# psteinb/libmultiviewnative

Hardware: AMD Instinct MI355X
Metric: RL iterations/sec on 512^3 f32, 6 views (higher is better)
Workload: dtype f32

## Files before the change

libmultiviewnative_amd/csrc/mvn_backend_emu.cpp:

```cpp
#ifndef MVN_HOST_EMU
#error "mvn_backend_emu.cpp is only for the MVN_HOST_EMU test build"
#endif

#include <atomic>
#include <chrono>
#include <cstdlib>
#include <cstring>
#include <map>
#include <memory>
#include <mutex>
#include <stdexcept>
#include <string>
#include <vector>

#include "mvn_backend.hpp"
#include "mvn_fixed_geom.hpp"
#include "mvn_wave_rows.hpp"

namespace mvn {
namespace be {

#define MVN_DISPATCH_T(T_, CALL)                                   \
  switch (T_) {                                                    \
    case 16: { constexpr int TT = 16; CALL; } break;               \
    case 8: { constexpr int TT = 8; CALL; } break;                 \
    case 4: { constexpr int TT = 4; CALL; } break;                 \
    case 2: { constexpr int TT = 2; CALL; } break;                 \
    case 1: { constexpr int TT = 1; CALL; } break;                 \
    default: throw std::invalid_argument("mvn: unsupported tile width"); \
  }


const char* backend_name() { return "host-emulation (test only)"; }

int device_count() {
  const char* e = std::getenv("MVN_EMU_DEVICES");
  const int n = e ? std::atoi(e) : 1;
  return n > 0 ? n : 1;
}
static thread_local int t_device = 0;
void set_device(int d) {
  if (d < 0 || d >= device_count()) throw std::runtime_error("emu: invalid device ordinal " + std::to_string(d));
  t_device = d;
}
int get_device() { return t_device; }
void device_name(int, char* name256) {
  std::memset(name256, 0, 256);
  std::strcpy(name256, "mvn host emulation");
}
static std::mutex g_mem_mu;
static std::map<void*, std::pair<int, size_t>> g_live;
static std::map<int, size_t> g_used;
static size_t emu_total() {
  const char* e = std::getenv("MVN_EMU_TOTAL_MB");
  return e ? (size_t)std::atoll(e) << 20 : (size_t)8 << 30;
}
long long device_total_mem(int) { return (long long)emu_total(); }
void device_mem_info(size_t* f, size_t* t) {
  std::lock_guard<std::mutex> lk(g_mem_mu);
  const size_t total = emu_total(), used = g_used[t_device];
  *t = total;
  *f = used < total ? total - used : 0;
}
void device_arch(int, int* major, int* minor) {
  *major = 0;
  *minor = 0;
}

void* dmalloc(size_t bytes) {
  {
    std::lock_guard<std::mutex> lk(g_mem_mu);
    if (g_used[t_device] + bytes > emu_total())
      throw std::runtime_error("emu: device memory exhausted (" + std::to_string(g_used[t_device]) + " + " +
                               std::to_string(bytes) + " bytes > MVN_EMU_TOTAL_MB)");
  }
  void* p = std::malloc(bytes ? bytes : 1);
  if (!p) throw std::bad_alloc();
  std::lock_guard<std::mutex> lk(g_mem_mu);
  g_live[p] = std::make_pair(t_device, bytes);
  g_used[t_device] += bytes;
  return p;
}
void dfree(void* p) {
  if (!p) return;
  {
    std::lock_guard<std::mutex> lk(g_mem_mu);
    auto it = g_live.find(p);
    if (it != g_live.end()) {
      g_used[it->second.first] -= it->second.second;
      g_live.erase(it);
    }
  }
  std::free(p);
}
void h2d(void* d, const void* h, size_t bytes, stream_t) { std::memcpy(d, h, bytes); }
void d2h(void* h, const void* d, size_t bytes, stream_t) { std::memcpy(h, d, bytes); }
void d2d(void* dst, const void* src, size_t bytes, stream_t) { std::memmove(dst, src, bytes); }
void h2d_2d(void* d, size_t dpitch, const void* h, size_t hpitch, size_t width, size_t height,
            stream_t) {
  for (size_t r = 0; r < height; ++r)
    std::memcpy((char*)d + r * dpitch, (const char*)h + r * hpitch, width);
}
void d2h_2d(void* h, size_t hpitch, const void* d, size_t dpitch, size_t width, size_t height,
            stream_t) {
  for (size_t r = 0; r < height; ++r)
    std::memcpy((char*)h + r * hpitch, (const char*)d + r * dpitch, width);
}
void d2d_2d(void* dst, size_t dpitch, const void* src, size_t spitch, size_t width, size_t height,
            stream_t) {
  for (size_t r = 0; r < height; ++r)
    std::memmove((char*)dst + r * dpitch, (const char*)src + r * spitch, width);
}
void dzero(void* d, size_t bytes, stream_t) { std::memset(d, 0, bytes); }
void enable_peer_access(int dev, int peer) {
  if (dev < 0 || dev >= device_count() || peer < 0 || peer >= device_count()) throw std::runtime_error("emu: invalid peer");
}
void copy_peer(void* dst, int, const void* src, int, size_t bytes, stream_t) { std::memmove(dst, src, bytes); }

int pointer_device(const void*) { return POINTER_ANY; }

stream_t stream_create() { return (stream_t)1; }
stream_t stream_create_upload() { return (stream_t)1; }
void stream_destroy(stream_t) {}
void stream_sync(stream_t) {}
void stream_wait_event(stream_t, event_t) {}

struct EmuEvent {
  std::chrono::steady_clock::time_point t;
};
event_t event_create() { return new EmuEvent(); }
event_t event_create_sync() { return new EmuEvent(); }
void event_destroy(event_t e) { delete (EmuEvent*)e; }
void event_record(event_t e, stream_t) { ((EmuEvent*)e)->t = std::chrono::steady_clock::now(); }
void event_sync(event_t) {}
float event_elapsed_ms(event_t a, event_t b) {
  return std::chrono::duration<float, std::milli>(((EmuEvent*)b)->t - ((EmuEvent*)a)->t).count();
}

bool graphs_supported() { return false; }
void capture_begin(stream_t) { throw std::runtime_error("mvn: no graphs in the host emulation"); }
graph_exec_t capture_end(stream_t) { throw std::runtime_error("mvn: no graphs in the host emulation"); }
void graph_launch(graph_exec_t, stream_t) { throw std::runtime_error("mvn: no graphs in the host emulation"); }
void graph_destroy(graph_exec_t) {}

static bool emu_wave_rows(const RowsParams& p, int kind_bit) {
  const char* m = std::getenv("MVN_WAVE_ROWS_MASK");
  const int mask = m && *m ? std::atoi(m) : 31;
  return (mask & kind_bit) && p.fixed && !p.lines && p.h == WrCfg::H && p.C == WrCfg::H;
}

template <int MODE, int EPI>
static void emu_wave_rows_run(const RowsParams& p) {
  typedef FxCtx<WrRegs, WrCfg::NT> Ctx;
  const long pairs = (p.rows + 1) / 2;
  const long full = (pairs + WrCfg::WAVES - 1) / WrCfg::WAVES;
  const long grid = full > 2 ? (full + 2) / 3 : full;
#pragma omp parallel
  {
    std::vector<char> lds(sizeof(cfloat) * WrCfg::lds_cfloats + 64);
    std::unique_ptr<Ctx> ctx(new Ctx());
#pragma omp for schedule(static)
    for (long b = 0; b < grid; ++b) wr_rows_body<MODE, EPI>(p, b, grid, (cfloat*)lds.data(), *ctx);
  }
}

template <int MODE>
static void emu_wave_rows_mode(const RowsParams& p) {
  switch (p.epi.mode) {
    case MVN_EPI_DIVIDE: emu_wave_rows_run<MODE, MVN_EPI_DIVIDE>(p); break;
    case MVN_EPI_DIVIDE_U16: emu_wave_rows_run<MODE, MVN_EPI_DIVIDE_U16>(p); break;
    case MVN_EPI_DIVIDE_NM: emu_wave_rows_run<MODE, MVN_EPI_DIVIDE_NM>(p); break;
    case MVN_EPI_DIVIDE_NM_U16: emu_wave_rows_run<MODE, MVN_EPI_DIVIDE_NM_U16>(p); break;
    case MVN_EPI_UPDATE: emu_wave_rows_run<MODE, MVN_EPI_UPDATE>(p); break;
    case MVN_EPI_UPDATE_STATS: emu_wave_rows_run<MODE, MVN_EPI_UPDATE_STATS>(p); break;
    case MVN_EPI_UPDATE_TV: emu_wave_rows_run<MODE, MVN_EPI_UPDATE_TV>(p); break;
    case MVN_EPI_UPDATE_STATS_TV: emu_wave_rows_run<MODE, MVN_EPI_UPDATE_STATS_TV>(p); break;
    case MVN_EPI_DELTA:
      if (MODE == MVN_WR_C2R) {
        emu_wave_rows_run<MVN_WR_C2R, MVN_EPI_DELTA>(p);
        break;
      }
      throw std::invalid_argument("mvn: DELTA epilogue only in the plain c2r pass");
    default: emu_wave_rows_run<MODE, MVN_EPI_STORE>(p); break;
  }
}

template <int H>
static long emu_rows_grid(long ntiles) {
  return FxRowsCfg<H>::WALK && ntiles > 2 ? (ntiles + 2) / 3 : ntiles;
}

static void emu_rows_lines(const RowsParams& p, long ntiles, int kind) {
  constexpr int H = 256;
  typedef FxCtx<FxRowsRegs<H>, FxRowsCfg<H>::NT> Ctx;
  typedef FxCtx<FxRowsStatRegs<H>, FxRowsCfg<H>::NT> SCtx;
  typedef FxCtx<FxRowsNmRegs<H>, FxRowsCfg<H>::NT> NCtx;
  if (!fx_rows_lines_ok<H>() || !p.fixed || p.h != H || p.C != H || !p.nyq_packed || p.lines_d1 < 1 ||
      p.lines_d1 % FxRowsCfg<H>::T || p.row_base % FxRowsCfg<H>::T || p.rows != ntiles * FxRowsCfg<H>::T)
    throw std::invalid_argument("mvn: line-layout last-axis pass outside its range");
#pragma omp parallel
  {
    std::vector<char> lds(sizeof(cfloat) * FxRowsCfg<H>::lds_cfloats + 64);
    std::unique_ptr<Ctx> ctx(new Ctx());
    std::unique_ptr<SCtx> sctx(new SCtx());
    std::unique_ptr<NCtx> nctx(new NCtx());
#pragma omp for schedule(static)
    for (long t = 0; t < ntiles; ++t) {
      cfloat* l = (cfloat*)lds.data();
      if (kind == 0) {
        fx_rows_run<H, 0, MVN_EPI_STORE, Ctx, true>(p, t, ntiles, l, *ctx);
      } else if (kind == 1) {
        switch (p.epi.mode) {
          case MVN_EPI_DIVIDE: fx_rows_run<H, 1, MVN_EPI_DIVIDE, Ctx, true>(p, t, ntiles, l, *ctx); break;
          case MVN_EPI_DIVIDE_U16: fx_rows_run<H, 1, MVN_EPI_DIVIDE_U16, Ctx, true>(p, t, ntiles, l, *ctx); break;
          case MVN_EPI_DIVIDE_NM: fx_rows_run_nm<H, 1, MVN_EPI_DIVIDE_NM, NCtx, true>(p, t, ntiles, l, *nctx); break;
          case MVN_EPI_DIVIDE_NM_U16: fx_rows_run_nm<H, 1, MVN_EPI_DIVIDE_NM_U16, NCtx, true>(p, t, ntiles, l, *nctx); break;
          case MVN_EPI_UPDATE: fx_rows_run<H, 1, MVN_EPI_UPDATE, Ctx, true>(p, t, ntiles, l, *ctx); break;
          case MVN_EPI_UPDATE_STATS: fx_rows_run_stats<H, 1, SCtx, true>(p, t, ntiles, l, *sctx); break;
          case MVN_EPI_UPDATE_TV: fx_rows_run<H, 1, MVN_EPI_UPDATE_TV, Ctx, true>(p, t, ntiles, l, *ctx); break;
          case MVN_EPI_UPDATE_STATS_TV: fx_rows_run_stats<H, 1, SCtx, true, MVN_EPI_UPDATE_STATS_TV>(p, t, ntiles, l, *sctx); break;
          case MVN_EPI_DELTA: fx_rows_run<H, 1, MVN_EPI_DELTA, Ctx, true>(p, t, ntiles, l, *ctx); break;
          default: fx_rows_run<H, 1, MVN_EPI_STORE, Ctx, true>(p, t, ntiles, l, *ctx); break;
        }
      } else {
        switch (p.epi.mode) {
          case MVN_EPI_DIVIDE: fx_rows_run<H, 2, MVN_EPI_DIVIDE, Ctx, true>(p, t, ntiles, l, *ctx); break;
          case MVN_EPI_DIVIDE_U16: fx_rows_run<H, 2, MVN_EPI_DIVIDE_U16, Ctx, true>(p, t, ntiles, l, *ctx); break;
          case MVN_EPI_DIVIDE_NM: fx_rows_run_nm<H, 2, MVN_EPI_DIVIDE_NM, NCtx, true>(p, t, ntiles, l, *nctx); break;
          case MVN_EPI_DIVIDE_NM_U16: fx_rows_run_nm<H, 2, MVN_EPI_DIVIDE_NM_U16, NCtx, true>(p, t, ntiles, l, *nctx); break;
          case MVN_EPI_UPDATE: fx_rows_run<H, 2, MVN_EPI_UPDATE, Ctx, true>(p, t, ntiles, l, *ctx); break;
          case MVN_EPI_UPDATE_STATS: fx_rows_run_stats<H, 2, SCtx, true>(p, t, ntiles, l, *sctx); break;
          case MVN_EPI_UPDATE_TV: fx_rows_run<H, 2, MVN_EPI_UPDATE_TV, Ctx, true>(p, t, ntiles, l, *ctx); break;
          case MVN_EPI_UPDATE_STATS_TV: fx_rows_run_stats<H, 2, SCtx, true, MVN_EPI_UPDATE_STATS_TV>(p, t, ntiles, l, *sctx); break;
          default: fx_rows_run<H, 2, MVN_EPI_STORE, Ctx, true>(p, t, ntiles, l, *ctx); break;
        }
      }
    }
  }
}

static std::atomic<long> g_mid_fused_launches{0};
long mid_fused_launch_count() { return g_mid_fused_launches.load(); }

template <int K>
static void emu_mid_fused(const MidFusedParams& p) {
  typedef FxCtx<MfRegs<K>, MF_NT> Ctx;
  const long blocks = mf_blocks(p);
#pragma omp parallel
  {
    std::vector<cfloat> lds(MF_LDS_CFLOATS + 8);
    std::unique_ptr<Ctx> ctx(new Ctx());
#pragma omp for schedule(static)
    for (long b = 0; b < blocks; ++b) mf_body<K>(p, b, lds.data(), *ctx);
  }
}
#define MVN_MF_TAP_COUNTS(X) X(1) X(3) X(5) X(7) X(9) X(11) X(13) X(15) X(17) X(19) X(21) X(23) X(25) X(27) X(29) X(31)
void launch_mid_fused(const MidFusedParams& p, stream_t) {
  mf_check(p);
  if (p.mode == MF_TAPS) {
    typedef FxCtx<MfRegs<1>, MF_NT> Ctx;
    const long blocks = mf_blocks(p);
#pragma omp parallel
    {
      std::vector<cfloat> lds(MF_LDS_CFLOATS + 8);
      std::unique_ptr<Ctx> ctx(new Ctx());
#pragma omp for schedule(static)
      for (long b = 0; b < blocks; ++b) mf_taps_body(p, b, lds.data(), *ctx);
    }
    return;
  }
  ++g_mid_fused_launches;
  switch (mvn_dim0_taps_template(p.k)) {
#define X(K) case K: emu_mid_fused<K>(p); break;
    MVN_MF_TAP_COUNTS(X)
#undef X
    default: throw std::invalid_argument("mvn: no fused middle pass for this tap count");
  }
}

template <int H>
static void emu_rows_fused(const RowsParams& p, long ntiles) {
  typedef FxCtx<FxRowsRegs<H>, FxRowsCfg<H>::NT> Ctx;
  typedef FxCtx<FxRowsStatRegs<H>, FxRowsCfg<H>::NT> SCtx;
  typedef FxCtx<FxRowsNmRegs<H>, FxRowsCfg<H>::NT> NCtx;
  const long grid = emu_rows_grid<H>(ntiles);
#pragma omp parallel
  {
    std::vector<char> lds(sizeof(cfloat) * FxRowsCfg<H>::lds_cfloats + 64);
    std::unique_ptr<Ctx> ctx(new Ctx());
    std::unique_ptr<SCtx> sctx(new SCtx());
    std::unique_ptr<NCtx> nctx(new NCtx());
#pragma omp for schedule(static)
    for (long t = 0; t < grid; ++t) {
      cfloat* l = (cfloat*)lds.data();
      switch (p.epi.mode) {
        case MVN_EPI_DIVIDE: fx_rows_run<H, 2, MVN_EPI_DIVIDE>(p, t, grid, l, *ctx); break;
        case MVN_EPI_DIVIDE_U16: fx_rows_run<H, 2, MVN_EPI_DIVIDE_U16>(p, t, grid, l, *ctx); break;
        case MVN_EPI_DIVIDE_NM: fx_rows_run_nm<H, 2, MVN_EPI_DIVIDE_NM, NCtx>(p, t, grid, l, *nctx); break;
        case MVN_EPI_DIVIDE_NM_U16: fx_rows_run_nm<H, 2, MVN_EPI_DIVIDE_NM_U16, NCtx>(p, t, grid, l, *nctx); break;
        case MVN_EPI_UPDATE: fx_rows_run<H, 2, MVN_EPI_UPDATE>(p, t, grid, l, *ctx); break;
        case MVN_EPI_UPDATE_STATS: fx_rows_run_stats<H, 2, SCtx>(p, t, grid, l, *sctx); break;
        case MVN_EPI_UPDATE_TV: fx_rows_run<H, 2, MVN_EPI_UPDATE_TV>(p, t, grid, l, *ctx); break;
        case MVN_EPI_UPDATE_STATS_TV: fx_rows_run_stats<H, 2, SCtx, false, MVN_EPI_UPDATE_STATS_TV>(p, t, grid, l, *sctx); break;
        default: fx_rows_run<H, 2, MVN_EPI_STORE>(p, t, grid, l, *ctx); break;
      }
    }
  }
}

void launch_rows_c2r_r2c(const RowsParams& p0, long ntiles, int, size_t lds_bytes, stream_t) {
  RowsParams p = p0;
  mvn_arm_poison(p.epi);
  if (p.lines) return emu_rows_lines(p, ntiles, 2);
  if (emu_wave_rows(p, mvn_epi_divides(p.epi.mode) ? 4 : 8)) return emu_wave_rows_mode<MVN_WR_C2R_R2C>(p);
  if (!p.fixed) {
#pragma omp parallel
    {
      std::vector<char> lds(lds_bytes + 64);
#pragma omp for schedule(static)
      for (long t = 0; t < ntiles; ++t) {
        cfloat* l = (cfloat*)lds.data();
        if (p.epi.mode == MVN_EPI_UPDATE_STATS) {
          MVN_DISPATCH_T(p.T, (rows_c2r_even_body<TT, true, true>(p, t, 0, 1, l)));
        } else if (p.epi.mode == MVN_EPI_UPDATE_STATS_TV) {
          MVN_DISPATCH_T(p.T, (rows_c2r_even_body<TT, true, true, false, true>(p, t, 0, 1, l)));
        } else if (p.epi.mode == MVN_EPI_UPDATE_TV) {
          MVN_DISPATCH_T(p.T, (rows_c2r_even_body<TT, true, false, false, true>(p, t, 0, 1, l)));
        } else if (p.epi.mode == MVN_EPI_DIVIDE_NM) {
          MVN_DISPATCH_T(p.T, (rows_c2r_even_body<TT, true, false, false, false, true>(p, t, 0, 1, l)));
        } else if (p.epi.mode == MVN_EPI_DIVIDE_NM_U16) {
          MVN_DISPATCH_T(p.T, (rows_c2r_even_body<TT, true, false, true, false, true>(p, t, 0, 1, l)));
        } else if (p.epi.mode == MVN_EPI_DIVIDE_U16) {
          MVN_DISPATCH_T(p.T, (rows_c2r_even_body<TT, true, false, true>(p, t, 0, 1, l)));
        } else {
          MVN_DISPATCH_T(p.T, (rows_c2r_even_body<TT, true>(p, t, 0, 1, l)));
        }
      }
    }
    return;
  }
  switch (p.h) {
#define X(H) case H: emu_rows_fused<H>(p, ntiles); return;
    MVN_FIXED_ROWS_LENGTHS(X)
#undef X
    default: throw std::invalid_argument("mvn: no fixed kernel");
  }
}

template <int H>
static void emu_rows_fixed(const RowsParams& p, long ntiles, bool r2c) {
  typedef FxCtx<FxRowsRegs<H>, FxRowsCfg<H>::NT> Ctx;
  typedef FxCtx<FxRowsStatRegs<H>, FxRowsCfg<H>::NT> SCtx;
  typedef FxCtx<FxRowsNmRegs<H>, FxRowsCfg<H>::NT> NCtx;
  const long grid = emu_rows_grid<H>(ntiles);
#pragma omp parallel
  {
    std::vector<char> lds(sizeof(cfloat) * FxRowsCfg<H>::lds_cfloats + 64);
    std::unique_ptr<Ctx> ctx(new Ctx());
    std::unique_ptr<SCtx> sctx(new SCtx());
    std::unique_ptr<NCtx> nctx(new NCtx());
#pragma omp for schedule(static)
    for (long t = 0; t < grid; ++t) {
      cfloat* l = (cfloat*)lds.data();
      if (r2c)
        fx_rows_run<H, 0, MVN_EPI_STORE>(p, t, grid, l, *ctx);
      else {
        switch (p.epi.mode) {
          case MVN_EPI_DIVIDE: fx_rows_run<H, 1, MVN_EPI_DIVIDE>(p, t, grid, l, *ctx); break;
          case MVN_EPI_DIVIDE_U16: fx_rows_run<H, 1, MVN_EPI_DIVIDE_U16>(p, t, grid, l, *ctx); break;
          case MVN_EPI_DIVIDE_NM: fx_rows_run_nm<H, 1, MVN_EPI_DIVIDE_NM, NCtx>(p, t, grid, l, *nctx); break;
          case MVN_EPI_DIVIDE_NM_U16: fx_rows_run_nm<H, 1, MVN_EPI_DIVIDE_NM_U16, NCtx>(p, t, grid, l, *nctx); break;
          case MVN_EPI_UPDATE: fx_rows_run<H, 1, MVN_EPI_UPDATE>(p, t, grid, l, *ctx); break;
          case MVN_EPI_UPDATE_STATS: fx_rows_run_stats<H, 1, SCtx>(p, t, grid, l, *sctx); break;
          case MVN_EPI_UPDATE_TV: fx_rows_run<H, 1, MVN_EPI_UPDATE_TV>(p, t, grid, l, *ctx); break;
          case MVN_EPI_UPDATE_STATS_TV: fx_rows_run_stats<H, 1, SCtx, false, MVN_EPI_UPDATE_STATS_TV>(p, t, grid, l, *sctx); break;
          case MVN_EPI_DELTA: fx_rows_run<H, 1, MVN_EPI_DELTA>(p, t, grid, l, *ctx); break;
          default: fx_rows_run<H, 1, MVN_EPI_STORE>(p, t, grid, l, *ctx); break;
        }
      }
    }
  }
}

template <int N, int MODE>
static void emu_strided_fixed_mode(const StridedParams& p0, long nblocks) {
  typedef FxStridedSel<N, MODE> Sel;
  typedef typename Sel::Ctx Ctx;
  StridedParams p = p0;
  p.nblocks = nblocks;
  const long grid = nblocks > 1 ? (nblocks + 1) / 2 : 1;
#pragma omp parallel
  {
    std::vector<char> lds(sizeof(cfloat) * FxStridedCfg<N>::lds_cfloats + 64);
    std::unique_ptr<Ctx> ctx(new Ctx());
#pragma omp for schedule(static)
    for (long b = 0; b < grid; ++b) Sel::run(p, b, nblocks, grid, (cfloat*)lds.data(), *ctx);
  }
}

static std::atomic<long> g_split_launches{0};
long split_launch_count() { return g_split_launches.load(); }

template <int N>
static bool emu_try_split(int mode, const StridedParams& p, long nblocks) {
  if constexpr (FxSplitCfg<N>::USE) {
    typedef FxSplitCfg<N> C;
    if (mode == MVN_ST_FWD_MUL_INV || p.cstride != 1 || p.ncols % C::T != 0 || p.tiles_per_outer < 1)
      return false;
    StridedParams q = p;
    const long outer = nblocks / p.tiles_per_outer;
    q.tiles_per_outer = p.ncols / C::T;
    q.T = q.TP = C::T;
    const long nb = outer * q.tiles_per_outer;
    q.nblocks = nb;
    ++g_split_launches;
    const long grid = nb > 1 ? (nb + 1) / 2 : 1;
    typedef FxCtx<FxSplitRegs<N>, C::NT> Ctx;
#pragma omp parallel
    {
      std::vector<char> lds(sizeof(cfloat) * C::lds_cfloats + 64);
      std::unique_ptr<Ctx> ctx(new Ctx());
#pragma omp for schedule(static)
      for (long b = 0; b < grid; ++b) {
        if (mode == MVN_ST_FWD)
          fx_strided_split_body<N, MVN_ST_FWD>(q, b, nb, grid, (cfloat*)lds.data(), *ctx);
        else
          fx_strided_split_body<N, MVN_ST_INV>(q, b, nb, grid, (cfloat*)lds.data(), *ctx);
      }
    }
    return true;
  } else {
    (void)mode; (void)p; (void)nblocks;
    return false;
  }
}

template <int N>
static void emu_strided_fixed(int mode, const StridedParams& p, long nblocks) {
  if (emu_try_split<N>(mode, p, nblocks)) return;
  if (mode == MVN_ST_FWD) emu_strided_fixed_mode<N, MVN_ST_FWD>(p, nblocks);
  if (mode == MVN_ST_INV) emu_strided_fixed_mode<N, MVN_ST_INV>(p, nblocks);
  if (mode == MVN_ST_FWD_MUL_INV) emu_strided_fixed_mode<N, MVN_ST_FWD_MUL_INV>(p, nblocks);
}

static bool emu_rows_fixed_dispatch(const RowsParams& p, long ntiles, bool r2c) {
  switch (p.h) {
#define X(H) case H: emu_rows_fixed<H>(p, ntiles, r2c); return true;
    MVN_FIXED_ROWS_LENGTHS(X)
#undef X
    default: return false;
  }
}

static bool emu_strided_fixed_dispatch(int mode, const StridedParams& p, long nblocks) {
  switch (p.ax.n) {
#define X(N) case N: emu_strided_fixed<N>(mode, p, nblocks); return true;
    MVN_FIXED_STRIDED_LENGTHS(X)
#undef X
    default: return false;
  }
}

void launch_rows_r2c(const RowsParams& p, bool even, long ntiles, int, size_t lds_bytes,
                     stream_t) {
  if (p.lines) return emu_rows_lines(p, ntiles, 0);
  if (emu_wave_rows(p, 1)) return emu_wave_rows_run<MVN_WR_R2C, MVN_EPI_STORE>(p);
  if (p.fixed) {
    if (!emu_rows_fixed_dispatch(p, ntiles, true)) throw std::invalid_argument("mvn: no fixed kernel");
    return;
  }
#pragma omp parallel
  {
    std::vector<char> lds(lds_bytes + 64);
#pragma omp for schedule(static)
    for (long t = 0; t < ntiles; ++t) {
      cfloat* l = (cfloat*)lds.data();
      if (even) {
        MVN_DISPATCH_T(p.T, rows_r2c_even_body<TT>(p, t, 0, 1, l));
      } else {
        MVN_DISPATCH_T(p.T, rows_r2c_odd_body<TT>(p, t, 0, 1, l));
      }
    }
  }
}

void launch_rows_c2r(const RowsParams& p0, bool even, long ntiles, int, size_t lds_bytes,
                     stream_t) {
  RowsParams p = p0;
  mvn_arm_poison(p.epi);
  if (p.lines) return emu_rows_lines(p, ntiles, 1);
  if (emu_wave_rows(p, p.epi.mode == MVN_EPI_DELTA ? 16 : 2)) return emu_wave_rows_mode<MVN_WR_C2R>(p);
  if (p.fixed) {
    if (!emu_rows_fixed_dispatch(p, ntiles, false)) throw std::invalid_argument("mvn: no fixed kernel");
    return;
  }
#pragma omp parallel
  {
    std::vector<char> lds(lds_bytes + 64);
#pragma omp for schedule(static)
    for (long t = 0; t < ntiles; ++t) {
      cfloat* l = (cfloat*)lds.data();
// ... 293 lines not shown
```

libmultiviewnative_amd/csrc/mvn_engine.cpp:

```cpp
#include "mvn_engine.hpp"

#include <algorithm>
#include <cmath>
#include <atomic>
#include <cstdlib>
#include <cstring>

#include "mvn_fixed_geom.hpp"

#include <cstdio>
#include <cstdlib>
#include <cstring>
#include <stdexcept>

namespace mvn {

static const size_t kLdsSoftBudget = 80 * 1024;
static const size_t kLdsHardBudget = 160 * 1024;
static const size_t kSideMinBytes = 16u << 20;

const char* kernel_kind_name(int k) {
  static const char* names[KK_COUNT] = {"rows_r2c",    "rows_c2r",  "rows_fused_div",
                                        "rows_fused_upd", "axis1_fwd", "axis1_inv",
                                        "axis0_fused", "axis0_fwd",  "axis0_inv",
                                        "nyquist",     "other",     "axis0_direct", "mid_fused",
                                        "tv_factor"};
  return (k >= 0 && k < KK_COUNT) ? names[k] : "?";
}

be::Event Profiler::get_event() {
  if (pool_.empty()) return be::Event::timing();
  be::Event e = std::move(pool_.back());
  pool_.pop_back();
  return e;
}

void Profiler::begin(int kind, be::stream_t s) {
  if (!enabled) return;
  Rec r;
  r.kind = kind;
  r.a = get_event();
  r.b = get_event();
  be::event_record(r.a.get(), s);
  recs_.push_back(std::move(r));
}

void Profiler::end(be::stream_t s) {
  if (!enabled || recs_.empty()) return;
  be::event_record(recs_.back().b.get(), s);
}

void Profiler::collect() {
  for (size_t i = 0; i < recs_.size(); ++i) {
    be::event_sync(recs_[i].b.get());
    total_ms[recs_[i].kind] += be::event_elapsed_ms(recs_[i].a.get(), recs_[i].b.get());
    count[recs_[i].kind] += 1;
    pool_.push_back(std::move(recs_[i].a));
    pool_.push_back(std::move(recs_[i].b));
  }
  recs_.clear();
}

void Profiler::reset() {
  collect();
  for (int k = 0; k < KK_COUNT; ++k) {
    total_ms[k] = 0;
    count[k] = 0;
  }
}

Profiler::~Profiler() {
  try {
    collect();
  } catch (...) {
  }
}

struct ProfScope {
  Profiler* p;
  be::stream_t s;
  ProfScope(Profiler* p_, int kind, be::stream_t s_) : p(p_), s(s_) {
    if (p) p->begin(kind, s);
  }
  ~ProfScope() {
    if (p) p->end(s);
  }
};

template <typename T>
static be::DeviceBuffer<T> upload(const std::vector<T>& src) {
  be::DeviceBuffer<T> d(sizeof(T) * src.size());
  be::h2d(d.get(), src.data(), sizeof(T) * src.size(), nullptr);
  return d;
}

DevAxis::DevAxis(int n, bool composite) : host(n, composite) {
  tw = upload(host.tw);
  rev = upload(host.rev);
  inv = upload(host.inv);
  if (!host.tws.empty()) tws = upload(host.tws);
  if (host.bluestein) {
    chirp = upload(host.chirp);
    bhat = upload(host.bhat);
  }
  be::stream_sync(nullptr);
  view = host.view(tw.get(), rev.get(), inv.get(), tws.get(), chirp.get(), bhat.get());
}

static int env_int(const char* name, int dflt) {
  const char* v = std::getenv(name);
  return (v && *v) ? std::atoi(v) : dflt;
}

PassGeom Plan3D::pick_geom(int n, bool generic, bool rows, int max_t) {
  static const int cand[5] = {16, 8, 4, 2, 1};
  PassGeom g;
  bool found = false;
  for (int pass = 0; pass < 2 && !found; ++pass) {
    const size_t budget = pass == 0 ? kLdsSoftBudget : kLdsHardBudget;
    for (int i = 0; i < 5; ++i) {
      const int T = cand[i];
      if (T > max_t) continue;
      const int TP = rows ? (T | 1) : T;
      const size_t one = (size_t)n * (size_t)TP * sizeof(cfloat);
      const size_t twb = (size_t)n * sizeof(cfloat);
      const size_t bytes = one * (generic ? 2 : 1) + twb;
      if (bytes <= budget) {
        g.T = T;
        g.TP = TP;
        g.lds_bytes = bytes;
        g.lds_alt = generic ? (long)n * TP : 0;
        g.lds_tw = (long)n * TP * (generic ? 2 : 1);
        found = true;
        break;
      }
    }
  }
  if (!found)
    throw std::invalid_argument("mvn: axis length " + std::to_string(n) +
                                " does not fit the single-pass LDS FFT (160 KiB)");
  if (!rows && g.T < 8 && max_t >= 8) {
    const size_t one = (size_t)n * 8 * sizeof(cfloat);
    const size_t bytes = one * (generic ? 2 : 1) + (size_t)n * sizeof(cfloat);
    if (bytes <= kLdsHardBudget - 4096) {
      g.T = g.TP = 8;
      g.lds_bytes = bytes;
      g.lds_alt = generic ? (long)n * 8 : 0;
      g.lds_tw = (long)n * 8 * (generic ? 2 : 1);
    }
  }
  const long work = (long)n * g.T / 8;
  g.threads = work >= 512 ? 512 : (work >= 256 ? 256 : (work >= 128 ? 128 : 64));
  return g;
}

FormSwitches FormSwitches::from_env() {
  FormSwitches sw;
  sw.direct = env_int("MVN_DIM0_DIRECT", 1) != 0;
  sw.direct_max = env_int("MVN_DIM0_DIRECT_MAX", MVN_D0_MAX_TAPS);
  sw.min_plane = env_int("MVN_DIM0_DIRECT_MIN_PLANE", 131072);
  sw.min_items = env_int("MVN_DIM0_DIRECT_MIN_ITEMS", 0);
  sw.mid_fused = env_int("MVN_MID_FUSED", 1);
  sw.fixed = env_int("MVN_NO_FIXED", 0) == 0;
  return sw;
}

bool rows_fixed(const Layout& L, bool fixed) {
  int T = 0, threads = 0;
  size_t lds = 0;
  return fixed && L.even && fixed_rows_geom(L.h, &T, &threads, &lds) && L.rows % (size_t)T == 0;
}
bool ax1_fixed(const Layout& L, bool fixed) {
  int T = 0, threads = 0;
  size_t lds = 0;
  return fixed && fixed_strided_geom(L.d1, &T, &threads, &lds) && L.C % T == 0;
}
bool ax0_fixed(const Layout& L, bool fixed) {
  int T = 0, threads = 0;
  size_t lds = 0;
  return fixed && fixed_strided_geom(L.d0, &T, &threads, &lds) && ((long)L.d1 * L.C) % T == 0;
}

bool lines_capable(const Layout& L, bool fixed) {
  int T = 0, threads = 0;
  size_t lds = 0;
  return rows_fixed(L, fixed) && fixed_rows_geom(L.h, &T, &threads, &lds) && T == 16 && L.h == 256 && L.C == 256 &&
         L.d1 == MF_N1;
}

bool FormRule::direct(const int* kdims) const {
  if (!sw.direct || kdims[0] > sw.direct_max || !mvn_dim0_direct_possible(kdims[0], L.d0) ||
      mvn_dim0_items_for(kdims[0], L.d0, (long)L.d1 * L.C, sw.min_plane) < sw.min_items)
    return false;
  const Layout T(taps_depth(kdims[0]), L.d1, L.d2);
  return rows_fixed(T, sw.fixed) == rows_fixed(L, plan_fixed) && ax1_fixed(T, sw.fixed) == ax1_fixed(L, plan_fixed);
}

bool FormRule::lines_taps(const int* kdims) const {
  return sw.mid_fused != 0 && lines_capable(L, plan_fixed) && direct(kdims) &&
         lines_capable(Layout(taps_depth(kdims[0]), L.d1, L.d2), sw.fixed) && mvn_dim0_taps_template(kdims[0]) <= 31;
}

bool FormRule::lines_worth(int k0) const { return sw.mid_fused >= 2 || L.d0 >= 3 * k0; }

bool FormRule::all_direct(const kernel_list_t& k) const {
  for (const std::array<int, 3>& d : k)
    if (!direct(d.data())) return false;
  return true;
}

bool FormRule::all_lines(const kernel_list_t& k) const {
  for (const std::array<int, 3>& d : k)
    if (!lines(d.data())) return false;
  return true;
}

Plan3D::Plan3D(int dev, int d0, int d1, int d2, bool fixed_allowed)
    : device(dev), L(d0, d1, d2), fixed(fixed_allowed), ax2(L.h, rows_fixed(L, fixed)), ax1(d1, ax1_fixed(L, fixed)),
      ax0(d0, ax0_fixed(L, fixed)) {
  no_poison = be::DeviceBuffer<unsigned>(64);
  be::dzero(no_poison.get(), 64, nullptr);
  be::stream_sync(nullptr);
  if (L.even) {
    std::vector<cfloat> roots((size_t)L.h / 2 + 1);
    for (size_t k = 0; k < roots.size(); ++k) {
      double a = -2.0 * M_PI * (double)k / (double)d2;
      roots[k].x = (float)std::cos(a);
      roots[k].y = (float)std::sin(a);
    }
    twr = be::DeviceBuffer<cfloat>(sizeof(cfloat) * roots.size());
    be::h2d(twr.get(), roots.data(), sizeof(cfloat) * roots.size(), nullptr);
    be::stream_sync(nullptr);
  }
  g_rows = pick_geom(ax2.host.nfft, ax2.host.generic, true, 16);
  g_ax1 = pick_geom(ax1.host.nfft, ax1.host.generic, false, 16);
  g_ax0 = pick_geom(ax0.host.nfft, ax0.host.generic, false, 16);
  g_nyq1 = g_ax1;
  g_nyq0 = g_ax0;
  g_nyq1_line = pick_geom(ax1.host.nfft, ax1.host.generic, false, 1);
  {
    int T = 0, threads = 0;
    size_t lds = 0;
    if (rows_fixed(L, fixed)) {
      fixed_rows_geom(L.h, &T, &threads, &lds);
      fx_rows = true;
      gx_rows.T = T;
      gx_rows.threads = threads;
      gx_rows.lds_bytes = lds;
    }
    if (ax1_fixed(L, fixed)) {
      fixed_strided_geom(d1, &T, &threads, &lds);
      fx_ax1 = true;
      gx_ax1.T = gx_ax1.TP = T;
      gx_ax1.threads = threads;
      gx_ax1.lds_bytes = lds;
    }
    if (ax0_fixed(L, fixed)) {
      fixed_strided_geom(d0, &T, &threads, &lds);
      fx_ax0 = true;
      gx_ax0.T = gx_ax0.TP = T;
      gx_ax0.threads = threads;
      gx_ax0.lds_bytes = lds;
    }
  }
}

static long rows_in_range(const Plan3D& P, long row0, long nrows) {
  const long all = (long)P.L.rows;
  const long n = nrows < 0 ? all - row0 : nrows;
  if (row0 < 0 || n < 1 || row0 + n > all) throw std::out_of_range("mvn: row range of a last-axis pass");
  if (P.rows_need_full_tiles() && (row0 % P.rows_tile() || n % P.rows_tile()))
    throw std::logic_error("mvn: a row range of the fixed last-axis kernels must be whole tiles");
  return n;
}

static void lines_args(const Plan3D& P, RowsParams& p, long row0, const void* nyq, const void* real_side,
                       const void* cplx_side) {
  if (!P.lines_capable()) throw std::logic_error("mvn: this shape has no line-layout last-axis passes");
  if (nyq) throw std::logic_error("mvn: the line layout keeps the Nyquist bins in the DC column");
  if (real_side && real_side == cplx_side) throw std::logic_error("mvn: a plain last-axis pass on the line layout is out of place");
  p.lines = 1;
  p.lines_d1 = P.L.d1;
  p.row_base = row0;
  p.nyq_packed = 1;
}

void Plan3D::rows_r2c(const float* in_real, cfloat* out, cfloat* out_nyq, be::stream_t s,
                      Profiler* prof, long row0, long nrows, bool lines) const {
  const long R = rows_in_range(*this, row0, nrows);
  const void* real0 = in_real;
  in_real += row0 * L.RP;
  if (!lines) out += row0 * L.C;
  if (out_nyq) out_nyq += row0;
  RowsParams p;
  std::memset(&p, 0, sizeof(p));
  p.ax = ax2.view;
  p.twr = twr.get();
  p.d2 = L.d2;
  p.h = L.h;
  p.C = L.C;
  p.RP = L.RP;
  p.rows = R;
  p.T = g_rows.T;
  p.TP = g_rows.TP;
  p.lds_alt = g_rows.lds_alt;
  p.lds_tw = g_rows.lds_tw;
  p.hmul = mvn_fastdiv_mul((unsigned)L.h);
  p.Cmul = mvn_fastdiv_mul((unsigned)L.C);
  p.in_real = in_real;
  p.out_cplx = out;
  p.out_nyq = out_nyq;
  p.nyq_packed = (L.even && !out_nyq) ? 1 : 0;
  if (lines) lines_args(*this, p, row0, out_nyq, real0, out);
  ProfScope ps(prof, KK_ROWS_R2C, s);
  if (fx_rows) {
    p.fixed = 1;
    p.T = gx_rows.T;
    be::launch_rows_r2c(p, true, R / p.T, gx_rows.threads, gx_rows.lds_bytes, s);
    return;
  }
  const long ntiles = (R + p.T - 1) / p.T;
  be::launch_rows_r2c(p, L.even, ntiles, g_rows.threads, g_rows.lds_bytes, s);
}

void Plan3D::rows_c2r(const cfloat* in, const cfloat* in_nyq, float* out_real,
                      const EpilogueParams& epi_all, be::stream_t s, Profiler* prof, long row0,
                      long nrows, bool lines, const MvnStatsParams* st) const {
  const long R = rows_in_range(*this, row0, nrows);
  const void* cplx0 = in;
  const void* real0 = out_real;
  if (!lines) in += row0 * L.C;
  if (in_nyq) in_nyq += row0;
  if (out_real) out_real += row0 * L.RP;
  EpilogueParams epi = epi_all;
  const long eoff = row0 * L.RP;
  if (mvn_epi_u16(epi.mode) && row0 != 0) throw std::logic_error("mvn: a row range on a uint16 image volume");
  if (epi.view) epi.view += eoff;
  if (epi.psi) epi.psi += eoff;
  if (epi.weights) epi.weights += eoff;
  if (epi.delta) epi.delta += eoff;
  if (epi.tv) epi.tv += eoff;
  RowsParams p;
  std::memset(&p, 0, sizeof(p));
  p.ax = ax2.view;
  p.twr = twr.get();
  p.d2 = L.d2;
  p.h = L.h;
  p.C = L.C;
  p.RP = L.RP;
  p.rows = R;
  p.T = g_rows.T;
  p.TP = g_rows.TP;
  p.lds_alt = g_rows.lds_alt;
  p.lds_tw = g_rows.lds_tw;
  p.hmul = mvn_fastdiv_mul((unsigned)L.h);
  p.Cmul = mvn_fastdiv_mul((unsigned)L.C);
  p.in_cplx = in;
  p.in_nyq = in_nyq;
  p.nyq_packed = (L.even && !in_nyq) ? 1 : 0;
  if (lines) lines_args(*this, p, row0, in_nyq, real0, cplx0);
  p.out_real = out_real;
  p.epi = epi;
  if (!p.epi.poison) {
    p.epi.poison = no_poison.get();
    p.epi.poison_epoch = 0xffffffffu;
  }
  if (st) {
    p.st = *st;
    p.st.row0 = row0;
  }
  ProfScope ps(prof, KK_ROWS_C2R, s);
  if (fx_rows) {
    p.fixed = 1;
    p.T = gx_rows.T;
    be::launch_rows_c2r(p, true, R / p.T, gx_rows.threads, gx_rows.lds_bytes, s);
    return;
  }
  const long ntiles = (R + p.T - 1) / p.T;
  be::launch_rows_c2r(p, L.even, ntiles, g_rows.threads, g_rows.lds_bytes, s);
}

void Plan3D::rows_c2r_r2c(cfloat* data, cfloat* nyq, const EpilogueParams& epi_all, be::stream_t s,
                          Profiler* prof, long row0, long nrows, bool lines, const MvnStatsParams* st) const {
  if (!L.even) throw std::logic_error("mvn: rows_c2r_r2c needs an even last extent");
  const long R = rows_in_range(*this, row0, nrows);
  if (!lines) data += row0 * L.C;
  if (nyq) nyq += row0;
  EpilogueParams epi = epi_all;
  const long eoff = row0 * L.RP;
  if (mvn_epi_u16(epi.mode) && row0 != 0) throw std::logic_error("mvn: a row range on a uint16 image volume");
  if (epi.view) epi.view += eoff;
  if (epi.psi) epi.psi += eoff;
  if (epi.weights) epi.weights += eoff;
  if (epi.delta) epi.delta += eoff;
  if (epi.tv) epi.tv += eoff;
  RowsParams p;
  std::memset(&p, 0, sizeof(p));
  p.ax = ax2.view;
  p.twr = twr.get();
  p.d2 = L.d2;
  p.h = L.h;
  p.C = L.C;
  p.RP = L.RP;
  p.rows = R;
  p.in_cplx = data;
  p.in_nyq = nyq;
  p.out_cplx = data;
  p.out_nyq = nyq;
  p.nyq_packed = nyq ? 0 : 1;
  if (lines) lines_args(*this, p, row0, nyq, nullptr, nullptr);
  p.epi = epi;
  if (!p.epi.poison) {
    p.epi.poison = no_poison.get();
    p.epi.poison_epoch = 0xffffffffu;
  }
  if (st) {
    p.st = *st;
    p.st.row0 = row0;
  }
  ProfScope ps(prof, mvn_epi_reads_psi(epi.mode) ? KK_ROWS_FUSED_UPD : KK_ROWS_FUSED, s);
  if (fx_rows) {
    p.fixed = 1;
    p.T = gx_rows.T;
    be::launch_rows_c2r_r2c(p, R / p.T, gx_rows.threads, gx_rows.lds_bytes, s);
    return;
  }
  p.T = g_rows.T;
  p.TP = g_rows.TP;
  p.lds_alt = g_rows.lds_alt;
  p.lds_tw = g_rows.lds_tw;
  p.hmul = mvn_fastdiv_mul((unsigned)L.h);
  p.Cmul = mvn_fastdiv_mul((unsigned)L.C);
  const long ntiles = (R + p.T - 1) / p.T;
  be::launch_rows_c2r_r2c(p, ntiles, g_rows.threads, g_rows.lds_bytes, s);
}

void Plan3D::mid_fused(const cfloat* in, cfloat* out, const cfloat* taps, int k, int kd, unsigned* poison,
                       unsigned poison_epoch, be::stream_t s, Profiler* prof, int zbeg, int zcount, int n_peers,
                       unsigned* const* peers) const {
  if (!lines_capable()) throw std::logic_error("mvn: this shape has no fused middle pass");
  MidFusedParams p;
  std::memset(&p, 0, sizeof(p));
  p.in = in;
  p.out = out;
  p.taps = taps;
  p.kd = kd;
  p.tw = ax1.view.tw;
  p.d0 = L.d0;
  p.H = L.C;
  p.k = k;
  p.h = k / 2;
  p.seg = 0;
  p.mode = MF_CONV;
  p.packed = 1;
  p.poison = poison;
  p.poison_epoch = poison_epoch;
  p.zbeg = zbeg;
  p.zcount = zcount;
  p.n_peers = n_peers;
  p.poison_peers = peers;
  ProfScope ps(prof, KK_MID_FUSED, s);
  be::launch_mid_fused(p, s);
}

void Plan3D::taps_to_lines(cfloat* taps, be::stream_t s) const {
  if (!lines_capable()) throw std::logic_error("mvn: this shape has no fused middle pass");
  MidFusedParams p;
  std::memset(&p, 0, sizeof(p));
  p.in = taps;
  p.out = taps;
  p.tw = ax1.view.tw;
  p.d0 = L.d0;
  p.H = L.C;
  p.mode = MF_TAPS;
  be::launch_mid_fused(p, s);
}

static StridedParams make_strided(const DevAxis& ax, const PassGeom& g, cfloat* data,
                                  const cfloat* spec, long ostride, long estride, long cstride,
                                  int ncols) {
  StridedParams p;
  std::memset(&p, 0, sizeof(p));
  p.ax = ax.view;
  p.data = data;
  p.spec = spec;
  p.ostride = ostride;
  p.estride = estride;
  p.cstride = cstride;
  p.ncols = ncols;
  p.T = g.T;
  p.TP = g.TP;
  p.lds_alt = g.lds_alt;
  p.lds_tw = g.lds_tw;
  p.tiles_per_outer = (ncols + g.T - 1) / g.T;
  return p;
}

void SideStream::create() {
  s = be::Stream::create();
  fork = be::Event::sync_only();
  join = be::Event::sync_only();
}

void SideStream::fork_from(be::stream_t main) {
  be::event_record(fork.get(), main);
  be::stream_wait_event(s.get(), fork.get());
}

void SideStream::join_into(be::stream_t main) {
  be::event_record(join.get(), s.get());
  be::stream_wait_event(main, join.get());
}

void Plan3D::axis1(int mode, cfloat* data, cfloat* nyq, be::stream_t s, Profiler* prof,
                   be::stream_t s_nyq, int z0, int nz) const {
  if (!s_nyq) s_nyq = s;
  if (nz < 0) nz = L.d0 - z0;
  if (z0 < 0 || nz < 1 || z0 + nz > L.d0) throw std::out_of_range("mvn: plane range of a dim1 pass");
  data += (size_t)z0 * L.d1 * L.C;
  if (nyq) nyq += (size_t)z0 * L.d1;
  const bool ride = nyq_rides() && L.even && nyq;
  {
    const PassGeom& g = fx_ax1 ? gx_ax1 : g_ax1;
    StridedParams p = make_strided(ax1, g, data, nullptr, (long)L.d1 * L.C, L.C, 1, L.C);
    p.fixed = fx_ax1 ? 1 : 0;
    ProfScope ps(prof, mode == MVN_ST_FWD ? KK_AXIS1_FWD : KK_AXIS1_INV, s);
    if (ride) {
      StridedParams r = make_strided(ax1, g_nyq1_line, nyq, nullptr, 0, 1, L.d1, nz);
      r.is_nyq = 1;
      be::launch_strided(mode, p, (long)nz * p.tiles_per_outer, g.threads, g.lds_bytes, s, &r, g_nyq1_line.lds_bytes);
    } else {
      be::launch_strided(mode, p, (long)nz * p.tiles_per_outer, g.threads, g.lds_bytes, s);
    }
  }
  if (L.even && nyq && !ride) {
    StridedParams p = make_strided(ax1, g_nyq1, nyq, nullptr, 0, 1, L.d1, nz);
    p.is_nyq = 1;
    ProfScope ps(s_nyq == s ? prof : nullptr, KK_NYQ, s_nyq);
    be::launch_strided(mode, p, p.tiles_per_outer, g_nyq1.threads, g_nyq1.lds_bytes, s_nyq);
  }
}

void Plan3D::retile_spectrum(const cfloat* natural, cfloat* tiled, be::stream_t s) const {
  const long cols = (long)L.d1 * L.C;
  const int T = gx_ax0.T;
  be::launch_copy3d((float*)tiled, 2L * T, 2L * T * L.d0, (const float*)natural, 2L * cols, 2L * T, 2 * T,
                    L.d0, (int)(cols / T), s);
}

void Plan3D::axis0(int mode, cfloat* data, cfloat* nyq, const cfloat* spec,
                   const cfloat* spec_nyq, be::stream_t s, Profiler* prof, be::stream_t s_nyq,
                   const cfloat* src, const cfloat* src_nyq, bool spec_tiled) const {
  if (!s_nyq) s_nyq = s;
  const int kind = mode == MVN_ST_FWD ? KK_AXIS0_FWD
                                      : (mode == MVN_ST_INV ? KK_AXIS0_INV : KK_AXIS0_FUSED);
  {
    const long cols = (long)L.d1 * L.C;
    if (cols > 0x7fffffffL) throw std::invalid_argument("mvn: d1*d2 too large");
    const PassGeom& g = fx_ax0 ? gx_ax0 : g_ax0;
    StridedParams p = make_strided(ax0, g, data, spec, 0, cols, 1, (int)cols);
    p.fixed = fx_ax0 ? 1 : 0;
    p.src = src;
    if (spec_tiled && !fx_ax0) throw std::logic_error("mvn: tile-contiguous spectra need the fixed dim0 kernels");
    p.spec_tiled = spec_tiled ? 1 : 0;
    ProfScope ps(prof, kind, s);
    be::launch_strided(mode, p, p.tiles_per_outer, g.threads, g.lds_bytes, s);
  }
  if (L.even) {
    StridedParams p = make_strided(ax0, g_nyq0, nyq, spec_nyq, 0, L.d1, 1, L.d1);
    p.is_nyq = 1;
    p.src = src_nyq;
    ProfScope ps(s_nyq == s ? prof : nullptr, KK_NYQ, s_nyq);
    be::launch_strided(mode, p, p.tiles_per_outer, g_nyq0.threads, g_nyq0.lds_bytes, s_nyq);
  }
}

void Plan3D::forward(float* vol, cfloat* nyq, be::stream_t s, Profiler* prof) const {
  rows_r2c(vol, (cfloat*)vol, nyq, s, prof);
  axis1(MVN_ST_FWD, (cfloat*)vol, nyq, s, prof);
  axis0(MVN_ST_FWD, (cfloat*)vol, nyq, nullptr, nullptr, s, prof);
}

void Plan3D::backward(float* vol, cfloat* nyq, float scale, be::stream_t s,
                      Profiler* prof) const {
  axis0(MVN_ST_INV, (cfloat*)vol, nyq, nullptr, nullptr, s, prof);
  axis1(MVN_ST_INV, (cfloat*)vol, nyq, s, prof);
// ... 2070 lines not shown
```

libmultiviewnative_amd/csrc/mvn_fixed.hpp:

```cpp
#pragma once

#include <type_traits>

#include "mvn_pass_bodies.hpp"

#if defined(__HIPCC__) && !defined(MVN_HOST_EMU)
typedef float4 qfloat;
#else
struct alignas(16) qfloat {
  float x, y, z, w;
};
#endif

MVN_HD qfloat qmake(float x, float y, float z, float w) {
  qfloat q;
  q.x = x;
  q.y = y;
  q.z = z;
  q.w = w;
  return q;
}

#if defined(__HIPCC__) && !defined(MVN_HOST_EMU)
template <typename Regs, int NT>
// ... 647 lines not shown
  constexpr int R = fx_radix(N, S), M = fx_M(N, S), CH = C::CH, TPQ = C::TPQ, NT = C::NT;
  static_assert(C::M0 % (R * M) == 0, "a stage's blocks must tile a sub-line");
  constexpr int nwork = (C::W / R) * CH;
  constexpr int iters = (nwork + NT - 1) / NT;
  qfloat* buf = reinterpret_cast<qfloat*>(bufc);
#pragma unroll
  for (int it = 0; it < iters; ++it) {
    const int w = tid + it * NT;
    if (nwork % NT != 0 && w >= nwork) break;
    const int b = w / CH, q = w % CH;
    const int blk = b / M, j2 = b % M;
    qfloat* p = buf + (blk * R * M + j2) * TPQ + q;
    qfloat a[R];
#pragma unroll
    for (int j = 0; j < R; ++j) a[j] = p[j * M * TPQ];
    cfloat tw[fx_rs(R)];
    fx_tw_row<R>(twl + (fx_twoff(N, S) - C::TW1) + j2 * fx_rs(R), tw);
    if (!DIF) {
#pragma unroll
      for (int k = 1; k < R; ++k) a[k] = fx_qmul_dir<SIGN>(a[k], tw[k]);
    }
    fx_dft_q<R, SIGN>(a);
    if (DIF) {
#pragma unroll
      for (int k = 1; k < R; ++k) a[k] = fx_qmul_dir<SIGN>(a[k], tw[k]);
    }
#pragma unroll
    for (int j = 0; j < R; ++j) p[j * M * TPQ] = a[j];
    MVN_SCHED_FENCE();
  }
}

template <int N, int SIGN, bool DIF, int S, int TO, typename Ctx>
struct FxStagesQWin {
  static MVN_HD void run(cfloat* buf, const cfloat* twl, Ctx& ctx) {
    constexpr int NT_ = FxSplitCfg<N>::NT;
    (void)NT_;
    if constexpr (DIF ? (S <= TO) : (S >= TO)) {
      MVN_PHASE(ctx, (fx_stage_q_win<N, S, SIGN, DIF>(buf, twl, tid)));
      FxStagesQWin<N, SIGN, DIF, DIF ? S + 1 : S - 1, TO, Ctx>::run(buf, twl, ctx);
    }
  }
};

template <int N>
MVN_HD void fx_sp_tables(const StridedParams& P, cfloat* twl, int tid) {
  typedef FxSplitCfg<N> C;
  fx_copy_table<C::NT>(twl, P.ax.tws + C::TW1, fx_twsize(N) - C::TW1, tid);
}

template <int N, int WIN>
MVN_HD void fx_sp_collect(const cfloat* buf, FxSplitRegs<N>& r, int tid) {
  typedef FxSplitCfg<N> C;
#pragma unroll
  for (int it = 0; it < C::IT0; ++it) {
    const int w = tid + it * C::NT;
    const int q = w % C::CH, j2 = w / C::CH;
    const qfloat* d = reinterpret_cast<const qfloat*>(buf) + j2 * C::TPQ + q;
#pragma unroll
    for (int kk = 0; kk < C::SUB; ++kk) r.a[it * 8 + C::SUB * WIN + kk] = d[kk * C::M0 * C::TPQ];
  }
}

template <int N, bool PERM, int IT_LO, int IT_HI>
MVN_HD void fx_sp_fetch(const StridedParams& P, long base, int win, FxSplitRegs<N>& r, int tid) {
  typedef FxSplitCfg<N> C;
  constexpr int CH = C::CH, RL = C::RL;
  const cfloat* src0 = (P.src ? P.src : P.data) + base;
  const long kstep = PERM ? (long)fx_W(N, C::NS - 1) * P.estride : P.estride;
#pragma unroll
  for (int it = IT_LO; it < IT_HI; ++it) {
    int w = tid + it * C::NT;
    if (C::NWL % C::NT != 0 && w >= C::NWL) w = tid % C::NWL;
    const int b = w / CH, q = w % CH;
    const int pos = win * C::W + b * RL;
    long off = (long)(PERM ? fx_rev<N>(pos) : pos) * P.estride + 2 * q;
#pragma unroll
    for (int k = 0; k < RL; ++k) {
      r.pf[it * RL + k] = *reinterpret_cast<const qfloat*>(src0 + off);
      off += kstep;
      MVN_JIT_ADDRESS(off);
    }
  }
}

template <int N, int SIGN>
MVN_HD void fx_sp_last_to_lds(cfloat* buf, FxSplitRegs<N>& r, int tid) {
  typedef FxSplitCfg<N> C;
  constexpr int CH = C::CH, RL = C::RL, ITL = C::ITL;
#pragma unroll
  for (int it = 0; it < ITL; ++it) {
    const int w = tid + it * C::NT;
    if (C::NWL % C::NT != 0 && w >= C::NWL) break;
    const int b = w / CH, q = w % CH;
    qfloat x[RL];
#pragma unroll
    for (int k = 0; k < RL; ++k) x[k] = r.pf[it * RL + k];
    fx_dft_q<RL, SIGN>(x);
    qfloat* d = reinterpret_cast<qfloat*>(buf) + (b * RL) * C::TPQ + q;
#pragma unroll
    for (int k = 0; k < RL; ++k) d[k * C::TPQ] = x[k];
    MVN_SCHED_FENCE();
  }
}

template <int N, int SIGN, bool PERM>
MVN_HD void fx_sp_stage0_store(const StridedParams& P, long base, const cfloat* twl, FxSplitRegs<N>& r,
                               int tid) {
  typedef FxSplitCfg<N> C;
  const long rstep = (long)C::M0 * P.estride;
  cfloat* dst0 = P.data + base;
#pragma unroll
  for (int it = 0; it < C::IT0; ++it) {
    const int w = tid + it * C::NT;
    const int q = w % C::CH, j2 = w / C::CH;
    cfloat tw[8];
    fx_tw_row<8>(twl + fx_twoff(N, 0) + j2 * fx_rs(8), tw);
    qfloat a[8];
    a[0] = r.a[it * 8];
#pragma unroll
    for (int k = 1; k < 8; ++k) a[k] = fx_qmul_dir<SIGN>(r.a[it * 8 + k], tw[k]);
    fx_dft_q<8, SIGN>(a);
    if (PERM) {
#pragma unroll
      for (int k = 0; k < 8; ++k)
        *reinterpret_cast<qfloat*>(dst0 + (long)fx_inv<N>(j2 + k * C::M0) * P.estride + 2 * q) = a[k];
    } else {
      long off = (long)j2 * P.estride + 2 * q;
#pragma unroll
      for (int k = 0; k < 8; ++k) {
        *reinterpret_cast<qfloat*>(dst0 + off) = a[k];
        off += rstep;
        MVN_JIT_ADDRESS(off);
      }
    }
    MVN_SCHED_FENCE();
  }
}

template <int N>
MVN_HD long fx_sp_base(const StridedParams& P, long block) {
  const unsigned o = (unsigned)block / (unsigned)P.tiles_per_outer;
  const unsigned t = (unsigned)block - o * (unsigned)P.tiles_per_outer;
  return (long)o * P.ostride + (long)t * FxSplitCfg<N>::T;
}

template <int N, int SIGN, bool PERM, int WIN, typename Ctx>
struct FxSplitWindows {
  static MVN_HD void run(const StridedParams& P, long base, long next_base, bool has_next, cfloat* buf,
                         const cfloat* twl, Ctx& ctx) {
    typedef FxSplitCfg<N> C;
    constexpr int NT_ = C::NT, NS = C::NS;
    (void)NT_;
    if constexpr (WIN < C::NWIN) {
      if constexpr (WIN + 1 < C::NWIN) {
        MVN_PHASE(ctx, (fx_sp_last_to_lds<N, SIGN>(buf, r, tid), fx_sp_fetch<N, PERM, 0, C::ITL>(P, base, WIN + 1, r, tid)));
      } else {
        MVN_PHASE(ctx, (fx_sp_last_to_lds<N, SIGN>(buf, r, tid)));
      }
      FxStagesQWin<N, SIGN, false, NS - 2, 1, Ctx>::run(buf, twl, ctx);
      MVN_PHASE(ctx, (fx_sp_collect<N, WIN>(buf, r, tid)));
      FxSplitWindows<N, SIGN, PERM, WIN + 1, Ctx>::run(P, base, next_base, has_next, buf, twl, ctx);
    }
  }
};

template <int N, int MODE, typename Ctx>
MVN_HD void fx_strided_split_body(const StridedParams& P, long first, long total, long step,
                                  cfloat* lds, Ctx& ctx) {
  typedef FxSplitCfg<N> C;
  constexpr int NT_ = C::NT;
  constexpr int SIGN = MODE == MVN_ST_FWD ? -1 : +1;
  constexpr bool PERM = MODE == MVN_ST_FWD;
  (void)NT_;
  cfloat* buf = lds;
  cfloat* twl = lds + C::W * C::TP;
  if (first >= total) return;
  MVN_PHASE(ctx, (fx_sp_tables<N>(P, twl, tid)));
  for (long block = first; block < total; block += step) {
    MVN_TILE_LOOP_TOP(ctx);
    const long base = fx_sp_base<N>(P, block);
    MVN_PHASE_NOSYNC(ctx, (fx_sp_fetch<N, PERM, 0, C::ITL>(P, base, 0, r, tid)));
    const bool has_next = block + step < total;
    const long next_base = has_next ? fx_sp_base<N>(P, block + step) : base;
    FxSplitWindows<N, SIGN, PERM, 0, Ctx>::run(P, base, next_base, has_next, buf, twl, ctx);
    MVN_PHASE_NOSYNC(ctx, (fx_sp_stage0_store<N, SIGN, PERM>(P, base, twl, r, tid)));
  }
}

template <int N, int MODE>
struct FxStridedSel {
  static constexpr bool LDS_FUSED = MODE == MVN_ST_FWD_MUL_INV && FxFusedCfg<N>::USE;
  static constexpr int NT = LDS_FUSED ? FxFusedCfg<N>::NT : FxStridedCfg<N>::NT;
  static constexpr int WAVES = LDS_FUSED ? FxFusedCfg<N>::WAVES : FxStridedCfg<N>::WAVES;
  typedef typename std::conditional<LDS_FUSED, FxFusedRegs<N>, FxStridedRegs<N>>::type Regs;
  typedef FxCtx<Regs, NT> Ctx;
  static MVN_HD void run(const StridedParams& P, long first, long total, long step, cfloat* lds,
                         Ctx& ctx) {
    if constexpr (LDS_FUSED) {
      for (long block = first; block < total; block += step) fx_fused_lds_body<N>(P, block, lds, ctx);
    } else
      fx_strided_body<N, MODE>(P, first, total, step, lds, ctx);
  }
};

template <int H>
struct FxRowsCfg {
  static constexpr bool PAD = fx_pow2(H);
  static constexpr int WALK_T = (H >= 640 || H == 480)                         ? 2
                                : (H == 192 || H == 144 || H == 80 || H == 48) ? 8
                                : (H >= 160 && !(fx_pow2(H) && H < 512))       ? 4
                                                                               : 0;
  static constexpr bool SMALL = WALK_T > 0;
  static constexpr bool WALK = SMALL;
  static constexpr bool TWT = WALK;
  static constexpr int T = SMALL ? WALK_T : (H > 512 ? 8 : 16);
  static constexpr int TP = T + 1;
  static constexpr int QR = H / 2;
  static constexpr int R0 = fx_radix(H, 0);
  static constexpr int M0 = fx_M(H, 0);
  static constexpr int NT = SMALL ? ((M0 * T + 63) / 64) * 64
                                  : fx_pick_nt(1024, H * T / 8 >= 64 ? H * T / 8 : 64, T * QR, M0 * T, H / 2 * T);
  static constexpr int NTD = NT > 0 ? NT : 1;
  static constexpr int U = (T * QR + NTD - 1) / NTD;
  static constexpr int IT0 = (M0 * T + NTD - 1) / NTD;
  static constexpr bool EXACT = (T * QR) % NTD == 0 && (M0 * T) % NTD == 0 && (H / 2 * T) % NTD == 0;
  static constexpr int ROWS = fx_rows_alloc(H, PAD);
  static constexpr int TILE = (ROWS * TP + 1) & ~1;
  static constexpr int TWR = (H / 2 + 2) & ~1;
  static constexpr int lds_cfloats = TILE + fx_twsize(H) + TWR + H / 2;
  static constexpr int ITP = (H / 2 * T + NTD - 1) / NTD;
  static_assert(fx_smooth(H) && H % 2 == 0 && H >= 32 && H <= 1024, "unsupported fixed length");
  static_assert(NT >= 64 && R0 == 8, "stage 0: whole radix-8 butterflies per thread");
  static_assert(sizeof(cfloat) * lds_cfloats <= 160 * 1024, "tile does not fit the LDS");
};

template <int H>
struct FxRowsRegs {
  qfloat v[FxRowsCfg<H>::U];
  cfloat ea[FxRowsCfg<H>::IT0][FxRowsCfg<H>::R0];
  cfloat eb[FxRowsCfg<H>::IT0][FxRowsCfg<H>::R0];
  unsigned eu[FxRowsCfg<H>::IT0][FxRowsCfg<H>::R0];
};
template <int H>
struct FxRowsStatRegs : FxRowsRegs<H> {
  MvnStatAcc st;
};
template <int H>
struct FxRowsNmRegs : FxRowsRegs<H> {
  MvnNmAcc nm;
};
template <int H, int EPI>
using FxRowsRegsFor = typename std::conditional<
    mvn_epi_base(EPI) == MVN_EPI_UPDATE_STATS, FxRowsStatRegs<H>,
    typename std::conditional<mvn_epi_nm(EPI), FxRowsNmRegs<H>, FxRowsRegs<H>>::type>::type;

struct FxPair {
  int a, b;
};

template <int H>
MVN_HD void fx_build_pair_table(FxPair* tab, int tid) {
  typedef FxRowsCfg<H> C;
  for (int k = tid; k < H / 2; k += C::NT) {
    FxPair e;
    e.a = fx_row<C::PAD>(fx_inv<H>(k)) * C::TP;
    e.b = fx_row<C::PAD>(fx_inv<H>(k == 0 ? H / 2 : H - k)) * C::TP;
    tab[k] = e;
  }
}

template <int R>
MVN_HD void fx_load_tw_row(const cfloat* row, cfloat* tw) {
  const qfloat* t4 = reinterpret_cast<const qfloat*>(row);
#pragma unroll
  for (int k = 0; k < fx_rs(R) / 2; ++k) {
    const qfloat t = t4[k];
    tw[2 * k] = cmake(t.x, t.y);
    tw[2 * k + 1] = cmake(t.z, t.w);
  }
}

template <int H>
MVN_HD void fx_rows_tables(const RowsParams& P, cfloat* tws, cfloat* twr, int tid) {
  typedef FxRowsCfg<H> C;
  if constexpr (C::TWT) {
    for (int st = 0; st < fx_nstages(H); ++st) {
      const int M = fx_M(H, st), Q = fx_rs(fx_radix(H, st)) / 2;
      if (M <= 1) continue;
      const qfloat* src = reinterpret_cast<const qfloat*>(P.ax.tws + fx_twoff(H, st));
      qfloat* dst = reinterpret_cast<qfloat*>(tws + fx_twoff(H, st));
      for (int i = tid; i < M * Q; i += C::NT) {
        const qfloat t = src[i];
        dst[(i % Q) * M + i / Q] = qmake(t.x, t.y, t.z, t.w);
      }
    }
  } else {
    fx_copy_table<C::NT>(tws, P.ax.tws, fx_twsize(H), tid);
  }
  fx_copy_table<C::NT>(twr, P.twr, H / 2 + 1, tid);
  fx_build_pair_table<H>(reinterpret_cast<FxPair*>(twr + C::TWR), tid);
}

template <int H>
MVN_HD void fx_r2c_load_stage0(const RowsParams& P, long r0, cfloat* buf, cfloat* tws, cfloat* twr,
                               int tid) {
  typedef FxRowsCfg<H> C;
  constexpr int TP = C::TP, NT = C::NT, R = C::R0, M = C::M0;
  cfloat a[C::IT0][R];
#pragma unroll
  for (int it = 0; it < C::IT0; ++it) {
    const int w = tid + it * NT;
    if (!C::EXACT && w >= M * C::T) break;
    const int j2 = w % M, rho = w / M;
    const cfloat* src = reinterpret_cast<const cfloat*>(P.in_real + (r0 + rho) * P.RP) + j2;
#pragma unroll
    for (int j = 0; j < R; ++j) a[it][j] = src[j * M];
  }
  if (!C::WALK) fx_rows_tables<H>(P, tws, twr, tid);
#pragma unroll
  for (int it = 0; it < C::IT0; ++it) {
    const int w = tid + it * NT;
    if (!C::EXACT && w >= M * C::T) break;
    const int j2 = w % M, rho = w / M;
    cfloat tw[fx_rs(R)];
    if constexpr (C::WALK)
      fx_tw_fetch<H, 0, C::TWT>(tws, j2, tw);
    else
      fx_load_tw_row<R>(P.ax.tws + j2 * fx_rs(R), tw);
    dftR<R, -1>(a[it]);
#pragma unroll
    for (int k = 1; k < R; ++k) a[it][k] = cmul(a[it][k], tw[k]);
    cfloat* p = buf + fx_row<C::PAD>(j2) * TP + rho;
#pragma unroll
    for (int k = 0; k < R; ++k) p[fx_rowoff<C::PAD, R, M>(k) * TP] = a[it][k];
  }
}

template <int H>
MVN_HD void fx_r2c_post(const RowsParams& P, long r0, cfloat* buf, const cfloat* twr, int tid) {
  typedef FxRowsCfg<H> C;
  constexpr int T = C::T, NT = C::NT;
  const FxPair* tab = reinterpret_cast<const FxPair*>(twr + C::TWR);
#pragma unroll
  for (int it = 0; it < C::ITP; ++it) {
    const int i = tid + it * NT;
    if (!C::EXACT && i >= H / 2 * T) break;
    const int k = i / T, rho = i % T;
    const FxPair t = tab[k];
    cfloat* pa = buf + t.a + rho;
    cfloat* pb = buf + t.b + rho;
    const cfloat zk = *pa;
    const cfloat zm = *pb;
    if (k == 0) {
      if (P.nyq_packed) {
        *pa = cmake(zk.x + zk.y, zk.x - zk.y);
      } else {
        *pa = cmake(zk.x + zk.y, 0.f);
        P.out_nyq[r0 + rho] = cmake(zk.x - zk.y, 0.f);
      }
      *pb = cconj(zm);
    } else {
      const cfloat E = cscale(cadd_c(zk, zm), 0.5f);
      const cfloat D = cscale(csub_c(zk, zm), 0.5f);
      const cfloat G = cmul(D, twr[k]);
      *pa = cadd_i<-1>(E, G);
      *pb = cconj_add_i<-1>(E, G);
    }
  }
}

template <int EPI>
constexpr bool fx_lines_wide() {
  return !mvn_epi_reads_psi(EPI);
}
template <int H>
MVN_HD long fx_lines_base(const RowsParams& P, long r0) {
  const long R = P.row_base + r0;
  const long z = R / P.lines_d1;
  return z * (long)H * P.lines_d1 + (R - z * P.lines_d1);
}

template <int H, bool LINES = false, bool W16 = true>
MVN_HD void fx_r2c_store(const RowsParams& P, long r0, const cfloat* buf, int tid) {
  typedef FxRowsCfg<H> C;
  constexpr int TP = C::TP, NT = C::NT, U = C::U;
  if constexpr (LINES) {
    static_assert((C::T * H) % NT == 0, "line layout: whole sweeps");
    cfloat* dst = P.out_cplx + fx_lines_base<H>(P, r0);
    if constexpr (W16) {
#pragma unroll
      for (int u = 0; u < U; ++u) {
        const int e = tid + u * NT;
        const int r2 = 2 * (e % (C::T / 2)), p = e / (C::T / 2);
        const cfloat a = buf[fx_row<C::PAD>(p) * TP + r2], b = buf[fx_row<C::PAD>(p) * TP + r2 + 1];
        *reinterpret_cast<qfloat*>(dst + (long)p * P.lines_d1 + r2) = qmake(a.x, a.y, b.x, b.y);
      }
    } else {
#pragma unroll
      for (int u = 0; u < 2 * U; ++u) {
        const int e = tid + u * NT;
        const int rho = e % C::T, p = e / C::T;
        dst[(long)p * P.lines_d1 + rho] = buf[fx_row<C::PAD>(p) * TP + rho];
      }
    }
    return;
  }
#pragma unroll
  for (int u = 0; u < U; ++u) {
    const int e = tid + u * NT;
    if (!C::EXACT && e >= C::T * C::QR) break;
    const int rho = e / C::QR, kk = e % C::QR;
    const cfloat a = buf[fx_row<C::PAD>(2 * kk) * TP + rho];
    const cfloat b = buf[fx_row<C::PAD>(2 * kk + 1) * TP + rho];
    reinterpret_cast<qfloat*>(P.out_cplx + (r0 + rho) * P.C)[kk] = qmake(a.x, a.y, b.x, b.y);
  }
}

template <int H, typename Ctx, bool LINES = false>
MVN_HD void fx_rows_r2c_body(const RowsParams& P, long tile, cfloat* lds, Ctx& ctx) {
  typedef FxRowsCfg<H> C;
  constexpr int T = C::T, TP = C::TP, NT = C::NT, NT_ = C::NT;
  (void)NT_;
  const long r0 = tile * T;
  cfloat* buf = lds;
  cfloat* tws = lds + C::TILE;
  cfloat* twr = tws + fx_twsize(H);
  MVN_PHASE(ctx, (fx_r2c_load_stage0<H>(P, r0, buf, tws, twr, tid)));
  fx_dif<H, T, TP, C::PAD, NT, -1, 1, C::TWT>(buf, tws, ctx);
  MVN_PHASE(ctx, (fx_r2c_post<H>(P, r0, buf, twr, tid)));
  MVN_PHASE(ctx, (fx_r2c_store<H, LINES, fx_lines_wide<MVN_EPI_STORE>()>(P, r0, buf, tid)));
}

template <int EPI>
MVN_HD cfloat fx_epilogue_pair_value(const EpilogueParams& e, long i, cfloat z, cfloat a, cfloat b) {
  return mvn_epilogue_pair_value<mvn_epi_tv(EPI)>(mvn_epi_math(EPI), e, i, z, a, b);
}

template <int EPI>
MVN_HD cfloat fx_operand(cfloat a, unsigned u) {
  if constexpr (mvn_epi_u16(EPI))
    return mvn_u16_pair_widen(u);
  else
    return a;
}

template <int H, int EPI, bool LINES = false>
MVN_HD void fx_c2r_load(const RowsParams& P, long r0, cfloat* buf, cfloat* tws, cfloat* twr,
                        FxRowsRegs<H>& r, int tid) {
  typedef FxRowsCfg<H> C;
  constexpr int TP = C::TP, NT = C::NT, U = C::U;
  if constexpr (LINES) {
    const cfloat* src = P.in_cplx + fx_lines_base<H>(P, r0);
    if constexpr (fx_lines_wide<EPI>()) {
#pragma unroll
      for (int u = 0; u < U; ++u) {
        const int e = tid + u * NT;
        r.v[u] = *reinterpret_cast<const qfloat*>(src + (long)(e / (C::T / 2)) * P.lines_d1 + 2 * (e % (C::T / 2)));
      }
    } else {
#pragma unroll
      for (int u = 0; u < U; ++u) {
        const int e0 = tid + 2 * u * NT, e1 = e0 + NT;
        const cfloat a = src[(long)(e0 / C::T) * P.lines_d1 + e0 % C::T];
        const cfloat b = src[(long)(e1 / C::T) * P.lines_d1 + e1 % C::T];
        r.v[u] = qmake(a.x, a.y, b.x, b.y);
      }
    }
  } else {
#pragma unroll
  for (int u = 0; u < U; ++u) {
    const int e = tid + u * NT;
    if (!C::EXACT && e >= C::T * C::QR) break;
    const int rho = e / C::QR, kk = e % C::QR;
    r.v[u] = reinterpret_cast<const qfloat*>(P.in_cplx + (r0 + rho) * P.C)[kk];
  }
  }
  constexpr int mode = EPI;
  const float* pa = mvn_epi_divides(mode) ? P.epi.view : P.epi.psi;
  if constexpr (mvn_epi_u16(mode)) {
#pragma unroll
    for (int it = 0; it < C::IT0; ++it) {
      const int w = tid + it * NT;
      if (!C::EXACT && w >= C::M0 * C::T) break;
      const unsigned short* src = P.epi.view16 + (r0 + w / C::M0) * P.RP + 2 * (w % C::M0);
#pragma unroll
      for (int jo = 0; jo < C::R0; ++jo) r.eu[it][jo] = mvn_u16_pair_fetch(src + 2 * jo * C::M0);
    }
  } else if (mode != MVN_EPI_STORE) {
#pragma unroll
    for (int it = 0; it < C::IT0; ++it) {
      const int w = tid + it * NT;
      if (!C::EXACT && w >= C::M0 * C::T) break;
      const cfloat* src = reinterpret_cast<const cfloat*>(pa + (r0 + w / C::M0) * P.RP) + (w % C::M0);
#pragma unroll
      for (int jo = 0; jo < C::R0; ++jo) r.ea[it][jo] = src[jo * C::M0];
    }
  }
  if (mvn_epi_reads_psi(mode)) {
#pragma unroll
    for (int it = 0; it < C::IT0; ++it) {
      const int w = tid + it * NT;
      if (!C::EXACT && w >= C::M0 * C::T) break;
      const cfloat* src =
          reinterpret_cast<const cfloat*>(P.epi.weights + (r0 + w / C::M0) * P.RP) + (w % C::M0);
#pragma unroll
      for (int jo = 0; jo < C::R0; ++jo) r.eb[it][jo] = src[jo * C::M0];
    }
  }
  if (!C::WALK) fx_rows_tables<H>(P, tws, twr, tid);
  if constexpr (LINES) {
    if constexpr (fx_lines_wide<EPI>()) {
#pragma unroll
      for (int u = 0; u < U; ++u) {
        const int e = tid + u * NT;
        cfloat* q = buf + fx_row<C::PAD>(e / (C::T / 2)) * TP + 2 * (e % (C::T / 2));
        q[0] = cmake(r.v[u].x, r.v[u].y);
        q[1] = cmake(r.v[u].z, r.v[u].w);
      }
    } else {
#pragma unroll
      for (int u = 0; u < U; ++u) {
        const int e0 = tid + 2 * u * NT, e1 = e0 + NT;
        buf[fx_row<C::PAD>(e0 / C::T) * TP + e0 % C::T] = cmake(r.v[u].x, r.v[u].y);
        buf[fx_row<C::PAD>(e1 / C::T) * TP + e1 % C::T] = cmake(r.v[u].z, r.v[u].w);
      }
    }
    return;
  }
#pragma unroll
  for (int u = 0; u < U; ++u) {
    const int e = tid + u * NT;
    if (!C::EXACT && e >= C::T * C::QR) break;
    const int rho = e / C::QR, kk = e % C::QR;
    buf[fx_row<C::PAD>(2 * kk) * TP + rho] = cmake(r.v[u].x, r.v[u].y);
    buf[fx_row<C::PAD>(2 * kk + 1) * TP + rho] = cmake(r.v[u].z, r.v[u].w);
  }
}

template <int H>
MVN_HD void fx_c2r_pre(const RowsParams& P, long r0, cfloat* buf, const cfloat* twr, int tid) {
  typedef FxRowsCfg<H> C;
  constexpr int T = C::T, NT = C::NT;
  const FxPair* tab = reinterpret_cast<const FxPair*>(twr + C::TWR);
#pragma unroll
  for (int it = 0; it < C::ITP; ++it) {
    const int i = tid + it * NT;
    if (!C::EXACT && i >= H / 2 * T) break;
    const int k = i / T, rho = i % T;
    const FxPair t = tab[k];
    cfloat* pa = buf + t.a + rho;
    cfloat* pb = buf + t.b + rho;
    const cfloat xk = *pa;
    const cfloat xm = *pb;
    if (k == 0) {
      const float xh = P.nyq_packed ? xk.y : P.in_nyq[r0 + rho].x;
      *pa = cmake(xk.x + xh, xk.x - xh);
      *pb = cmake(2.f * xm.x, -2.f * xm.y);
    } else {
      const cfloat E = cadd_c(xk, xm);
      const cfloat Dk = csub_c(xk, xm);
      const cfloat O = cmulc(Dk, twr[k]);
      *pa = cadd_i<+1>(E, O);
      *pb = cconj_add_i<+1>(E, O);
    }
  }
}

template <int H, bool KEEP, int EPI, typename Regs>
MVN_HD void fx_c2r_stage0_epilogue(const RowsParams& P, long r0, cfloat* buf, const cfloat* tws, Regs& r, int tid) {
  typedef FxRowsCfg<H> C;
  constexpr int TP = C::TP, NT = C::NT, R = C::R0, M = C::M0;
#pragma unroll
  for (int it = 0; it < C::IT0; ++it) {
    const int w = tid + it * NT;
    if (!C::EXACT && w >= M * C::T) break;
    const int j2 = w % M, rho = w / M;
    cfloat* p = buf + fx_row<C::PAD>(j2) * TP + rho;
    cfloat a[R];
#pragma unroll
    for (int k = 0; k < R; ++k) a[k] = p[fx_rowoff<C::PAD, R, M>(k) * TP];
    cfloat tw[fx_rs(R)];
    fx_tw_fetch<H, 0, C::TWT>(tws, j2, tw);
#pragma unroll
    for (int k = 1; k < R; ++k) a[k] = cmulc(a[k], tw[k]);
    dftR<R, +1>(a);
    const long i0 = (r0 + rho) * P.RP + 2 * j2;
    if constexpr (mvn_epi_nm(EPI)) {
      const bool row_in = mvn_stat_row_in(P.st, r0 + rho);
#pragma unroll
      for (int jo = 0; jo < R; ++jo) {
        a[jo] = mvn_nm_pair(P.epi, a[jo], fx_operand<EPI>(r.ea[it][jo], r.eu[it][jo]), r.nm, P.st, row_in, 2 * (j2 + jo * M));
        if (!KEEP) *reinterpret_cast<cfloat*>(P.out_real + i0 + 2 * jo * M) = a[jo];
      }
    }
    if constexpr (mvn_epi_base(EPI) == MVN_EPI_UPDATE_STATS) {
      const bool row_in = mvn_stat_row_in(P.st, r0 + rho);
#pragma unroll
      for (int jo = 0; jo < R; ++jo)
        a[jo] = mvn_update_pair_stats<mvn_epi_tv(EPI)>(P.epi, i0 + 2 * jo * M, a[jo], r.ea[it][jo], r.eb[it][jo], r.st, P.st, row_in,
                                      2 * (j2 + jo * M));
    }
    if (KEEP) {
#pragma unroll
      for (int jo = 0; jo < R; ++jo)
        if constexpr (mvn_epi_base(EPI) != MVN_EPI_UPDATE_STATS && !mvn_epi_nm(EPI))
          a[jo] = fx_epilogue_pair_value<EPI>(P.epi, i0 + 2 * jo * M, a[jo], fx_operand<EPI>(r.ea[it][jo], r.eu[it][jo]),
                                                            r.eb[it][jo]);
      dftR<R, -1>(a);
#pragma unroll
      for (int k = 1; k < R; ++k) a[k] = cmul(a[k], tw[k]);
#pragma unroll
      for (int k = 0; k < R; ++k) p[fx_rowoff<C::PAD, R, M>(k) * TP] = a[k];
    } else if constexpr (mvn_epi_base(EPI) != MVN_EPI_UPDATE_STATS && !mvn_epi_nm(EPI)) {
#pragma unroll
      for (int jo = 0; jo < R; ++jo)
        mvn_epilogue_pair_t<EPI>(P.epi, P.out_real, i0 + 2 * jo * M, a[jo], fx_operand<EPI>(r.ea[it][jo], r.eu[it][jo]),
                                               r.eb[it][jo]);
    }
  }
}

template <int H, int EPI, typename Ctx, bool LINES = false>
MVN_HD void fx_rows_c2r_r2c_body(const RowsParams& P, long tile, cfloat* lds, Ctx& ctx) {
  typedef FxRowsCfg<H> C;
  constexpr int T = C::T, TP = C::TP, NT = C::NT, NT_ = C::NT;
  (void)NT_;
  const long r0 = tile * T;
  cfloat* buf = lds;
  cfloat* tws = lds + C::TILE;
  cfloat* twr = tws + fx_twsize(H);
  MVN_PHASE(ctx, (fx_c2r_load<H, EPI, LINES>(P, r0, buf, tws, twr, r, tid)));
  MVN_PHASE(ctx, (fx_c2r_pre<H>(P, r0, buf, twr, tid)));
  fx_dit<H, T, TP, C::PAD, NT, +1, 1, C::TWT>(buf, tws, ctx);
  MVN_PHASE(ctx, (fx_c2r_stage0_epilogue<H, true, EPI>(P, r0, buf, tws, r, tid)));
  fx_dif<H, T, TP, C::PAD, NT, -1, 1, C::TWT>(buf, tws, ctx);
  MVN_PHASE(ctx, (fx_r2c_post<H>(P, r0, buf, twr, tid)));
  MVN_PHASE(ctx, (fx_r2c_store<H, LINES, fx_lines_wide<EPI>()>(P, r0, buf, tid)));
}

template <int H, int EPI, typename Ctx, bool LINES = false>
MVN_HD void fx_rows_c2r_body(const RowsParams& P, long tile, cfloat* lds, Ctx& ctx) {
  typedef FxRowsCfg<H> C;
  constexpr int T = C::T, TP = C::TP, NT = C::NT, NT_ = C::NT;
  (void)NT_;
  const long r0 = tile * T;
  cfloat* buf = lds;
  cfloat* tws = lds + C::TILE;
  cfloat* twr = tws + fx_twsize(H);
  MVN_PHASE(ctx, (fx_c2r_load<H, EPI, LINES>(P, r0, buf, tws, twr, r, tid)));
  MVN_PHASE(ctx, (fx_c2r_pre<H>(P, r0, buf, twr, tid)));
  fx_dit<H, T, TP, C::PAD, NT, +1, 1, C::TWT>(buf, tws, ctx);
  MVN_PHASE(ctx, (fx_c2r_stage0_epilogue<H, false, EPI>(P, r0, buf, tws, r, tid)));
}

template <int H, int KIND, int EPI, typename Ctx, bool LINES = false>
MVN_HD void fx_rows_tile(const RowsParams& P, long tile, cfloat* lds, Ctx& ctx) {
  if constexpr (KIND == 0)
    fx_rows_r2c_body<H, Ctx, LINES>(P, tile, lds, ctx);
  else if constexpr (KIND == 1)
    fx_rows_c2r_body<H, EPI, Ctx, LINES>(P, tile, lds, ctx);
  else
    fx_rows_c2r_r2c_body<H, EPI, Ctx, LINES>(P, tile, lds, ctx);
}

template <int H>
constexpr bool fx_rows_lines_ok() {
  return H == 256 && !FxRowsCfg<H>::WALK && FxRowsCfg<H>::T == 16 && FxRowsCfg<H>::EXACT;
}

template <int H, int KIND, int EPI, typename Ctx, bool LINES = false>
MVN_HD void fx_rows_run(const RowsParams& P, long block, long nblocks, cfloat* lds, Ctx& ctx) {
  if constexpr (LINES) {
    fx_rows_tile<H, KIND, EPI, Ctx, true>(P, block, lds, ctx);
    return;
  }
  typedef FxRowsCfg<H> C;
  if constexpr (C::WALK) {
    constexpr int NT_ = C::NT;
    (void)NT_;
    cfloat* tws = lds + C::TILE;
    cfloat* twr = tws + fx_twsize(H);
    MVN_PHASE(ctx, (fx_rows_tables<H>(P, tws, twr, tid)));
    const long ntiles = P.rows / C::T;
    for (long tile = block; tile < ntiles; tile += nblocks) fx_rows_tile<H, KIND, EPI>(P, tile, lds, ctx);
  } else {
    fx_rows_tile<H, KIND, EPI>(P, block, lds, ctx);
  }
}

template <int NT, typename Ctx>
MVN_HD void fx_stat_flush(const MvnStatsParams& s, long block, long nblocks, cfloat* lds, Ctx& ctx) {
  constexpr int NT_ = NT;
  (void)NT_;
  char* l = reinterpret_cast<char*>(lds);
  MVN_PHASE(ctx, (void)0);
  MVN_PHASE(ctx, (mvn_stat_put(l, NT, tid, r.st)));
  for (int h = mvn_pow2_ceil(NT) >> 1; h > 0; h >>= 1) {
    MVN_PHASE(ctx, (mvn_stat_tree_step(l, NT, h, tid)));
  }
  MVN_PHASE_NOSYNC(ctx, (tid == 0 ? mvn_stat_record(s, l, NT, block, nblocks) : (void)0));
}

template <int H, int KIND, typename Ctx, bool LINES = false, int EPI = MVN_EPI_UPDATE_STATS>
MVN_HD void fx_rows_run_stats(const RowsParams& P, long block, long nblocks, cfloat* lds, Ctx& ctx) {
  static_assert(mvn_stat_lds_bytes(FxRowsCfg<H>::NT) <= (long)sizeof(cfloat) * FxRowsCfg<H>::lds_cfloats,
                "statistics scratch exceeds the LDS");
  constexpr int NT_ = FxRowsCfg<H>::NT;
  (void)NT_;
  MVN_PHASE_NOSYNC(ctx, (mvn_stat_init(r.st)));
  fx_rows_run<H, KIND, EPI, Ctx, LINES>(P, block, nblocks, lds, ctx);
  fx_stat_flush<FxRowsCfg<H>::NT>(P.st, block, nblocks, lds, ctx);
}

template <int NT, typename Ctx>
MVN_HD void fx_nm_flush(const MvnStatsParams& s, long block, long nblocks, cfloat* lds, Ctx& ctx) {
  constexpr int NT_ = NT;
  (void)NT_;
  char* l = reinterpret_cast<char*>(lds);
  MVN_PHASE(ctx, (void)0);
  MVN_PHASE(ctx, (mvn_nm_put(l, NT, tid, r.nm)));
  for (int h = mvn_pow2_ceil(NT) >> 1; h > 0; h >>= 1) {
    MVN_PHASE(ctx, (mvn_nm_tree_step(l, NT, h, tid)));
  }
  MVN_PHASE_NOSYNC(ctx, (tid == 0 ? mvn_nm_record(s, l, NT, block, nblocks) : (void)0));
}

template <int H, int KIND, int EPI, typename Ctx, bool LINES = false>
MVN_HD void fx_rows_run_nm(const RowsParams& P, long block, long nblocks, cfloat* lds, Ctx& ctx) {
  static_assert(mvn_epi_nm(EPI), "a noise-model divide epilogue");
  static_assert(mvn_nm_lds_bytes(FxRowsCfg<H>::NT) <= (long)sizeof(cfloat) * FxRowsCfg<H>::lds_cfloats,
                "statistics scratch exceeds the LDS");
  constexpr int NT_ = FxRowsCfg<H>::NT;
  (void)NT_;
  MVN_PHASE_NOSYNC(ctx, (mvn_nm_init(r.nm)));
  fx_rows_run<H, KIND, EPI, Ctx, LINES>(P, block, nblocks, lds, ctx);
  fx_nm_flush<FxRowsCfg<H>::NT>(P.st, block, nblocks, lds, ctx);
}
```

libmultiviewnative_amd/csrc/mvn_kernels.hip:

```cpp
#include <hip/hip_runtime.h>

#include <atomic>
#include <cstdio>
#include <cstdlib>
#include <cstring>
#include <map>
#include <mutex>
#include <tuple>
#include <stdexcept>
#include <string>

#include "mvn_backend.hpp"
#include "mvn_fixed_geom.hpp"
#include "mvn_wave_rows.hpp"

#define HIP_CHECK(expr)                                                                      \
  do {                                                                                       \
    hipError_t _e = (expr);                                                                  \
    if (_e != hipSuccess)                                                                    \
      throw std::runtime_error(std::string("HIP error '") + hipGetErrorString(_e) + "' at " + \
                               __FILE__ + ":" + std::to_string(__LINE__) + " (" #expr ")");  \
  } while (0)

template <bool EVEN, int T>
// ... 328 lines not shown
  hipDeviceProp_t prop;
  HIP_CHECK(hipGetDeviceProperties(&prop, dev));
  std::memset(name256, 0, 256);
  std::strncpy(name256, prop.name, 255);
  if (!name256[0]) std::snprintf(name256, 256, "AMD GPU %s", prop.gcnArchName);
}

long long device_total_mem(int dev) {
  hipDeviceProp_t prop;
  HIP_CHECK(hipGetDeviceProperties(&prop, dev));
  return (long long)prop.totalGlobalMem;
}

void device_mem_info(size_t* free_b, size_t* total_b) { HIP_CHECK(hipMemGetInfo(free_b, total_b)); }

void device_arch(int dev, int* major, int* minor) {
  hipDeviceProp_t prop;
  HIP_CHECK(hipGetDeviceProperties(&prop, dev));
  const char* a = prop.gcnArchName;
  *major = 0;
  *minor = 0;
  if (std::strncmp(a, "gfx", 3) != 0) return;
  a += 3;
  size_t len = 0;
  while (a[len] && a[len] != ':') ++len;
  if (len == 0) return;
  for (size_t i = 0; i + 1 < len; ++i)
    if (a[i] >= '0' && a[i] <= '9') *major = *major * 10 + (a[i] - '0');
  const char c = a[len - 1];
  *minor = (c >= '0' && c <= '9') ? c - '0' : ((c >= 'a' && c <= 'f') ? 10 + c - 'a' : 0);
}

void* dmalloc(size_t bytes) {
  void* p = nullptr;
  HIP_CHECK(hipMalloc(&p, bytes ? bytes : 1));
  return p;
}

void dfree(void* p) {
  if (p) (void)hipFree(p);
}

static hipStream_t hs(stream_t s) { return (hipStream_t)s; }

void h2d(void* d, const void* h, size_t bytes, stream_t s) {
  HIP_CHECK(hipMemcpyAsync(d, h, bytes, hipMemcpyHostToDevice, hs(s)));
}
void d2h(void* h, const void* d, size_t bytes, stream_t s) {
  HIP_CHECK(hipMemcpyAsync(h, d, bytes, hipMemcpyDeviceToHost, hs(s)));
}
void d2d(void* dst, const void* src, size_t bytes, stream_t s) {
  HIP_CHECK(hipMemcpyAsync(dst, src, bytes, hipMemcpyDeviceToDevice, hs(s)));
}
void h2d_2d(void* d, size_t dpitch, const void* h, size_t hpitch, size_t width, size_t height,
            stream_t s) {
  if (dpitch == width && hpitch == width) return h2d(d, h, width * height, s);
  HIP_CHECK(hipMemcpy2DAsync(d, dpitch, h, hpitch, width, height, hipMemcpyHostToDevice, hs(s)));
}
void d2h_2d(void* h, size_t hpitch, const void* d, size_t dpitch, size_t width, size_t height,
            stream_t s) {
  if (dpitch == width && hpitch == width) return d2h(h, d, width * height, s);
  HIP_CHECK(hipMemcpy2DAsync(h, hpitch, d, dpitch, width, height, hipMemcpyDeviceToHost, hs(s)));
}
void d2d_2d(void* dst, size_t dpitch, const void* src, size_t spitch, size_t width, size_t height,
            stream_t s) {
  if (dpitch == width && spitch == width) return d2d(dst, src, width * height, s);
  HIP_CHECK(hipMemcpy2DAsync(dst, dpitch, src, spitch, width, height, hipMemcpyDeviceToDevice, hs(s)));
}
void dzero(void* d, size_t bytes, stream_t s) { HIP_CHECK(hipMemsetAsync(d, 0, bytes, hs(s))); }

void enable_peer_access(int dev, int peer) {
  if (dev == peer) return;
  int can = 0;
  HIP_CHECK(hipDeviceCanAccessPeer(&can, dev, peer));
  if (!can) throw std::runtime_error("mvn: device " + std::to_string(dev) + " cannot access device " + std::to_string(peer));
  int cur = 0;
  HIP_CHECK(hipGetDevice(&cur));
  HIP_CHECK(hipSetDevice(dev));
  const hipError_t e = hipDeviceEnablePeerAccess(peer, 0);
  (void)hipSetDevice(cur);
  if (e == hipErrorPeerAccessAlreadyEnabled) {
    (void)hipGetLastError();
    return;
  }
  HIP_CHECK(e);
}
void copy_peer(void* dst, int dst_dev, const void* src, int src_dev, size_t bytes, stream_t s) {
  if (dst_dev == src_dev)
    HIP_CHECK(hipMemcpyAsync(dst, src, bytes, hipMemcpyDeviceToDevice, hs(s)));
  else
    HIP_CHECK(hipMemcpyPeerAsync(dst, dst_dev, src, src_dev, bytes, hs(s)));
}

int pointer_device(const void* p) {
  hipPointerAttribute_t attr;
  std::memset(&attr, 0, sizeof(attr));
  const hipError_t e = hipPointerGetAttributes(&attr, p);
  if (e != hipSuccess) {
    (void)hipGetLastError();
    return POINTER_HOST;
  }
  switch (attr.type) {
    case hipMemoryTypeDevice: return attr.device;
    case hipMemoryTypeManaged: return POINTER_ANY;
    default: return POINTER_HOST;
  }
}

stream_t stream_create() {
  hipStream_t s;
  HIP_CHECK(hipStreamCreateWithFlags(&s, hipStreamNonBlocking));
  return (stream_t)s;
}
stream_t stream_create_upload() {
  int least = 0, greatest = 0;
  HIP_CHECK(hipDeviceGetStreamPriorityRange(&least, &greatest));
  hipStream_t s;
  HIP_CHECK(hipStreamCreateWithPriority(&s, hipStreamNonBlocking, greatest));
  return (stream_t)s;
}
void stream_destroy(stream_t s) {
  if (s) (void)hipStreamDestroy(hs(s));
}
void stream_sync(stream_t s) { HIP_CHECK(hipStreamSynchronize(hs(s))); }

void stream_wait_event(stream_t s, event_t e) {
  HIP_CHECK(hipStreamWaitEvent(hs(s), (hipEvent_t)e, 0));
}

event_t event_create() {
  hipEvent_t e;
  HIP_CHECK(hipEventCreate(&e));
  return (event_t)e;
}
event_t event_create_sync() {
  hipEvent_t e;
  HIP_CHECK(hipEventCreateWithFlags(&e, hipEventDisableTiming));
  return (event_t)e;
}
void event_destroy(event_t e) {
  if (e) (void)hipEventDestroy((hipEvent_t)e);
}
void event_record(event_t e, stream_t s) { HIP_CHECK(hipEventRecord((hipEvent_t)e, hs(s))); }
void event_sync(event_t e) { HIP_CHECK(hipEventSynchronize((hipEvent_t)e)); }
float event_elapsed_ms(event_t a, event_t b) {
  float ms = 0.f;
  HIP_CHECK(hipEventElapsedTime(&ms, (hipEvent_t)a, (hipEvent_t)b));
  return ms;
}

bool graphs_supported() { return true; }
void capture_begin(stream_t s) {
  HIP_CHECK(hipStreamBeginCapture(hs(s), hipStreamCaptureModeThreadLocal));
}
graph_exec_t capture_end(stream_t s) {
  hipGraph_t g = nullptr;
  HIP_CHECK(hipStreamEndCapture(hs(s), &g));
  hipGraphExec_t e = nullptr;
  hipError_t err = hipGraphInstantiate(&e, g, nullptr, nullptr, 0);
  (void)hipGraphDestroy(g);
  HIP_CHECK(err);
  return (graph_exec_t)e;
}
void graph_launch(graph_exec_t g, stream_t s) { HIP_CHECK(hipGraphLaunch((hipGraphExec_t)g, hs(s))); }
void graph_destroy(graph_exec_t g) {
  if (g) (void)hipGraphExecDestroy((hipGraphExec_t)g);
}

template <typename K>
static void ensure_lds(K kernel, size_t lds_bytes) {
  if (lds_bytes <= 64 * 1024) return;
  static std::mutex mu;
  static std::map<std::pair<const void*, int>, size_t> done;
  int dev = 0;
  HIP_CHECK(hipGetDevice(&dev));
  const void* fn = reinterpret_cast<const void*>(kernel);
  const auto key = std::make_pair(fn, dev);
  std::lock_guard<std::mutex> lk(mu);
  auto it = done.find(key);
  if (it != done.end() && it->second >= lds_bytes) return;
  HIP_CHECK(hipFuncSetAttribute(fn, hipFuncAttributeMaxDynamicSharedMemorySize, (int)lds_bytes));
  done[key] = lds_bytes;
}

static void check_launch(long nblocks, int nthreads, size_t lds_bytes) {
  if (nblocks < 1 || nblocks > 0x7fffffffL) throw std::invalid_argument("mvn: grid size out of range");
  if (nthreads < 64 || nthreads > 1024 || nthreads % 64) throw std::invalid_argument("mvn: bad block size");
  if (lds_bytes > 160 * 1024) throw std::invalid_argument("mvn: LDS request exceeds 160 KiB");
}

template <typename K, typename P>
static void launch_pass(K kernel, const P& p, long nblocks, int nthreads, size_t lds_bytes, stream_t s) {
  ensure_lds(kernel, lds_bytes);
  hipLaunchKernelGGL(kernel, dim3((unsigned)nblocks), dim3(nthreads), lds_bytes, hs(s), p);
  HIP_CHECK(hipGetLastError());
}

template <bool WALK, typename K>
static void launch_rows_fixed(K kernel, const RowsParams& p, long nblocks, int nthreads, size_t lds_bytes,
                              stream_t s);

static int current_device() {
  int dev = 0;
  HIP_CHECK(hipGetDevice(&dev));
  return dev;
}

static int device_cu_count() {
  static std::mutex mu;
  static std::map<int, int> cache;
  const int dev = current_device();
  std::lock_guard<std::mutex> lk(mu);
  auto it = cache.find(dev);
  if (it != cache.end()) return it->second;
  hipDeviceProp_t prop;
  HIP_CHECK(hipGetDeviceProperties(&prop, dev));
  const int cus = prop.multiProcessorCount > 0 ? prop.multiProcessorCount : 1;
  cache[dev] = cus;
  return cus;
}

static int resident_per_cu(const void* kernel, int nthreads, size_t lds_bytes) {
  static std::mutex mu;
  static std::map<std::tuple<int, const void*, int, size_t>, int> cache;
  const int dev = current_device();
  std::lock_guard<std::mutex> lk(mu);
  const auto key = std::make_tuple(dev, kernel, nthreads, lds_bytes);
  auto it = cache.find(key);
  if (it != cache.end()) return it->second;
  int per_cu = 0;
  HIP_CHECK(hipOccupancyMaxActiveBlocksPerMultiprocessor(&per_cu, kernel, nthreads, lds_bytes));
  if (per_cu < 1) per_cu = 1;
  cache[key] = per_cu;
  return per_cu;
}

template <typename K>
static void launch_walking(K kernel, StridedParams p, long nblocks, int nthreads, size_t lds_bytes,
                           stream_t s, bool walk, const StridedParams* rider = nullptr, size_t rider_lds = 0) {
  if (rider && rider_lds > lds_bytes) lds_bytes = rider_lds;
  ensure_lds(kernel, lds_bytes);
  long grid = nblocks;
  if (walk) {
    const long resident = (long)resident_per_cu(reinterpret_cast<const void*>(kernel), nthreads, lds_bytes) *
                          device_cu_count();
    if (grid > resident) grid = resident;
  }
  p.nblocks = nblocks;
  const long lines = rider ? rider->tiles_per_outer : 0;
  if (grid + lines > 0x7fffffffL) throw std::invalid_argument("mvn: grid size out of range");
  hipLaunchKernelGGL(kernel, dim3((unsigned)(grid + lines)), dim3(nthreads), lds_bytes, hs(s), p, rider ? *rider : p,
                     (unsigned)grid);
  HIP_CHECK(hipGetLastError());
}

static bool wave_rows_enabled(const RowsParams& p, int kind_bit) {
  static const int mask = [] {
    const char* e = std::getenv("MVN_WAVE_ROWS_MASK");
    return e && *e ? std::atoi(e) : 28;
  }();
  return (mask & kind_bit) && p.fixed && !p.lines && p.h == WrCfg::H && p.C == WrCfg::H;
}

template <typename K>
static void launch_wave_rows(K kernel, const RowsParams& p, stream_t s, long mult = 16) {
  const size_t lds = sizeof(cfloat) * (size_t)WrCfg::lds_cfloats;
  const long pairs = (p.rows + 1) / 2;
  long grid = (pairs + WrCfg::WAVES - 1) / WrCfg::WAVES;
  const long resident = (long)resident_per_cu(reinterpret_cast<const void*>(kernel), WrCfg::NT, lds) *
                        device_cu_count() * mult;
  if (grid > resident) grid = resident;
  hipLaunchKernelGGL(kernel, dim3((unsigned)grid), dim3(WrCfg::NT), lds, hs(s), p);
  HIP_CHECK(hipGetLastError());
}

template <bool WALK, typename K>
static void launch_rows_fixed(K kernel, const RowsParams& p, long nblocks, int nthreads, size_t lds_bytes,
                              stream_t s) {
  if (WALK) {
    ensure_lds(kernel, lds_bytes);
    const long resident = (long)resident_per_cu(reinterpret_cast<const void*>(kernel), nthreads, lds_bytes) *
                          device_cu_count() * 8;
    if (nblocks > resident) nblocks = resident;
  }
  launch_pass(kernel, p, nblocks, nthreads, lds_bytes, s);
}

#define MVN_DISPATCH_T(T_, KERNEL_EXPR)                                        \
  switch (T_) {                                                                \
    case 16: { constexpr int TT = 16; launch_pass(KERNEL_EXPR, p, nblocks, nthreads, lds_bytes, s); } break; \
    case 8: { constexpr int TT = 8; launch_pass(KERNEL_EXPR, p, nblocks, nthreads, lds_bytes, s); } break;   \
    case 4: { constexpr int TT = 4; launch_pass(KERNEL_EXPR, p, nblocks, nthreads, lds_bytes, s); } break;   \
    case 2: { constexpr int TT = 2; launch_pass(KERNEL_EXPR, p, nblocks, nthreads, lds_bytes, s); } break;   \
    case 1: { constexpr int TT = 1; launch_pass(KERNEL_EXPR, p, nblocks, nthreads, lds_bytes, s); } break;   \
    default: throw std::invalid_argument("mvn: unsupported tile width");       \
  }

static void check_aligned16(const void* p, const char* what) {
  if (((size_t)p) & 15) throw std::invalid_argument(std::string("mvn: fixed kernels need 16-byte aligned ") + what);
}

static void check_lines(const RowsParams& p, long nblocks) {
  constexpr int H = 256;
  if (!fx_rows_lines_ok<H>() || !p.fixed || p.h != H || p.C != H || !p.nyq_packed || p.lines_d1 < 1 ||
      p.lines_d1 % FxRowsCfg<H>::T || p.row_base % FxRowsCfg<H>::T || p.rows != nblocks * FxRowsCfg<H>::T)
    throw std::invalid_argument("mvn: line-layout last-axis pass outside its range");
}

void launch_rows_r2c(const RowsParams& p, bool even, long nblocks, int nthreads, size_t lds_bytes,
                     stream_t s) {
  check_launch(nblocks, nthreads, lds_bytes);
  if (p.lines) {
    check_lines(p, nblocks);
    return launch_pass(kx_rows_r2c<256, true>, p, nblocks, nthreads, lds_bytes, s);
  }
  if (p.fixed) {
    check_aligned16(p.in_real, "input");
    check_aligned16(p.out_cplx, "output");
    if (wave_rows_enabled(p, 1)) return launch_wave_rows(kw_rows<MVN_WR_R2C, MVN_EPI_STORE>, p, s);
    switch (p.h) {
#define X(H) case H: launch_rows_fixed<FxRowsCfg<H>::WALK>(kx_rows_r2c<H>, p, nblocks, nthreads, lds_bytes, s); return;
      MVN_FIXED_ROWS_LENGTHS(X)
#undef X
      default: throw std::invalid_argument("mvn: no fixed rows kernel for this length");
    }
  }
  if (even) {
    MVN_DISPATCH_T(p.T, (k_rows_r2c<true, TT>));
  } else {
    MVN_DISPATCH_T(p.T, (k_rows_r2c<false, TT>));
  }
}

void launch_rows_c2r(const RowsParams& p, bool even, long nblocks, int nthreads, size_t lds_bytes,
                     stream_t s) {
  check_launch(nblocks, nthreads, lds_bytes);
  if (p.lines) {
    check_lines(p, nblocks);
    switch (p.epi.mode) {
      case MVN_EPI_DIVIDE: return launch_pass(kx_rows_c2r<256, MVN_EPI_DIVIDE, true>, p, nblocks, nthreads, lds_bytes, s);
      case MVN_EPI_DIVIDE_U16: return launch_pass(kx_rows_c2r<256, MVN_EPI_DIVIDE_U16, true>, p, nblocks, nthreads, lds_bytes, s);
      case MVN_EPI_DIVIDE_NM: return launch_pass(kx_rows_c2r<256, MVN_EPI_DIVIDE_NM, true>, p, nblocks, nthreads, lds_bytes, s);
      case MVN_EPI_DIVIDE_NM_U16: return launch_pass(kx_rows_c2r<256, MVN_EPI_DIVIDE_NM_U16, true>, p, nblocks, nthreads, lds_bytes, s);
      case MVN_EPI_UPDATE: return launch_pass(kx_rows_c2r<256, MVN_EPI_UPDATE, true>, p, nblocks, nthreads, lds_bytes, s);
      case MVN_EPI_UPDATE_STATS: return launch_pass(kx_rows_c2r<256, MVN_EPI_UPDATE_STATS, true>, p, nblocks, nthreads, lds_bytes, s);
      case MVN_EPI_UPDATE_TV: return launch_pass(kx_rows_c2r<256, MVN_EPI_UPDATE_TV, true>, p, nblocks, nthreads, lds_bytes, s);
      case MVN_EPI_UPDATE_STATS_TV: return launch_pass(kx_rows_c2r<256, MVN_EPI_UPDATE_STATS_TV, true>, p, nblocks, nthreads, lds_bytes, s);
      case MVN_EPI_DELTA: return launch_pass(kx_rows_c2r<256, MVN_EPI_DELTA, true>, p, nblocks, nthreads, lds_bytes, s);
      default: return launch_pass(kx_rows_c2r<256, MVN_EPI_STORE, true>, p, nblocks, nthreads, lds_bytes, s);
    }
  }
  if (p.fixed) {
    check_aligned16(p.in_cplx, "input");
    check_aligned16(p.out_real, "output");
    if (wave_rows_enabled(p, p.epi.mode == MVN_EPI_DELTA ? 16 : 2)) {
      switch (p.epi.mode) {
        case MVN_EPI_DIVIDE: return launch_wave_rows(kw_rows<MVN_WR_C2R, MVN_EPI_DIVIDE>, p, s);
        case MVN_EPI_DIVIDE_U16: return launch_wave_rows(kw_rows<MVN_WR_C2R, MVN_EPI_DIVIDE_U16>, p, s);
        case MVN_EPI_DIVIDE_NM: return launch_wave_rows(kw_rows<MVN_WR_C2R, MVN_EPI_DIVIDE_NM>, p, s);
        case MVN_EPI_DIVIDE_NM_U16: return launch_wave_rows(kw_rows<MVN_WR_C2R, MVN_EPI_DIVIDE_NM_U16>, p, s);
        case MVN_EPI_UPDATE: return launch_wave_rows(kw_rows<MVN_WR_C2R, MVN_EPI_UPDATE>, p, s);
        case MVN_EPI_UPDATE_STATS: return launch_wave_rows(kw_rows<MVN_WR_C2R, MVN_EPI_UPDATE_STATS>, p, s);
        case MVN_EPI_UPDATE_TV: return launch_wave_rows(kw_rows<MVN_WR_C2R, MVN_EPI_UPDATE_TV>, p, s);
        case MVN_EPI_UPDATE_STATS_TV: return launch_wave_rows(kw_rows<MVN_WR_C2R, MVN_EPI_UPDATE_STATS_TV>, p, s);
        case MVN_EPI_DELTA: return launch_wave_rows(kw_rows<MVN_WR_C2R, MVN_EPI_DELTA>, p, s);
        default: return launch_wave_rows(kw_rows<MVN_WR_C2R, MVN_EPI_STORE>, p, s);
      }
    }
    switch (p.h) {
#define X(H)                                                                                  \
  case H:                                                                                     \
    switch (p.epi.mode) {                                                                     \
      case MVN_EPI_DIVIDE: launch_rows_fixed<FxRowsCfg<H>::WALK>(kx_rows_c2r<H, MVN_EPI_DIVIDE>, p, nblocks, nthreads, lds_bytes, s); break; \
      case MVN_EPI_DIVIDE_U16: launch_rows_fixed<FxRowsCfg<H>::WALK>(kx_rows_c2r<H, MVN_EPI_DIVIDE_U16>, p, nblocks, nthreads, lds_bytes, s); break; \
      case MVN_EPI_DIVIDE_NM: launch_rows_fixed<FxRowsCfg<H>::WALK>(kx_rows_c2r<H, MVN_EPI_DIVIDE_NM>, p, nblocks, nthreads, lds_bytes, s); break; \
      case MVN_EPI_DIVIDE_NM_U16: launch_rows_fixed<FxRowsCfg<H>::WALK>(kx_rows_c2r<H, MVN_EPI_DIVIDE_NM_U16>, p, nblocks, nthreads, lds_bytes, s); break; \
      case MVN_EPI_UPDATE: launch_rows_fixed<FxRowsCfg<H>::WALK>(kx_rows_c2r<H, MVN_EPI_UPDATE>, p, nblocks, nthreads, lds_bytes, s); break; \
      case MVN_EPI_UPDATE_STATS: launch_rows_fixed<FxRowsCfg<H>::WALK>(kx_rows_c2r<H, MVN_EPI_UPDATE_STATS>, p, nblocks, nthreads, lds_bytes, s); break; \
      case MVN_EPI_UPDATE_TV: launch_rows_fixed<FxRowsCfg<H>::WALK>(kx_rows_c2r<H, MVN_EPI_UPDATE_TV>, p, nblocks, nthreads, lds_bytes, s); break; \
      case MVN_EPI_UPDATE_STATS_TV: launch_rows_fixed<FxRowsCfg<H>::WALK>(kx_rows_c2r<H, MVN_EPI_UPDATE_STATS_TV>, p, nblocks, nthreads, lds_bytes, s); break; \
      case MVN_EPI_DELTA: launch_rows_fixed<FxRowsCfg<H>::WALK>(kx_rows_c2r<H, MVN_EPI_DELTA>, p, nblocks, nthreads, lds_bytes, s); break;   \
      default: launch_rows_fixed<FxRowsCfg<H>::WALK>(kx_rows_c2r<H, MVN_EPI_STORE>, p, nblocks, nthreads, lds_bytes, s); break;             \
    }                                                                                         \
    return;
      MVN_FIXED_ROWS_LENGTHS(X)
#undef X
      default: throw std::invalid_argument("mvn: no fixed rows kernel for this length");
    }
  }
  if (p.epi.mode == MVN_EPI_UPDATE_STATS) {
    lds_bytes = std::max(lds_bytes, (size_t)mvn_stat_lds_bytes(nthreads));
    if (even) {
      MVN_DISPATCH_T(p.T, (k_rows_c2r_stats<true, TT>));
    } else {
      MVN_DISPATCH_T(p.T, (k_rows_c2r_stats<false, TT>));
    }
    return;
  }
  if (mvn_epi_tv(p.epi.mode)) {
    const bool stats = p.epi.mode == MVN_EPI_UPDATE_STATS_TV;
    if (stats) lds_bytes = std::max(lds_bytes, (size_t)mvn_stat_lds_bytes(nthreads));
    if (even && stats) {
      MVN_DISPATCH_T(p.T, (k_rows_c2r_tv<true, TT, true>));
    } else if (even) {
      MVN_DISPATCH_T(p.T, (k_rows_c2r_tv<true, TT, false>));
    } else if (stats) {
      MVN_DISPATCH_T(p.T, (k_rows_c2r_tv<false, TT, true>));
    } else {
      MVN_DISPATCH_T(p.T, (k_rows_c2r_tv<false, TT, false>));
    }
    return;
  }
  if (mvn_epi_nm(p.epi.mode)) {
    lds_bytes = std::max(lds_bytes, (size_t)mvn_nm_lds_bytes(nthreads));
    const bool u16 = p.epi.mode == MVN_EPI_DIVIDE_NM_U16;
    if (even && u16) {
      MVN_DISPATCH_T(p.T, (k_rows_c2r_nm<true, TT, true>));
    } else if (even) {
      MVN_DISPATCH_T(p.T, (k_rows_c2r_nm<true, TT, false>));
    } else if (u16) {
      MVN_DISPATCH_T(p.T, (k_rows_c2r_nm<false, TT, true>));
    } else {
      MVN_DISPATCH_T(p.T, (k_rows_c2r_nm<false, TT, false>));
    }
    return;
  }
  if (p.epi.mode == MVN_EPI_DIVIDE_U16) {
    if (even) {
      MVN_DISPATCH_T(p.T, (k_rows_c2r_u16<true, TT>));
    } else {
      MVN_DISPATCH_T(p.T, (k_rows_c2r_u16<false, TT>));
    }
    return;
  }
  if (even) {
    MVN_DISPATCH_T(p.T, (k_rows_c2r<true, TT>));
  } else {
    MVN_DISPATCH_T(p.T, (k_rows_c2r<false, TT>));
  }
}

void launch_rows_c2r_r2c(const RowsParams& p, long nblocks, int nthreads, size_t lds_bytes,
                         stream_t s) {
  check_launch(nblocks, nthreads, lds_bytes);
  if (p.lines) {
    check_lines(p, nblocks);
    switch (p.epi.mode) {
      case MVN_EPI_DIVIDE: return launch_pass(kx_rows_c2r_r2c<256, MVN_EPI_DIVIDE, true>, p, nblocks, nthreads, lds_bytes, s);
      case MVN_EPI_DIVIDE_U16: return launch_pass(kx_rows_c2r_r2c<256, MVN_EPI_DIVIDE_U16, true>, p, nblocks, nthreads, lds_bytes, s);
      case MVN_EPI_DIVIDE_NM: return launch_pass(kx_rows_c2r_r2c<256, MVN_EPI_DIVIDE_NM, true>, p, nblocks, nthreads, lds_bytes, s);
      case MVN_EPI_DIVIDE_NM_U16: return launch_pass(kx_rows_c2r_r2c<256, MVN_EPI_DIVIDE_NM_U16, true>, p, nblocks, nthreads, lds_bytes, s);
      case MVN_EPI_UPDATE: return launch_pass(kx_rows_c2r_r2c<256, MVN_EPI_UPDATE, true>, p, nblocks, nthreads, lds_bytes, s);
      case MVN_EPI_UPDATE_STATS: return launch_pass(kx_rows_c2r_r2c<256, MVN_EPI_UPDATE_STATS, true>, p, nblocks, nthreads, lds_bytes, s);
      case MVN_EPI_UPDATE_TV: return launch_pass(kx_rows_c2r_r2c<256, MVN_EPI_UPDATE_TV, true>, p, nblocks, nthreads, lds_bytes, s);
      case MVN_EPI_UPDATE_STATS_TV: return launch_pass(kx_rows_c2r_r2c<256, MVN_EPI_UPDATE_STATS_TV, true>, p, nblocks, nthreads, lds_bytes, s);
      default: return launch_pass(kx_rows_c2r_r2c<256, MVN_EPI_STORE, true>, p, nblocks, nthreads, lds_bytes, s);
    }
  }
  if (!p.fixed) {
    if (p.epi.mode == MVN_EPI_UPDATE_STATS) {
      lds_bytes = std::max(lds_bytes, (size_t)mvn_stat_lds_bytes(nthreads));
      MVN_DISPATCH_T(p.T, (k_rows_c2r_r2c_stats<TT>));
      return;
    }
    if (p.epi.mode == MVN_EPI_UPDATE_STATS_TV) {
      lds_bytes = std::max(lds_bytes, (size_t)mvn_stat_lds_bytes(nthreads));
      MVN_DISPATCH_T(p.T, (k_rows_c2r_r2c_tv<TT, true>));
      return;
    }
    if (p.epi.mode == MVN_EPI_UPDATE_TV) {
      MVN_DISPATCH_T(p.T, (k_rows_c2r_r2c_tv<TT, false>));
      return;
    }
    if (mvn_epi_nm(p.epi.mode)) {
      lds_bytes = std::max(lds_bytes, (size_t)mvn_nm_lds_bytes(nthreads));
      if (p.epi.mode == MVN_EPI_DIVIDE_NM_U16) {
        MVN_DISPATCH_T(p.T, (k_rows_c2r_r2c_nm<TT, true>));
      } else {
        MVN_DISPATCH_T(p.T, (k_rows_c2r_r2c_nm<TT, false>));
      }
      return;
    }
    if (p.epi.mode == MVN_EPI_DIVIDE_U16) {
      MVN_DISPATCH_T(p.T, (k_rows_c2r_r2c_u16<TT>));
      return;
    }
    MVN_DISPATCH_T(p.T, (k_rows_c2r_r2c<TT>));
    return;
  }
  check_aligned16(p.in_cplx, "input");
  check_aligned16(p.out_cplx, "output");
  if (wave_rows_enabled(p, mvn_epi_divides(p.epi.mode) ? 4 : 8)) {
    switch (p.epi.mode) {
      case MVN_EPI_DIVIDE: return launch_wave_rows(kw_rows<MVN_WR_C2R_R2C, MVN_EPI_DIVIDE>, p, s);
      case MVN_EPI_DIVIDE_U16: return launch_wave_rows(kw_rows<MVN_WR_C2R_R2C, MVN_EPI_DIVIDE_U16>, p, s);
      case MVN_EPI_DIVIDE_NM: return launch_wave_rows(kw_rows<MVN_WR_C2R_R2C, MVN_EPI_DIVIDE_NM>, p, s);
      case MVN_EPI_DIVIDE_NM_U16: return launch_wave_rows(kw_rows<MVN_WR_C2R_R2C, MVN_EPI_DIVIDE_NM_U16>, p, s);
      case MVN_EPI_UPDATE: return launch_wave_rows(kw_rows<MVN_WR_C2R_R2C, MVN_EPI_UPDATE>, p, s, 32);
      case MVN_EPI_UPDATE_STATS: return launch_wave_rows(kw_rows<MVN_WR_C2R_R2C, MVN_EPI_UPDATE_STATS>, p, s, 32);
      case MVN_EPI_UPDATE_TV: return launch_wave_rows(kw_rows<MVN_WR_C2R_R2C, MVN_EPI_UPDATE_TV>, p, s, 32);
      case MVN_EPI_UPDATE_STATS_TV: return launch_wave_rows(kw_rows<MVN_WR_C2R_R2C, MVN_EPI_UPDATE_STATS_TV>, p, s, 32);
      default: return launch_wave_rows(kw_rows<MVN_WR_C2R_R2C, MVN_EPI_STORE>, p, s);
    }
  }
  switch (p.h) {
#define X(H)                                                                                  \
  case H:                                                                                     \
    switch (p.epi.mode) {                                                                     \
      case MVN_EPI_DIVIDE: launch_rows_fixed<FxRowsCfg<H>::WALK>(kx_rows_c2r_r2c<H, MVN_EPI_DIVIDE>, p, nblocks, nthreads, lds_bytes, s); break; \
      case MVN_EPI_DIVIDE_U16: launch_rows_fixed<FxRowsCfg<H>::WALK>(kx_rows_c2r_r2c<H, MVN_EPI_DIVIDE_U16>, p, nblocks, nthreads, lds_bytes, s); break; \
      case MVN_EPI_DIVIDE_NM: launch_rows_fixed<FxRowsCfg<H>::WALK>(kx_rows_c2r_r2c<H, MVN_EPI_DIVIDE_NM>, p, nblocks, nthreads, lds_bytes, s); break; \
      case MVN_EPI_DIVIDE_NM_U16: launch_rows_fixed<FxRowsCfg<H>::WALK>(kx_rows_c2r_r2c<H, MVN_EPI_DIVIDE_NM_U16>, p, nblocks, nthreads, lds_bytes, s); break; \
      case MVN_EPI_UPDATE: launch_rows_fixed<FxRowsCfg<H>::WALK>(kx_rows_c2r_r2c<H, MVN_EPI_UPDATE>, p, nblocks, nthreads, lds_bytes, s); break; \
      case MVN_EPI_UPDATE_STATS: launch_rows_fixed<FxRowsCfg<H>::WALK>(kx_rows_c2r_r2c<H, MVN_EPI_UPDATE_STATS>, p, nblocks, nthreads, lds_bytes, s); break; \
      case MVN_EPI_UPDATE_TV: launch_rows_fixed<FxRowsCfg<H>::WALK>(kx_rows_c2r_r2c<H, MVN_EPI_UPDATE_TV>, p, nblocks, nthreads, lds_bytes, s); break; \
      case MVN_EPI_UPDATE_STATS_TV: launch_rows_fixed<FxRowsCfg<H>::WALK>(kx_rows_c2r_r2c<H, MVN_EPI_UPDATE_STATS_TV>, p, nblocks, nthreads, lds_bytes, s); break; \
      default: launch_rows_fixed<FxRowsCfg<H>::WALK>(kx_rows_c2r_r2c<H, MVN_EPI_STORE>, p, nblocks, nthreads, lds_bytes, s); break;             \
    }                                                                                         \
    return;
    MVN_FIXED_ROWS_LENGTHS(X)
#undef X
    default: throw std::invalid_argument("mvn: no fixed rows kernel for this length");
  }
}

void launch_convergence_reduce(const double* rec, const unsigned* counts, int nviews, long cap, double* out,
                               stream_t s) {
  hipLaunchKernelGGL(k_convergence_reduce, dim3(1), dim3(256), 0, hs(s), rec, counts, nviews, cap, out);
  HIP_CHECK(hipGetLastError());
}

void launch_nm_reduce(const double* rec, const unsigned* counts, int nviews, long cap, double* out, stream_t s) {
  hipLaunchKernelGGL(k_nm_reduce, dim3((unsigned)nviews), dim3(256), 0, hs(s), rec, counts, cap, out);
  HIP_CHECK(hipGetLastError());
}

static std::atomic<long> g_split_launches{0};
long split_launch_count() { return g_split_launches.load(); }
static std::atomic<long> g_mid_fused_launches{0};
long mid_fused_launch_count() { return g_mid_fused_launches.load(); }

template <int N>
static bool try_launch_split(int mode, const StridedParams& p, long nblocks, stream_t s, const StridedParams* rider,
                             size_t rider_lds) {
  if constexpr (FxSplitCfg<N>::USE) {
    typedef FxSplitCfg<N> C;
    if (mode == MVN_ST_FWD_MUL_INV || p.cstride != 1 || p.ncols % C::T != 0 || p.tiles_per_outer < 1)
      return false;
    StridedParams q = p;
    const long outer = nblocks / p.tiles_per_outer;
    q.tiles_per_outer = p.ncols / C::T;
    q.T = q.TP = C::T;
    const long nb = outer * q.tiles_per_outer;
    const size_t lds = sizeof(cfloat) * (size_t)C::lds_cfloats;
    ++g_split_launches;
    if (mode == MVN_ST_FWD)
      launch_walking(kx_strided_split<N, MVN_ST_FWD>, q, nb, C::NT, lds, s, true, rider, rider_lds);
    else
      launch_walking(kx_strided_split<N, MVN_ST_INV>, q, nb, C::NT, lds, s, true, rider, rider_lds);
    return true;
  } else {
    (void)mode; (void)p; (void)nblocks; (void)s; (void)rider; (void)rider_lds;
    return false;
  }
}

void launch_strided(int mode, const StridedParams& p, long nblocks, int nthreads,
                    size_t lds_bytes, stream_t s, const StridedParams* rider, size_t rider_lds) {
  check_launch(nblocks, nthreads, lds_bytes);
  if (rider && (!p.fixed || mode == MVN_ST_FWD_MUL_INV || rider->T != 1 || rider->fixed || rider_lds > 160 * 1024))
    throw std::invalid_argument("mvn: Nyquist lines ride only in the plain fixed-length strided passes, one per workgroup");
  if (p.fixed) {
    check_aligned16(p.data, "data");
    if (mode == MVN_ST_FWD_MUL_INV) check_aligned16(p.spec, "spectrum");
    switch (p.ax.n) {
#define X(N)                                                                                       \
  case N:                                                                                          \
    if (try_launch_split<N>(mode, p, nblocks, s, rider, rider_lds)) return;                        \
    if (mode == MVN_ST_FWD) launch_walking(kx_strided<N, MVN_ST_FWD>, p, nblocks, FxStridedSel<N, MVN_ST_FWD>::NT, lds_bytes, s, true, rider, rider_lds); \
    else if (mode == MVN_ST_INV) launch_walking(kx_strided<N, MVN_ST_INV>, p, nblocks, FxStridedSel<N, MVN_ST_INV>::NT, lds_bytes, s, true, rider, rider_lds); \
    else launch_walking(kx_strided<N, MVN_ST_FWD_MUL_INV>, p, nblocks, FxStridedSel<N, MVN_ST_FWD_MUL_INV>::NT, lds_bytes, s, !FxStridedSel<N, MVN_ST_FWD_MUL_INV>::LDS_FUSED); \
    return;
      MVN_FIXED_STRIDED_LENGTHS(X)
#undef X
      default: throw std::invalid_argument("mvn: no fixed strided kernel for this length");
    }
  }
  if (p.is_nyq) {
    switch (mode) {
      case MVN_ST_FWD: MVN_DISPATCH_T(p.T, (k_strided<MVN_ST_FWD, TT, true>)); break;
      case MVN_ST_INV: MVN_DISPATCH_T(p.T, (k_strided<MVN_ST_INV, TT, true>)); break;
      case MVN_ST_FWD_MUL_INV: MVN_DISPATCH_T(p.T, (k_strided<MVN_ST_FWD_MUL_INV, TT, true>)); break;
      default: throw std::invalid_argument("mvn: unknown strided mode");
    }
    return;
  }
  switch (mode) {
    case MVN_ST_FWD: MVN_DISPATCH_T(p.T, (k_strided<MVN_ST_FWD, TT, false>)); break;
    case MVN_ST_INV: MVN_DISPATCH_T(p.T, (k_strided<MVN_ST_INV, TT, false>)); break;
    case MVN_ST_FWD_MUL_INV: MVN_DISPATCH_T(p.T, (k_strided<MVN_ST_FWD_MUL_INV, TT, false>)); break;
    default: throw std::invalid_argument("mvn: unknown strided mode");
  }
}

void launch_dim0_direct(const Dim0DirectParams& p, stream_t s) {
  if (!mvn_dim0_direct_possible(p.k, p.d0) || p.kd < p.k + 1 || p.h != p.k / 2 || p.plane < 0 || p.plane + p.plane2 < 1 || (p.plane > 0 && p.in == p.out) ||
      p.plane2 < 0 || (p.plane2 > 0 && (!p.in2 || !p.out2 || !p.taps2 || p.in2 == p.out2)))
    throw std::invalid_argument("mvn: direct dim0 convolution called outside its range");
// ... 240 lines not shown
```

libmultiviewnative_amd/csrc/mvn_mid_fused.hpp:

```cpp
#pragma once

#include <stdexcept>

#include "mvn_dim0_direct.hpp"
#include "mvn_wave_rows.hpp"

#if defined(__HIPCC__) && !defined(MVN_HOST_EMU)
#define MF_WPHASE(ctx, ...)                                         \
  {                                                                 \
    const int tid = (ctx).tid;                                      \
    auto& r = (ctx).regs;                                           \
    (void)r;                                                        \
    __VA_ARGS__;                                                    \
  }                                                                 \
  __builtin_amdgcn_fence(__ATOMIC_SEQ_CST, "wavefront", "local");   \
  __builtin_amdgcn_wave_barrier();
#else
#define MF_WPHASE(ctx, ...) MVN_PHASE(ctx, __VA_ARGS__)
#endif

#define MF_N1 512
#define MF_NT 512
#define MF_LINES 8
#define MF_PITCH 576
#define MF_BUF (MF_LINES * MF_PITCH)
#define MF_TWL 512
#define MF_LDS_CFLOATS (4 * MF_BUF + MF_TWL)

struct MidFusedParams {
  const cfloat* in;
  cfloat* out;
  const cfloat* taps;
  int kd;
  const cfloat* tw;
  int d0, H;
  int k, h;
  int seg;
  int mode;
  int packed;
  int zbeg, zcount;
  unsigned* poison;
  unsigned poison_epoch;
  int n_peers;
  unsigned* const* poison_peers;
};
enum { MF_CONV = 0, MF_TAPS = 1 };
enum { MF_DC_NONE = 0, MF_DC_LOW = 1, MF_DC_HIGH = 2, MF_DC_SELF = 3 };

constexpr int mf_slots(int K) { return (K + 7) / 8 * 8; }

template <int K>
struct MfRegs {
  cfloat tap[K];
  cfloat w[mf_slots(K)];
  cfloat xr[8];
  cfloat t[8];
  cfloat bad;
  cfloat t2[8];
  cfloat xn[2], xp[2];
  int dcmode, qm, cpar;
};

inline long mf_pieces(const MidFusedParams& P) { return (P.seg > 0 && P.zcount <= 0) ? (P.d0 + P.seg - 1) / P.seg : 1; }
inline long mf_blocks(const MidFusedParams& P) { return P.mode == MF_TAPS ? (long)P.H * ((P.d0 + MF_LINES - 1) / MF_LINES) : (long)P.H * mf_pieces(P); }

MVN_HD void mf_job(const MidFusedParams& P, long block, int& c, int& z0, int& nout) {
  const long piece = block / P.H;
  c = (int)(block - piece * P.H);
  if (P.zcount > 0) {
    z0 = P.zbeg;
    nout = P.zcount;
  } else if (P.seg > 0) {
    z0 = (int)(piece * P.seg);
    nout = P.d0 - z0 < P.seg ? P.d0 - z0 : P.seg;
  } else {
    z0 = 0;
    nout = P.d0;
  }
}

MVN_HD int mf_tap_plane(const MidFusedParams& P, int j) {
  const int p = j - P.h;
  return p < 0 ? p + P.kd : p;
}

inline void mf_check(const MidFusedParams& P) {
  const bool taps_mode = P.mode == MF_TAPS;
  if (!P.in || !P.out || !P.tw || P.d0 < 1 || P.H < 1 || (long)P.d0 * P.H * MF_N1 >= (1L << 31) * 4 || P.seg < 0)
    throw std::invalid_argument("mvn: fused middle pass: bad arguments");
  if (P.zcount < 0 || P.zbeg < 0 || P.zbeg + P.zcount > P.d0 || P.n_peers < 0 || P.n_peers > MVN_D0_MAX_PEERS ||
      (P.n_peers > 0 && !P.poison_peers))
    throw std::invalid_argument("mvn: fused middle pass: bad plane range or peers");
  if (!taps_mode && (!P.taps || P.in == P.out || P.k < 1 || mvn_dim0_taps_template(P.k) > 31 || P.h != P.k / 2 || P.kd < P.k))
    throw std::invalid_argument("mvn: fused middle pass called outside its range");
}

MVN_HD int mf_in_plane(const MidFusedParams& P, int z0, int n) {
  int z = (z0 - P.h + n) % P.d0;
  return z < 0 ? z + P.d0 : z;
}

template <int K>
MVN_HD void mf_fetch(const MidFusedParams& P, MfRegs<K>& r, int c, int z0, int batch, int nsteps, int tid) {
  const int wv = tid >> 6, l = tid & 63;
  const int n = batch * MF_LINES + wv;
  if (n >= nsteps) return;
  const cfloat* src = P.in + ((long)mf_in_plane(P, z0, n) * P.H + c) * MF_N1 + l;
#pragma unroll
  for (int m = 0; m < 8; ++m) r.xr[m] = src[64 * m];
}

template <int K>
MVN_HD void mf_setup(const MidFusedParams& P, MfRegs<K>& r, int c, int z0, int nsteps, int tid) {
  r.bad = cmake(0.f, 0.f);
  r.dcmode = MF_DC_NONE;
  r.qm = r.cpar = 0;
#pragma unroll
  for (int j = 0; j < K; ++j) r.tap[j] = j < P.k ? P.taps[((long)mf_tap_plane(P, j) * P.H + c) * MF_N1 + tid] : cmake(0.f, 0.f);
#pragma unroll
  for (int s = 0; s < mf_slots(K); ++s) r.w[s] = cmake(0.f, 0.f);
  mf_fetch<K>(P, r, c, z0, 0, nsteps, tid);
}

MVN_HD cfloat mf_cmul(cfloat a, cfloat w) {
#if defined(MVN_PACKED)
  cfloat t, r;
  MVN_PK2(t, "v_pk_mul_f32", a, w, "op_sel_hi:[0,1]");
  MVN_PK3(r, "v_pk_fma_f32", a, w, t, "op_sel:[1,1,0] op_sel_hi:[1,0,1] neg_lo:[0,1,0]");
  return r;
#else
  return cmul(a, w);
#endif
}
MVN_HD cfloat mf_cmulc(cfloat a, cfloat w) {
#if defined(MVN_PACKED)
  cfloat t, r;
  MVN_PK2(t, "v_pk_mul_f32", a, w, "op_sel_hi:[0,1] neg_hi:[0,1]");
  MVN_PK3(r, "v_pk_fma_f32", a, w, t, "op_sel:[1,1,0] op_sel_hi:[1,0,1]");
  return r;
#else
  return cmulc(a, w);
#endif
}

MVN_HD void mf_build_twiddles(const MidFusedParams& P, cfloat* twl, int tid) {
  if (tid < 448) {
    const int m = tid / 64 + 1, l = tid & 63;
    twl[tid] = P.tw[l * m];
  } else if (tid < 448 + 56) {
    const int e = tid - 448, m = e / 8 + 1, j = e & 7;
    twl[tid] = P.tw[8 * j * m];
  }
}
MVN_HD cfloat mf_tw0(const cfloat* twl, int l, int m) { return twl[(m - 1) * 64 + l]; }
MVN_HD cfloat mf_tw1(const cfloat* twl, int l, int m) { return twl[448 + (m - 1) * 8 + (l & 7)]; }

template <int K>
MVN_HD void mf_fwd0(MfRegs<K>& r, cfloat* buf, int tid) {
  const int wv = tid >> 6, l = tid & 63;
  cfloat* line = buf + wv * MF_PITCH;
  cfloat a[8];
#pragma unroll
  for (int m = 0; m < 8; ++m) a[m] = r.xr[m];
  dftR<8, -1>(a);
#pragma unroll
  for (int m = 1; m < 8; ++m) a[m] = mf_cmul(a[m], r.t2[m]);
#pragma unroll
  for (int m = 0; m < 8; ++m) line[72 * m + l] = a[m];
}
template <int K>
MVN_HD void mf_tw0_ahead(MfRegs<K>& r, const cfloat* twl, int tid) {
  const int l = tid & 63;
#pragma unroll
  for (int m = 1; m < 8; ++m) r.t2[m] = mf_tw0(twl, l, m);
}
template <int K>
MVN_HD void mf_fwd1_r(MfRegs<K>& r, const cfloat* buf, int tid) {
  const int wv = tid >> 6, l = tid & 63;
  const cfloat* p = buf + wv * MF_PITCH + 72 * (l >> 3) + (l & 7);
#pragma unroll
  for (int m = 0; m < 8; ++m) r.t[m] = p[8 * m];
}
template <int K>
MVN_HD void mf_fwd1_c(MfRegs<K>& r, const cfloat* twl, int tid) {
  const int l = tid & 63;
  (void)l;
  dftR<8, -1>(r.t);
#pragma unroll
  for (int m = 1; m < 8; ++m) r.t[m] = mf_cmul(r.t[m], mf_tw1(twl, l, m));
}
template <int K>
MVN_HD void mf_fwd1_r2(MfRegs<K>& r, const cfloat* buf, int tid) {
  const int wv = tid >> 6, l = tid & 63;
  const cfloat* p = buf + wv * MF_PITCH + 72 * (l >> 3) + (l & 7);
#pragma unroll
  for (int m = 0; m < 8; ++m) r.t2[m] = p[8 * m];
}
template <int K>
MVN_HD void mf_fwd1_c2(MfRegs<K>& r, const cfloat* twl, int tid) {
  const int l = tid & 63;
  (void)l;
  dftR<8, -1>(r.t2);
#pragma unroll
  for (int m = 1; m < 8; ++m) r.t2[m] = mf_cmul(r.t2[m], mf_tw1(twl, l, m));
}
template <int K>
MVN_HD void mf_fwd1_b2(const MfRegs<K>& r, cfloat* buf, int tid) {
  const int wv = tid >> 6, l = tid & 63;
  cfloat* p = buf + wv * MF_PITCH + 72 * (l >> 3) + (l & 7);
#pragma unroll
  for (int m = 0; m < 8; ++m) p[9 * m] = r.t2[m];
}
template <int K>
MVN_HD void mf_fwd2_r2(MfRegs<K>& r, const cfloat* buf, int tid) {
  const int wv = tid >> 6, l = tid & 63;
  const cfloat* p = buf + wv * MF_PITCH + 72 * (l >> 3) + 9 * (l & 7);
#pragma unroll
  for (int m = 0; m < 8; ++m) r.t2[m] = p[m];
}
template <int K>
MVN_HD void mf_fwd2_b2(const MfRegs<K>& r, cfloat* buf, int tid) {
  const int wv = tid >> 6, l = tid & 63;
  cfloat* line = buf + wv * MF_PITCH;
#pragma unroll
  for (int m = 0; m < 8; ++m) line[64 * m + l] = r.t2[m];
}
template <int K>
MVN_HD void mf_fwd1_a(MfRegs<K>& r, const cfloat* buf, const cfloat* twl, int tid) {
  mf_fwd1_r<K>(r, buf, tid);
  mf_fwd1_c<K>(r, twl, tid);
}
template <int K>
MVN_HD void mf_fwd1_b(const MfRegs<K>& r, cfloat* buf, int tid) {
  const int wv = tid >> 6, l = tid & 63;
  cfloat* p = buf + wv * MF_PITCH + 72 * (l >> 3) + (l & 7);
#pragma unroll
  for (int m = 0; m < 8; ++m) p[9 * m] = r.t[m];
}
template <int K>
MVN_HD void mf_fwd2_r(MfRegs<K>& r, const cfloat* buf, int tid) {
  const int wv = tid >> 6, l = tid & 63;
  const cfloat* p = buf + wv * MF_PITCH + 72 * (l >> 3) + 9 * (l & 7);
#pragma unroll
  for (int m = 0; m < 8; ++m) r.t[m] = p[m];
}
template <int K>
MVN_HD void mf_fwd2_a(MfRegs<K>& r, const cfloat* buf, int tid) {
  mf_fwd2_r<K>(r, buf, tid);
  dftR<8, -1>(r.t);
}
template <int K>
MVN_HD void mf_fwd2_b(const MfRegs<K>& r, cfloat* buf, int tid) {
  const int wv = tid >> 6, l = tid & 63;
  cfloat* line = buf + wv * MF_PITCH;
#pragma unroll
  for (int m = 0; m < 8; ++m) line[64 * m + l] = r.t[m];
}

template <int K>
MVN_HD void mf_inv2_r(MfRegs<K>& r, const cfloat* buf, int tid) {
  const int wv = tid >> 6, l = tid & 63;
  const cfloat* line = buf + wv * MF_PITCH;
#pragma unroll
  for (int m = 0; m < 8; ++m) r.t[m] = line[64 * m + l];
}
template <int K>
MVN_HD void mf_inv2_a(MfRegs<K>& r, const cfloat* buf, int tid) {
  mf_inv2_r<K>(r, buf, tid);
  dftR<8, +1>(r.t);
}
template <int K>
MVN_HD void mf_inv2_b(const MfRegs<K>& r, cfloat* buf, int tid) {
  const int wv = tid >> 6, l = tid & 63;
  cfloat* p = buf + wv * MF_PITCH + 72 * (l >> 3) + 9 * (l & 7);
#pragma unroll
  for (int m = 0; m < 8; ++m) p[m] = r.t[m];
}
template <int K>
MVN_HD void mf_inv1_r(MfRegs<K>& r, const cfloat* buf, int tid) {
  const int wv = tid >> 6, l = tid & 63;
  const cfloat* p = buf + wv * MF_PITCH + 72 * (l >> 3) + (l & 7);
#pragma unroll
  for (int m = 0; m < 8; ++m) r.t[m] = p[9 * m];
}
template <int K>
MVN_HD void mf_inv1_c(MfRegs<K>& r, const cfloat* twl, int tid) {
  const int l = tid & 63;
  (void)l;
#pragma unroll
  for (int m = 1; m < 8; ++m) r.t[m] = mf_cmulc(r.t[m], mf_tw1(twl, l, m));
  dftR<8, +1>(r.t);
}
template <int K>
MVN_HD void mf_inv1_a(MfRegs<K>& r, const cfloat* buf, const cfloat* twl, int tid) {
  mf_inv1_r<K>(r, buf, tid);
  mf_inv1_c<K>(r, twl, tid);
}
template <int K>
MVN_HD void mf_inv1_b(const MfRegs<K>& r, cfloat* buf, int tid) {
  const int wv = tid >> 6, l = tid & 63;
  cfloat* p = buf + wv * MF_PITCH + 72 * (l >> 3) + (l & 7);
#pragma unroll
  for (int m = 0; m < 8; ++m) p[8 * m] = r.t[m];
}
template <int K>
MVN_HD void mf_inv0_r(MfRegs<K>& r, const cfloat* buf, int tid) {
  const int wv = tid >> 6, l = tid & 63;
  const cfloat* line = buf + wv * MF_PITCH;
#pragma unroll
  for (int m = 0; m < 8; ++m) r.t[m] = line[72 * m + l];
}
template <int K>
MVN_HD void mf_inv0_c_store(MfRegs<K>& r, const cfloat* twl, cfloat* dst, int tid) {
  const int l = tid & 63;
#pragma unroll
  for (int m = 1; m < 8; ++m) r.t[m] = mf_cmulc(r.t[m], mf_tw0(twl, l, m));
  dftR<8, +1>(r.t);
#pragma unroll
  for (int m = 0; m < 8; ++m) dst[l + 64 * m] = r.t[m];
}
template <int K>
MVN_HD void mf_inv0_store(MfRegs<K>& r, const cfloat* buf, const cfloat* twl, cfloat* dst, int tid) {
  mf_inv0_r<K>(r, buf, tid);
  mf_inv0_c_store<K>(r, twl, dst, tid);
}

template <int K>
MVN_HD void mf_store_line(const MidFusedParams& P, MfRegs<K>& r, const cfloat* buf, const cfloat* twl, int c, int z0,
                          int nout, int batch, int tid) {
  const int m = batch * MF_LINES + (tid >> 6) - (K - 1);
  if (m < 0 || m >= nout) return;
  int z = z0 + m;
  z = z >= P.d0 ? z - P.d0 : z;
  mf_inv0_store<K>(r, buf, twl, P.out + ((long)z * P.H + c) * MF_N1, tid);
}
template <int K>
MVN_HD void mf_store_line_c(const MidFusedParams& P, MfRegs<K>& r, const cfloat* twl, int c, int z0, int nout, int batch,
                            int tid) {
  const int m = batch * MF_LINES + (tid >> 6) - (K - 1);
  if (m < 0 || m >= nout) return;
  int z = z0 + m;
  z = z >= P.d0 ? z - P.d0 : z;
  mf_inv0_c_store<K>(r, twl, P.out + ((long)z * P.H + c) * MF_N1, tid);
}

MVN_HD int mf_bin_of(int f) { return 64 * (f >> 6) + 8 * (f & 7) + ((f >> 3) & 7); }
MVN_HD int mf_freq_of(int q) { return ((q >> 3) & 7) + 8 * (q & 7) + 64 * (q >> 6); }
MVN_HD cfloat mf_herm0(cfloat a, cfloat b) { return cmake(0.5f * (a.x + b.x), 0.5f * (a.y - b.y)); }
MVN_HD cfloat mf_hermh(cfloat a, cfloat b) { return cmake(0.5f * (a.y + b.y), 0.5f * (b.x - a.x)); }


template <int K>
MVN_HD void mf_setup_dc(const MidFusedParams& P, MfRegs<K>& r, int tid) {
  const int f = mf_freq_of(tid), fm = (MF_N1 - f) & (MF_N1 - 1);
  r.qm = mf_bin_of(fm);
  r.dcmode = f == fm ? MF_DC_SELF : (f < MF_N1 / 2 ? MF_DC_LOW : MF_DC_HIGH);
  {
    const int l = tid & 63, g = (l >> 3) + 8 * (l & 7);
    r.cpar = g == 0 ? 64 : 8 * ((64 - g) & 7) + ((64 - g) >> 3);
  }
  const cfloat* tp = P.taps + r.qm;
#pragma unroll
  for (int j = 0; j < K; ++j) {
    const cfloat a = r.tap[j], b = j < P.k ? tp[(long)mf_tap_plane(P, j) * P.H * MF_N1] : cmake(0.f, 0.f);
    r.tap[j] = f == fm ? a : (f < MF_N1 / 2 ? mf_herm0(a, b) : mf_hermh(b, a));
  }
}

template <int K>
MVN_HD void mf_fread(MfRegs<K>& r, const cfloat* in, int c, bool dc, int tid) {
  r.xn[c & 1] = in[c * MF_PITCH + tid];
  if (dc) r.xp[c & 1] = in[c * MF_PITCH + r.qm];
}
template <int K>
MVN_HD cfloat mf_filter_input(MfRegs<K>& r, int c, bool dc) {
  cfloat x = r.xn[c & 1];
  if (dc) {
    const cfloat xp = r.xp[c & 1];
    const cfloat lo = mf_herm0(x, xp), hi = mf_hermh(xp, x);
    x = r.dcmode == MF_DC_LOW ? lo : (r.dcmode == MF_DC_HIGH ? hi : x);
  }
  return x;
}
template <int K, int U, int C, bool FILL>
MVN_HD void mf_filter_line(MfRegs<K>& r, const cfloat* in, cfloat* out, bool dc, int tid) {
  constexpr int KW = mf_slots(K), S = 8 * U + C;
  if (FILL) {
    r.w[S] = mf_filter_input<K>(r, C, dc);
    return;
  }
  constexpr int NC = K < 4 ? K : 4;
  cfloat a1[NC], a2[NC];
#pragma unroll
  for (int j = K - 1; j >= 1; --j) {
    const int ch = j % NC;
    const bool first = j + NC > K - 1;
    if (first)
      mvn_cmul2(a1[ch], a2[ch], r.w[(S - j + 2 * KW) % KW], r.tap[j]);
    else
      mvn_cmac2(a1[ch], a2[ch], r.w[(S - j + 2 * KW) % KW], r.tap[j]);
  }
  const cfloat x = mf_filter_input<K>(r, C, dc);
  if (K <= NC)
    mvn_cmul2(a1[0], a2[0], x, r.tap[0]);
  else
    mvn_cmac2(a1[0], a2[0], x, r.tap[0]);
  cfloat s1 = a1[0], s2 = a2[0];
#pragma unroll
  for (int ch = 1; ch < NC; ++ch) {
    s1 = cadd(s1, a1[ch]);
    s2 = cadd(s2, a2[ch]);
  }
  r.w[S] = x;
  r.bad = mvn_dim0_track(r.bad, x);
  cfloat o = cadd_i<+1>(s1, s2);
  if (dc) o = r.dcmode == MF_DC_SELF ? cmake(s1.x, s2.y) : o;
  out[C * MF_PITCH + tid] = o;
}
template <int K, int C>
MVN_HD void mf_fread_ahead(MfRegs<K>& r, const cfloat* in, bool dc, int tid) {
  if (C + 1 < MF_LINES) mf_fread<K>(r, in, C + 1, dc, tid);
}
template <int K, int C, int U>
MVN_HD void mf_fline_dispatch(MfRegs<K>& r, const cfloat* in, cfloat* out, int u, bool fill, bool dc, int tid) {
  if (u == U) {
    if (fill)
      mf_filter_line<K, U, C, true>(r, in, out, dc, tid);
    else
      mf_filter_line<K, U, C, false>(r, in, out, dc, tid);
    return;
  }
  if constexpr (U + 1 < mf_slots(K) / 8) mf_fline_dispatch<K, C, U + 1>(r, in, out, u, fill, dc, tid);
}

template <int K>
MVN_HD void mf_inv2_fix_dc(MfRegs<K>& r, const cfloat* buf, int tid) {
  const int wv = tid >> 6, l = tid & 63;
  const cfloat* line = buf + wv * MF_PITCH;
#pragma unroll
  for (int m = 0; m < 8; ++m) {
    const cfloat o = r.t[m];
    const cfloat p = line[(64 * (7 - m) + r.cpar) & (MF_N1 - 1)];
    const cfloat low = cmake(o.x - p.y, o.y + p.x), high = cmake(p.x + o.y, o.x - p.y);
    cfloat v = m < 4 ? low : high;
    if (m == 0 || m == 4) v = l == 0 ? o : v;
    r.t[m] = v;
  }
}
template <int K>
MVN_HD void mf_inv2_r_dc(MfRegs<K>& r, const cfloat* buf, int tid) {
  mf_inv2_r<K>(r, buf, tid);
  mf_inv2_fix_dc<K>(r, buf, tid);
}

template <int K>
MVN_HD void mf_report(const MidFusedParams& P, const MfRegs<K>& r) {
  if (r.bad.x != 0.f || r.bad.y != 0.f) {
    if (P.poison) *P.poison = P.poison_epoch;
    for (int i = 0; i < P.n_peers; ++i) *P.poison_peers[i] = P.poison_epoch;
  }
}

template <int K, typename Ctx>
MVN_HD void mf_body(const MidFusedParams& P, long block, cfloat* lds, Ctx& ctx) {
  constexpr int NT_ = MF_NT;
  (void)NT_;
  int c, z0, nout;
  mf_job(P, block, c, z0, nout);
  const int nsteps = nout + K - 1;
  const int nb = (nsteps + MF_LINES - 1) / MF_LINES;
  const bool dc = P.packed && c == 0;
  cfloat* twl = lds + 4 * MF_BUF;
  MVN_PHASE_NOSYNC(ctx, (mf_setup<K>(P, r, c, z0, nsteps, tid), mf_build_twiddles(P, twl, tid)));
  if (dc) {
    MVN_PHASE_NOSYNC(ctx, (mf_setup_dc<K>(P, r, tid)));
  }
  MVN_PHASE(ctx, (void)0);
  MVN_PHASE_NOSYNC(ctx, (mf_tw0_ahead<K>(r, twl, tid)));
#if defined(__HIPCC__) && !defined(MVN_HOST_EMU)
  const int wave_young = mvn_uniform((ctx.tid >> 8) & 1);
#define MF_PRIO_RESET() __builtin_amdgcn_s_setprio(0);
#define MF_PRIO_RAISE_YOUNG() \
  if (wave_young != 0) __builtin_amdgcn_s_setprio(2);
#else
#define MF_PRIO_RESET()
#define MF_PRIO_RAISE_YOUNG()
#endif
  for (int i = -1; i <= nb; ++i) {
    const cfloat* fin = lds + (i & 1) * MF_BUF;
    cfloat* fout = lds + (2 + (i & 1)) * MF_BUF;
    cfloat* fwd = lds + ((i + 1) & 1) * MF_BUF;
    cfloat* inv = lds + (2 + ((i + 1) & 1)) * MF_BUF;
    const bool F = i >= 0 && i < nb;
    const bool fill = i * MF_LINES + MF_LINES - 1 < K - 1;
    const int u = F ? i % (mf_slots(K) / 8) : 0;
#define MF_FLINE(C)                                                                \
  if (F) {                                                                         \
    MF_WPHASE(ctx, (mf_fread_ahead<K, C>(r, fin, dc, tid), mf_fline_dispatch<K, C, 0>(r, fin, fout, u, fill, dc, tid)));  \
  }
    MF_PRIO_RESET()
    if (F) {
      MF_WPHASE(ctx, (mf_fread<K>(r, fin, 0, dc, tid)));
    }
    MF_WPHASE(ctx, (mf_inv2_r<K>(r, inv, tid)));
    if (dc) {
      MF_WPHASE(ctx, (mf_inv2_fix_dc<K>(r, inv, tid)));
    }
    MF_WPHASE(ctx, (mf_fwd0<K>(r, fwd, tid), mf_fetch<K>(P, r, c, z0, i + 2, nsteps, tid)));
    MF_FLINE(0)
    MF_WPHASE(ctx, (dftR<8, +1>(r.t), mf_inv2_b<K>(r, inv, tid)));
    MF_WPHASE(ctx, (mf_inv1_r<K>(r, inv, tid)));
    MF_WPHASE(ctx, (mf_fwd1_r2<K>(r, fwd, tid)));
    MF_FLINE(1)
    MF_FLINE(2)
    MF_PRIO_RAISE_YOUNG()
    MF_WPHASE(ctx, (mf_inv1_c<K>(r, twl, tid), mf_inv1_b<K>(r, inv, tid)));
    MF_WPHASE(ctx, (mf_fwd1_c2<K>(r, twl, tid), mf_fwd1_b2<K>(r, fwd, tid)));
    MF_WPHASE(ctx, (mf_inv0_r<K>(r, inv, tid)));
    MF_WPHASE(ctx, (mf_fwd2_r2<K>(r, fwd, tid)));
    MF_FLINE(3)
    MF_FLINE(4)
    MF_WPHASE(ctx, (mf_store_line_c<K>(P, r, twl, c, z0, nout, i - 1, tid)));
    MF_WPHASE(ctx, (dftR<8, -1>(r.t2), mf_fwd2_b2<K>(r, fwd, tid)));
    MF_FLINE(5)
    MF_FLINE(6)
    MF_FLINE(7)
#undef MF_FLINE
    MF_WPHASE(ctx, (mf_tw0_ahead<K>(r, twl, tid)));
    MVN_PHASE(ctx, (void)0);
  }
#undef MF_PRIO_RESET
#undef MF_PRIO_RAISE_YOUNG
  MVN_PHASE_NOSYNC(ctx, (mf_report<K>(P, r)));
}

MVN_HD void mf_taps_load(const MidFusedParams& P, MfRegs<1>& r, long batch, int c, int tid) {
  const int l = tid & 63, z = (int)batch * MF_LINES + (tid >> 6);
  if (z >= P.d0) return;
  const cfloat* src = P.in + ((long)z * P.H + c) * MF_N1 + l;
#pragma unroll
  for (int m = 0; m < 8; ++m) r.xr[m] = src[64 * m];
}
MVN_HD void mf_taps_store(const MidFusedParams& P, const cfloat* lds, long batch, int c, int tid) {
  const int l = tid & 63, wv = tid >> 6, z = (int)batch * MF_LINES + wv;
  if (z >= P.d0) return;
  cfloat* dst = P.out + ((long)z * P.H + c) * MF_N1 + l;
#pragma unroll
  for (int m = 0; m < 8; ++m) dst[64 * m] = lds[wv * MF_PITCH + 64 * m + l];
}
template <typename Ctx>
MVN_HD void mf_taps_body(const MidFusedParams& P, long block, cfloat* lds, Ctx& ctx) {
  constexpr int NT_ = MF_NT;
  (void)NT_;
  const long batch = block / P.H;
  const int c = (int)(block - batch * P.H);
  cfloat* twl = lds + 4 * MF_BUF;
  MVN_PHASE(ctx, (mf_taps_load(P, r, batch, c, tid), mf_build_twiddles(P, twl, tid)));
  MF_WPHASE(ctx, (mf_tw0_ahead<1>(r, twl, tid)));
  MF_WPHASE(ctx, (mf_fwd0<1>(r, lds, tid)));
  MF_WPHASE(ctx, (mf_fwd1_a<1>(r, lds, twl, tid)));
  MF_WPHASE(ctx, (mf_fwd1_b<1>(r, lds, tid)));
  MF_WPHASE(ctx, (mf_fwd2_a<1>(r, lds, tid)));
  MF_WPHASE(ctx, (mf_fwd2_b<1>(r, lds, tid)));
  MVN_PHASE_NOSYNC(ctx, (mf_taps_store(P, lds, batch, c, tid)));
}
```

libmultiviewnative_amd/csrc/mvn_pass_bodies.hpp:

```cpp
#pragma once

#include <math.h>

#include "mvn_fft_core.hpp"

#if defined(__clang__)
#define MVN_FP_EXACT _Pragma("clang fp contract(off)")
#else
#define MVN_FP_EXACT
#endif

enum MvnEpilogue {
  MVN_EPI_STORE = 0,
  MVN_EPI_DIVIDE = 1,
  MVN_EPI_UPDATE = 2,
  MVN_EPI_DELTA = 3,
  MVN_EPI_UPDATE_STATS = 4,
  MVN_EPI_DIVIDE_U16 = 5,
  MVN_EPI_UPDATE_TV = 6,
  MVN_EPI_UPDATE_STATS_TV = 7,
  MVN_EPI_DIVIDE_NM = 8,
  MVN_EPI_DIVIDE_NM_U16 = 9
};

// ... 191 lines not shown

MVN_HD float mvn_blend(float w, float next, float last) {
  MVN_FP_EXACT
  return w * (next - last) + last;
}

struct MvnStatsParams {
  long row0;
  int d1;
  int o0, o1, o2;
  unsigned n0, n1, n2;
  double* rec;
  unsigned* count;
  long cap;
};

struct MvnStatAcc {
  double sum, mass;
  float max;
};

MVN_HD void mvn_stat_init(MvnStatAcc& a) {
  a.sum = 0.;
  a.mass = 0.;
  a.max = 0.f;
}

MVN_HD bool mvn_stat_row_in(const MvnStatsParams& s, long row) {
  const unsigned g = (unsigned)(s.row0 + row), d1 = (unsigned)s.d1;
  const unsigned z = g / d1, y = g - z * d1;
  return z - (unsigned)s.o0 < s.n0 && y - (unsigned)s.o1 < s.n1;
}

MVN_HD float mvn_stat_max(float m, float d) { return (d > m || d != d) ? d : m; }

MVN_HD void mvn_stat_add(MvnStatAcc& a, bool in, float last, float y, float x) {
  MVN_FP_EXACT
  const float d = fabsf(y - last) + (x - x);
  a.sum += in ? (double)d : 0.;
  a.mass += in ? (double)y : 0.;
  a.max = in ? mvn_stat_max(a.max, d) : a.max;
}

template <bool TV = false>
MVN_HD cfloat mvn_update_pair_stats(const EpilogueParams& e, long i, cfloat z, cfloat a, cfloat b, MvnStatAcc& acc,
                                    const MvnStatsParams& s, bool row_in, int col) {
  MVN_FP_EXACT
  float x0 = z.x * e.scale, x1 = z.y * e.scale;
  if constexpr (TV) {
    const cfloat t = mvn_tv_pair<TV>(e, i);
    x0 *= t.x, x1 *= t.y;
  }
  const float n0 = mvn_next_value(a.x, x0, e.lambda, e.lambda_inv, e.min_value);
  const float n1 = mvn_next_value(a.y, x1, e.lambda, e.lambda_inv, e.min_value);
  const cfloat y = cmake(mvn_blend(b.x, n0, a.x), mvn_blend(b.y, n1, a.y));
  *reinterpret_cast<cfloat*>(e.psi + i) = y;
  const unsigned c = (unsigned)(col - s.o2);
  mvn_stat_add(acc, row_in && c < s.n2, a.x, y.x, x0);
  mvn_stat_add(acc, row_in && c + 1u < s.n2, a.y, y.y, x1);
  return y;
}

template <bool TV = false>
MVN_HD void mvn_update_stats(const EpilogueParams& e, long i, float x, MvnStatAcc& acc, bool in) {
  MVN_FP_EXACT
  x *= e.scale;
  if constexpr (TV) x *= mvn_tv_one<TV>(e, i);
  const float last = e.psi[i];
  const float next = mvn_next_value(last, x, e.lambda, e.lambda_inv, e.min_value);
  const float y = e.weights[i] * (next - last) + last;
  e.psi[i] = y;
  mvn_stat_add(acc, in, last, y, x);
}

MVN_HD constexpr long mvn_stat_lds_bytes(int nthreads) { return 20L * nthreads; }

MVN_HD void mvn_stat_tree_step(char* lds, int n, int h, int tid) {
  double* ls = reinterpret_cast<double*>(lds);
  double* lm = ls + n;
  float* lx = reinterpret_cast<float*>(lm + n);
  if (tid < h && tid + h < n) {
    ls[tid] += ls[tid + h];
    lm[tid] += lm[tid + h];
    lx[tid] = mvn_stat_max(lx[tid], lx[tid + h]);
  }
}
MVN_HD void mvn_stat_put(char* lds, int n, int tid, const MvnStatAcc& a) {
  double* ls = reinterpret_cast<double*>(lds);
  ls[tid] = a.sum;
  ls[n + tid] = a.mass;
  reinterpret_cast<float*>(ls + 2 * n)[tid] = a.max;
}
MVN_HD void mvn_stat_record(const MvnStatsParams& s, const char* lds, int n, long block, long nblocks) {
  const double* ls = reinterpret_cast<const double*>(lds);
  if (block < s.cap) {
    s.rec[3 * block] = ls[0];
    s.rec[3 * block + 1] = (double)reinterpret_cast<const float*>(ls + 2 * n)[0];
    s.rec[3 * block + 2] = ls[n];
  }
  if (block == 0) *s.count = (unsigned)nblocks;
}
MVN_HD int mvn_pow2_ceil(int n) {
  int p = 1;
  while (p < n) p <<= 1;
  return p;
}

MVN_HD void mvn_stat_flush(const MvnStatsParams& s, const MvnStatAcc& a, long block, long nblocks, cfloat* lds,
                           int tid, int nthreads) {
  char* l = reinterpret_cast<char*>(lds);
  MVN_SYNC();
  for (int t = tid; t < nthreads; t += nthreads) mvn_stat_put(l, nthreads, t, a);
  MVN_SYNC();
  for (int h = mvn_pow2_ceil(nthreads) >> 1; h > 0; h >>= 1) {
    for (int t = tid; t < h; t += nthreads) mvn_stat_tree_step(l, nthreads, h, t);
    MVN_SYNC();
  }
  if (tid == 0) mvn_stat_record(s, l, nthreads, block, nblocks);
}

MVN_HD void mvn_convergence_reduce_body(const double* rec, const unsigned* counts, int nviews, long cap,
                                        double* out, double* lds, int tid, int nthreads) {
  for (int t = tid; t < nthreads; t += nthreads) {
    double s = 0., m = 0., p = 0.;
    for (int v = 0; v < nviews; ++v) {
      const long n = (long)counts[v] < cap ? (long)counts[v] : cap;
      const double* r = rec + 3 * (long)v * cap;
      for (long i = t; i < n; i += nthreads) {
        s += r[3 * i];
        m = (r[3 * i + 1] > m || r[3 * i + 1] != r[3 * i + 1]) ? r[3 * i + 1] : m;
        p += r[3 * i + 2];
      }
    }
    lds[t] = s;
    lds[nthreads + t] = m;
    lds[2 * nthreads + t] = p;
  }
  MVN_SYNC();
  for (int h = mvn_pow2_ceil(nthreads) >> 1; h > 0; h >>= 1) {
    for (int t = tid; t < h; t += nthreads) {
      if (t + h < nthreads) {
        lds[t] += lds[t + h];
        const double a = lds[nthreads + t], b = lds[nthreads + t + h];
        lds[nthreads + t] = (b > a || b != b) ? b : a;
        lds[2 * nthreads + t] += lds[2 * nthreads + t + h];
      }
    }
    MVN_SYNC();
  }
  if (tid == 0) {
    out[0] = lds[0];
    out[1] = lds[nthreads];
    out[2] = lds[2 * nthreads];
  }
}

struct MvnNmAcc {
  double d, y, m;
};

MVN_HD void mvn_nm_init(MvnNmAcc& a) {
  a.d = 0.;
  a.y = 0.;
  a.m = 0.;
}

MVN_HD float mvn_nm_one(const EpilogueParams& e, float y, float x, MvnNmAcc& a, bool in) {
  MVN_FP_EXACT
  const float m = e.background != 0.f ? x + e.background : x;
  const float q = mvn_quotient_g(y, m, e.guard_zero_view);
  const float term = y > 0.f ? (y * logf(q) - y) + m : m - y;
  a.d += in ? (double)term : 0.;
  a.y += in ? (double)y : 0.;
  a.m += in ? (double)m : 0.;
  return q;
}

MVN_HD cfloat mvn_nm_pair(const EpilogueParams& e, cfloat z, cfloat a, MvnNmAcc& acc, const MvnStatsParams& s,
                          bool row_in, int col) {
  MVN_FP_EXACT
  const float x0 = z.x * e.scale, x1 = z.y * e.scale;
  const unsigned c = (unsigned)(col - s.o2);
  const float q0 = mvn_nm_one(e, a.x, x0, acc, row_in && c < s.n2);
  const float q1 = mvn_nm_one(e, a.y, x1, acc, row_in && c + 1u < s.n2);
  return cmake(q0, q1);
}

MVN_HD constexpr long mvn_nm_lds_bytes(int nthreads) { return 24L * nthreads; }

MVN_HD void mvn_nm_put(char* lds, int n, int tid, const MvnNmAcc& a) {
  double* l = reinterpret_cast<double*>(lds);
  l[tid] = a.d;
  l[n + tid] = a.y;
  l[2 * n + tid] = a.m;
}
MVN_HD void mvn_nm_tree_step(char* lds, int n, int h, int tid) {
  double* l = reinterpret_cast<double*>(lds);
  if (tid < h && tid + h < n) {
    l[tid] += l[tid + h];
    l[n + tid] += l[n + tid + h];
    l[2 * n + tid] += l[2 * n + tid + h];
  }
}
MVN_HD void mvn_nm_record(const MvnStatsParams& s, const char* lds, int n, long block, long nblocks) {
  const double* l = reinterpret_cast<const double*>(lds);
  if (block < s.cap) {
    s.rec[3 * block] = l[0];
    s.rec[3 * block + 1] = l[n];
    s.rec[3 * block + 2] = l[2 * n];
  }
  if (block == 0) *s.count = (unsigned)nblocks;
}

MVN_HD void mvn_nm_flush(const MvnStatsParams& s, const MvnNmAcc& a, long block, long nblocks, cfloat* lds, int tid,
                         int nthreads) {
  char* l = reinterpret_cast<char*>(lds);
  MVN_SYNC();
  for (int t = tid; t < nthreads; t += nthreads) mvn_nm_put(l, nthreads, t, a);
  MVN_SYNC();
  for (int h = mvn_pow2_ceil(nthreads) >> 1; h > 0; h >>= 1) {
    for (int t = tid; t < h; t += nthreads) mvn_nm_tree_step(l, nthreads, h, t);
    MVN_SYNC();
  }
  if (tid == 0) mvn_nm_record(s, l, nthreads, block, nblocks);
}

MVN_HD void mvn_nm_reduce_body(const double* rec, const unsigned* count, long cap, double* out, double* lds, int tid,
                               int nthreads) {
  for (int t = tid; t < nthreads; t += nthreads) {
    double d = 0., y = 0., m = 0.;
    const long n = (long)*count < cap ? (long)*count : cap;
    for (long i = t; i < n; i += nthreads) {
      d += rec[3 * i];
      y += rec[3 * i + 1];
      m += rec[3 * i + 2];
    }
    lds[t] = d;
    lds[nthreads + t] = y;
    lds[2 * nthreads + t] = m;
  }
  MVN_SYNC();
  for (int h = mvn_pow2_ceil(nthreads) >> 1; h > 0; h >>= 1) {
    for (int t = tid; t < h; t += nthreads) mvn_nm_tree_step(reinterpret_cast<char*>(lds), nthreads, h, t);
    MVN_SYNC();
  }
  if (tid == 0) {
    out[0] = lds[0];
    out[1] = lds[nthreads];
    out[2] = lds[2 * nthreads];
  }
}

template <bool TV = false>
MVN_HD cfloat mvn_epilogue_pair_value(int mode, const EpilogueParams& e, long i, cfloat z, cfloat a,
                                      cfloat b) {
  MVN_FP_EXACT
  float x0 = z.x * e.scale, x1 = z.y * e.scale;
  if constexpr (TV) {
    const cfloat t = mvn_tv_pair<TV>(e, i);
    x0 *= t.x, x1 *= t.y;
  }
  if (mode == MVN_EPI_DIVIDE)
    return cmake(mvn_quotient_g(a.x, x0, e.guard_zero_view), mvn_quotient_g(a.y, x1, e.guard_zero_view));
  if (mode == MVN_EPI_UPDATE) {
    const float n0 = mvn_next_value(a.x, x0, e.lambda, e.lambda_inv, e.min_value);
    const float n1 = mvn_next_value(a.y, x1, e.lambda, e.lambda_inv, e.min_value);
    const cfloat y = cmake(mvn_blend(b.x, n0, a.x), mvn_blend(b.y, n1, a.y));
    *reinterpret_cast<cfloat*>(e.psi + i) = y;
    return y;
  }
  return cmake(x0, x1);
}

template <int EPI>
MVN_HD void mvn_epilogue_pair_t(const EpilogueParams& e, float* out, long i, cfloat z, cfloat a,
                                cfloat b) {
  EpilogueParams ee = e;
  ee.mode = mvn_epi_math(EPI);
  mvn_epilogue_pair<mvn_epi_tv(EPI)>(ee, out, i, z, a, b);
}

#define MVN_ROWS_U 8

struct RowsParams {
  AxisPlan ax;
  const cfloat* twr;
  int d2, h, C, RP;
  long rows;
  int T, TP;
  long lds_alt;
  long lds_tw;
  unsigned hmul, Cmul;
  int fixed;
  const float* in_real;
  cfloat* out_cplx;
  cfloat* out_nyq;
  const cfloat* in_cplx;
  const cfloat* in_nyq;
  float* out_real;
  EpilogueParams epi;
  int nyq_packed;
  int lines, lines_d1;
  long row_base;
  MvnStatsParams st;
};

template <int T>
MVN_HD unsigned mvn_stat_tile_rows(const RowsParams& P, long r0) {
  static_assert(T <= 32, "one bit per row");
  unsigned bits = 0;
  for (int rho = 0; rho < T; ++rho)
    if (r0 + rho < P.rows && mvn_stat_row_in(P.st, r0 + rho)) bits |= 1u << rho;
  return bits;
}

template <int T>
MVN_HD void rows_r2c_even_tail(const RowsParams& P, long r0, cfloat*& buf, cfloat*& alt,
                               const cfloat* tw, int tid, int nthreads) {
  const int h = P.h, TP = P.TP;
  lds_fft_dif<-1, T>(buf, alt, TP, P.ax, tw, tid, nthreads);
  const int npairs = h / 2 + 1;
  for (int w = tid; w < npairs * T; w += nthreads) {
    const int k = w / T, rho = w - k * T;
    const int m = (h - k) % h;
    const int pk = P.ax.inv[k], pm = P.ax.inv[m];
    const cfloat zk = buf[pk * TP + rho];
    if (k == 0) {
      if (P.nyq_packed) {
        buf[pk * TP + rho] = cmake(zk.x + zk.y, zk.x - zk.y);
      } else {
        buf[pk * TP + rho] = cmake(zk.x + zk.y, 0.f);
        if (r0 + rho < P.rows) P.out_nyq[r0 + rho] = cmake(zk.x - zk.y, 0.f);
      }
    } else {
      const cfloat zm = buf[pm * TP + rho];
      const cfloat E = cmake(0.5f * (zk.x + zm.x), 0.5f * (zk.y - zm.y));
      const cfloat D = cmake(0.5f * (zk.x - zm.x), 0.5f * (zk.y + zm.y));
      const cfloat G = cmul(P.twr[k], D);
      buf[pk * TP + rho] = cadd(E, cmul_si<-1>(G));
      if (m != k) buf[pm * TP + rho] = cadd(cconj(E), cmul_si<-1>(cconj(G)));
    }
  }
  MVN_SYNC();
  for (int w = tid; w < T * h; w += nthreads) {
    const int rho = (int)mvn_fastdiv((unsigned)w, (unsigned)h, P.hmul), p = w - rho * h;
    const long row = r0 + rho;
    if (row < P.rows) P.out_cplx[row * P.C + p] = buf[p * TP + rho];
  }
}

template <int T>
MVN_HD void rows_r2c_even_body(const RowsParams& P, long tile, int tid, int nthreads, cfloat* lds) {
  const int h = P.h, TP = P.TP;
  const long r0 = tile * T;
  cfloat* buf = lds;
  cfloat* alt = lds + P.lds_alt;
  const cfloat* tw = lds_stage_twiddles(lds + P.lds_tw, P.ax, tid, nthreads);
  constexpr int U = MVN_ROWS_U;
  const int total = T * h;
  const long last_row = P.rows - 1;
  for (int w0 = tid; w0 < total; w0 += U * nthreads) {
    cfloat v[U];
#pragma unroll
    for (int u = 0; u < U; ++u) {
      int w = w0 + u * nthreads;
      w = w < total ? w : total - 1;
      const int rho = (int)mvn_fastdiv((unsigned)w, (unsigned)h, P.hmul), j = w - rho * h;
      long row = r0 + rho;
      row = row < last_row ? row : last_row;
      v[u] = reinterpret_cast<const cfloat*>(P.in_real + row * P.RP)[j];
    }
#pragma unroll
    for (int u = 0; u < U; ++u) {
      const int w = w0 + u * nthreads;
      if (w < total) {
        const int rho = (int)mvn_fastdiv((unsigned)w, (unsigned)h, P.hmul), j = w - rho * h;
        buf[j * TP + rho] = (r0 + rho <= last_row) ? v[u] : cmake(0.f, 0.f);
      }
    }
  }
  MVN_SYNC();
  rows_r2c_even_tail<T>(P, r0, buf, alt, tw, tid, nthreads);
}

template <int T, bool KEEP = false, bool STATS = false, bool U16 = false, bool TV = false, bool NM = false>
MVN_HD void rows_c2r_even_body(const RowsParams& P, long tile, int tid, int nthreads, cfloat* lds) {
  EpilogueParams epi = P.epi;
  mvn_arm_poison(epi);
  MvnStatAcc acc;
  unsigned rin = 0;
  if constexpr (STATS) {
    epi.mode = MVN_EPI_UPDATE;
    mvn_stat_init(acc);
    rin = mvn_stat_tile_rows<T>(P, tile * T);
  }
  if constexpr (U16) epi.mode = MVN_EPI_DIVIDE;
  if constexpr (TV) epi.mode = MVN_EPI_UPDATE;
  MvnNmAcc nacc;
  if constexpr (NM) {
    epi.mode = MVN_EPI_DIVIDE;
    mvn_nm_init(nacc);
    rin = mvn_stat_tile_rows<T>(P, tile * T);
  }
  constexpr int U = MVN_ROWS_U;
  const int h = P.h, TP = P.TP;
  const long r0 = tile * T;
  const int total = T * h;
  const bool single = total <= U * nthreads;
  cfloat* buf = lds;
  cfloat* alt = lds + P.lds_alt;
  const cfloat* tw = lds_stage_twiddles(lds + P.lds_tw, P.ax, tid, nthreads);
  cfloat ea[U], eb[U];
  unsigned eu[U];
#pragma unroll
  for (int u = 0; u < U; ++u) {
    ea[u] = cmake(0.f, 0.f);
    eb[u] = cmake(0.f, 0.f);
    eu[u] = 0u;
  }
  const long last_row = P.rows - 1;
  for (int w0 = tid; w0 < total; w0 += U * nthreads) {
    cfloat v[U];
    long idx[U];
#pragma unroll
    for (int u = 0; u < U; ++u) {
      int w = w0 + u * nthreads;
      w = w < total ? w : total - 1;
      const int rho = (int)mvn_fastdiv((unsigned)w, (unsigned)h, P.hmul), k = w - rho * h;
      long row = r0 + rho;
      row = row < last_row ? row : last_row;
      v[u] = P.in_cplx[row * P.C + k];
      idx[u] = row * P.RP + 2 * k;
    }
    if (single) {
      if constexpr (U16)
        mvn_epilogue_fetch_batch_u16<U>(epi, idx, eu);
      else
        mvn_epilogue_fetch_batch<U>(epi, idx, ea, eb);
    }
#pragma unroll
    for (int u = 0; u < U; ++u) {
      const int w = w0 + u * nthreads;
      if (w < total) {
        const int rho = (int)mvn_fastdiv((unsigned)w, (unsigned)h, P.hmul), p = w - rho * h;
        buf[p * TP + rho] = (r0 + rho <= last_row) ? v[u] : cmake(0.f, 0.f);
      }
    }
  }
  MVN_SYNC();
  const int npairs = h / 2 + 1;
  for (int w = tid; w < npairs * T; w += nthreads) {
    const int k = w / T, rho = w - k * T;
    const int m = (h - k) % h;
    const int pk = P.ax.inv[k], pm = P.ax.inv[m];
    const cfloat xk = buf[pk * TP + rho];
    if (k == 0) {
      float xh = 0.f;
      if (P.nyq_packed)
        xh = xk.y;
      else if (r0 + rho < P.rows)
        xh = P.in_nyq[r0 + rho].x;
      buf[pk * TP + rho] = cmake(xk.x + xh, xk.x - xh);
    } else {
      const cfloat xm = buf[pm * TP + rho];
      const cfloat E = cmake(xk.x + xm.x, xk.y - xm.y);
      const cfloat Dk = cmake(xk.x - xm.x, xk.y + xm.y);
      const cfloat O = cmul(Dk, cconj(P.twr[k]));
      buf[pk * TP + rho] = cadd(E, cmul_si<+1>(O));
      if (m != k) buf[pm * TP + rho] = cadd(cconj(E), cmul_si<+1>(cconj(O)));
    }
  }
  MVN_SYNC();
  lds_fft_dit<+1, T>(buf, alt, TP, P.ax, tw, tid, nthreads);
  for (int w0 = tid; w0 < total; w0 += U * nthreads) {
    if (!single) {
      long idx[U];
#pragma unroll
      for (int u = 0; u < U; ++u) {
        int w = w0 + u * nthreads;
        w = w < total ? w : total - 1;
        const int rho = (int)mvn_fastdiv((unsigned)w, (unsigned)h, P.hmul), j = w - rho * h;
        long row = r0 + rho;
        row = row < last_row ? row : last_row;
        idx[u] = row * P.RP + 2 * j;
      }
      if constexpr (U16)
        mvn_epilogue_fetch_batch_u16<U>(epi, idx, eu);
      else
        mvn_epilogue_fetch_batch<U>(epi, idx, ea, eb);
    }
#pragma unroll
    for (int u = 0; u < U; ++u) {
      const int w = w0 + u * nthreads;
      const int rho = (int)mvn_fastdiv((unsigned)w, (unsigned)h, P.hmul), j = w - rho * h;
      const long row = r0 + rho;
      if (w < total && row <= last_row) {
        if constexpr (U16) ea[u] = mvn_u16_pair_widen(eu[u]);
        if constexpr (NM) {
          const cfloat q = mvn_nm_pair(epi, buf[j * TP + rho], ea[u], nacc, P.st, (rin >> rho) & 1u, 2 * j);
          if (KEEP)
            buf[j * TP + rho] = q;
          else
            *reinterpret_cast<cfloat*>(P.out_real + row * P.RP + 2 * j) = q;
        } else if constexpr (STATS) {
          const cfloat y = mvn_update_pair_stats<TV>(epi, row * P.RP + 2 * j, buf[j * TP + rho], ea[u], eb[u], acc,
                                                     P.st, (rin >> rho) & 1u, 2 * j);
          if (KEEP) buf[j * TP + rho] = y;
        } else if (KEEP)
          buf[j * TP + rho] = mvn_epilogue_pair_value<TV>(epi.mode, epi, row * P.RP + 2 * j,
                                                          buf[j * TP + rho], ea[u], eb[u]);
        else
          mvn_epilogue_pair<TV>(epi, P.out_real, row * P.RP + 2 * j, buf[j * TP + rho], ea[u], eb[u]);
      }
    }
  }
  if (KEEP) {
    MVN_SYNC();
    rows_r2c_even_tail<T>(P, r0, buf, alt, tw, tid, nthreads);
  }
  if constexpr (STATS) mvn_stat_flush(P.st, acc, tile, (P.rows + T - 1) / T, lds, tid, nthreads);
  if constexpr (NM) mvn_nm_flush(P.st, nacc, tile, (P.rows + T - 1) / T, lds, tid, nthreads);
}

template <int T>
MVN_HD void rows_r2c_odd_body(const RowsParams& P, long tile, int tid, int nthreads, cfloat* lds) {
  const int n = P.h, TP = P.TP;
  const long r0 = tile * T;
  cfloat* buf = lds;
  cfloat* alt = lds + P.lds_alt;
  const cfloat* tw = lds_stage_twiddles(lds + P.lds_tw, P.ax, tid, nthreads);
  for (int w = tid; w < T * n; w += nthreads) {
    const int rho = (int)mvn_fastdiv((unsigned)w, (unsigned)n, P.hmul), j = w - rho * n;
    const long row = r0 + rho;
    float v = 0.f;
    if (row < P.rows) v = P.in_real[row * P.RP + j];
    buf[j * TP + rho] = cmake(v, 0.f);
  }
  MVN_SYNC();
  lds_fft_dif<-1, T>(buf, alt, TP, P.ax, tw, tid, nthreads);
  for (int w = tid; w < T * P.C; w += nthreads) {
    const int rho = (int)mvn_fastdiv((unsigned)w, (unsigned)P.C, P.Cmul), k = w - rho * P.C;
    const long row = r0 + rho;
    if (row < P.rows) P.out_cplx[row * P.C + k] = buf[P.ax.inv[k] * TP + rho];
  }
}

template <int T, bool STATS = false, bool U16 = false, bool TV = false, bool NM = false>
MVN_HD void rows_c2r_odd_body(const RowsParams& P, long tile, int tid, int nthreads, cfloat* lds) {
  EpilogueParams epi = P.epi;
  mvn_arm_poison(epi);
  MvnStatAcc acc;
  unsigned rin = 0;
  if constexpr (STATS) {
    mvn_stat_init(acc);
    rin = mvn_stat_tile_rows<T>(P, tile * T);
  }
  if constexpr (TV) epi.mode = MVN_EPI_UPDATE;
  MvnNmAcc nacc;
  if constexpr (NM) {
    mvn_nm_init(nacc);
    rin = mvn_stat_tile_rows<T>(P, tile * T);
  }
  const int n = P.h, TP = P.TP;
  const long r0 = tile * T;
  cfloat* buf = lds;
  cfloat* alt = lds + P.lds_alt;
  const cfloat* tw = lds_stage_twiddles(lds + P.lds_tw, P.ax, tid, nthreads);
  for (int w = tid; w < T * n; w += nthreads) {
    const int rho = (int)mvn_fastdiv((unsigned)w, (unsigned)n, P.hmul), k = w - rho * n;
    const long row = r0 + rho;
    cfloat v = cmake(0.f, 0.f);
    if (row < P.rows) {
      if (k < P.C) {
        v = P.in_cplx[row * P.C + k];
        if (k == 0) v.y = 0.f;
      } else {
        v = cconj(P.in_cplx[row * P.C + (n - k)]);
      }
    }
    buf[P.ax.inv[k] * TP + rho] = v;
  }
  MVN_SYNC();
  lds_fft_dit<+1, T>(buf, alt, TP, P.ax, tw, tid, nthreads);
  for (int w = tid; w < T * n; w += nthreads) {
    const int rho = (int)mvn_fastdiv((unsigned)w, (unsigned)n, P.hmul), j = w - rho * n;
    const long row = r0 + rho;
    if constexpr (NM) {
      MVN_FP_EXACT
      if (row < P.rows) {
        const long i = row * P.RP + j;
        const float view = U16 ? (float)epi.view16[i] : epi.view[i];
        P.out_real[i] = mvn_nm_one(epi, view, buf[j * TP + rho].x * epi.scale, nacc,
                                   ((rin >> rho) & 1u) && (unsigned)(j - P.st.o2) < P.st.n2);
      }
    } else if constexpr (STATS) {
      if (row < P.rows)
        mvn_update_stats<TV>(epi, row * P.RP + j, buf[j * TP + rho].x, acc,
                         ((rin >> rho) & 1u) && (unsigned)(j - P.st.o2) < P.st.n2);
    } else if constexpr (U16) {
      MVN_FP_EXACT
      if (row < P.rows) {
        const long i = row * P.RP + j;
        const float view = (float)epi.view16[i];
        P.out_real[i] = mvn_quotient_g(view, buf[j * TP + rho].x * epi.scale, epi.guard_zero_view);
      }
    } else if (row < P.rows) {
// ... 132 lines not shown
```

Baseline: 101.5.

## Move outer radix-8 stage of axis-1 FFT into last-axis row passes on line layout

The line-layout last-axis passes now map each 16-row tile to rows strided by 64 along axis 1 and apply the first (outermost) radix-8 stage of the 512-point axis-1 FFT, with twiddles, inside the r2c post and c2r pre steps. The fused mid-axis kernel correspondingly drops its own first radix-8 stage, its 64-entry-per-m twiddle table and the digit-reversed bin mapping, which shortens its phase schedule and shrinks LDS. This trades extra arithmetic and a strided row gather in the row kernels for fewer LDS round-trips and barriers in the mid-axis kernel. The line path is now restricted to d1 == 512 and whole 512-row ranges.

Result: no change. 101.1 (-0.4%).

```diff
diff --git a/libmultiviewnative_amd/csrc/mvn_backend_emu.cpp b/libmultiviewnative_amd/csrc/mvn_backend_emu.cpp
--- a/libmultiviewnative_amd/csrc/mvn_backend_emu.cpp
+++ b/libmultiviewnative_amd/csrc/mvn_backend_emu.cpp
@@ -195,8 +195,8 @@
   typedef FxCtx<FxRowsRegs<H>, FxRowsCfg<H>::NT> Ctx;
   typedef FxCtx<FxRowsStatRegs<H>, FxRowsCfg<H>::NT> SCtx;
   typedef FxCtx<FxRowsNmRegs<H>, FxRowsCfg<H>::NT> NCtx;
-  if (!fx_rows_lines_ok<H>() || !p.fixed || p.h != H || p.C != H || !p.nyq_packed || p.lines_d1 < 1 ||
-      p.lines_d1 % FxRowsCfg<H>::T || p.row_base % FxRowsCfg<H>::T || p.rows != ntiles * FxRowsCfg<H>::T)
+  if (!fx_rows_lines_ok<H>() || !p.fixed || p.h != H || p.C != H || !p.nyq_packed || !p.lines_tw || p.lines_d1 != FX_LINES_N1 ||
+      p.row_base % FX_LINES_N1 || p.rows % FX_LINES_N1 || p.rows != ntiles * FxRowsCfg<H>::T)
     throw std::invalid_argument("mvn: line-layout last-axis pass outside its range");
 #pragma omp parallel
   {
diff --git a/libmultiviewnative_amd/csrc/mvn_engine.cpp b/libmultiviewnative_amd/csrc/mvn_engine.cpp
--- a/libmultiviewnative_amd/csrc/mvn_engine.cpp
+++ b/libmultiviewnative_amd/csrc/mvn_engine.cpp
@@ -282,6 +282,7 @@
   p.lines = 1;
   p.lines_d1 = P.L.d1;
   p.row_base = row0;
+  p.lines_tw = P.ax1.view.tw;
   p.nyq_packed = 1;
 }
 
diff --git a/libmultiviewnative_amd/csrc/mvn_fixed.hpp b/libmultiviewnative_amd/csrc/mvn_fixed.hpp
--- a/libmultiviewnative_amd/csrc/mvn_fixed.hpp
+++ b/libmultiviewnative_amd/csrc/mvn_fixed.hpp
@@ -973,7 +973,34 @@
   fx_build_pair_table<H>(reinterpret_cast<FxPair*>(twr + C::TWR), tid);
 }
 
-template <int H>
+#define FX_LINES_N1 512
+template <bool LINES>
+MVN_HD long fx_real_row(long r0, int rho) {
+  if constexpr (LINES)
+    return (r0 & ~(long)(FX_LINES_N1 - 1)) + ((r0 & (FX_LINES_N1 - 1)) >> 3) + (rho >> 3) + 64 * (rho & 7);
+  else
+    return r0 + rho;
+}
+#if defined(__HIPCC__) && !defined(MVN_HOST_EMU)
+MVN_HD int fx_wave_uniform(int v) { return __builtin_amdgcn_readfirstlane(v); }
+#else
+MVN_HD int fx_wave_uniform(int v) { return v; }
+#endif
+
+template <int DIR>
+MVN_HD void fx_lines_outer8(const cfloat* tw, int n, cfloat* a) {
+  if (DIR < 0) {
+    dftR<8, -1>(a);
+#pragma unroll
+    for (int k = 1; k < 8; ++k) a[k] = cmul(a[k], tw[n * k]);
+  } else {
+#pragma unroll
+    for (int k = 1; k < 8; ++k) a[k] = cmulc(a[k], tw[n * k]);
+    dftR<8, +1>(a);
+  }
+}
+
+template <int H, bool LINES = false>
 MVN_HD void fx_r2c_load_stage0(const RowsParams& P, long r0, cfloat* buf, cfloat* tws, cfloat* twr,
                                int tid) {
   typedef FxRowsCfg<H> C;
@@ -984,7 +1011,7 @@
     const int w = tid + it * NT;
     if (!C::EXACT && w >= M * C::T) break;
     const int j2 = w % M, rho = w / M;
-    const cfloat* src = reinterpret_cast<const cfloat*>(P.in_real + (r0 + rho) * P.RP) + j2;
+    const cfloat* src = reinterpret_cast<const cfloat*>(P.in_real + fx_real_row<LINES>(r0, rho) * P.RP) + j2;
 #pragma unroll
     for (int j = 0; j < R; ++j) a[it][j] = src[j * M];
   }
@@ -1008,11 +1035,41 @@
   }
 }
 
-template <int H>
+template <int H, bool LINES = false>
 MVN_HD void fx_r2c_post(const RowsParams& P, long r0, cfloat* buf, const cfloat* twr, int tid) {
   typedef FxRowsCfg<H> C;
   constexpr int T = C::T, NT = C::NT;
   const FxPair* tab = reinterpret_cast<const FxPair*>(twr + C::TWR);
+  if constexpr (LINES) {
+    static_assert(T == 16 && (H / 2) % 64 == 0 && H <= NT, "split lines: 16-row tiles, whole waves per e");
+    if (tid >= H) return;
+    const int e = fx_wave_uniform(tid / (H / 2)), k = tid % (H / 2);
+    const int n = ((int)(r0 & (FX_LINES_N1 - 1)) >> 3) + e;
+    const FxPair t = tab[k];
+    cfloat* pa = buf + t.a + 8 * e;
+    cfloat* pb = buf + t.b + 8 * e;
+    const cfloat w = twr[k];
+    cfloat xa[8], xb[8];
+#pragma unroll
+    for (int m = 0; m < 8; ++m) {
+      const cfloat zk = pa[m], zm = pb[m];
+      if (k == 0) {
+        xa[m] = cmake(zk.x + zk.y, zk.x - zk.y);
+        xb[m] = cconj(zm);
+      } else {
+        const cfloat E = cscale(cadd_c(zk, zm), 0.5f);
+        const cfloat D = cscale(csub_c(zk, zm), 0.5f);
+        const cfloat G = cmul(D, w);
+        xa[m] = cadd_i<-1>(E, G);
+        xb[m] = cconj_add_i<-1>(E, G);
+      }
+    }
+    fx_lines_outer8<-1>(P.lines_tw, n, xa);
+    fx_lines_outer8<-1>(P.lines_tw, n, xb);
+#pragma unroll
+    for (int m = 0; m < 8; ++m) pa[m] = xa[m], pb[m] = xb[m];
+    return;
+  }
 #pragma unroll
   for (int it = 0; it < C::ITP; ++it) {
     const int i = tid + it * NT;
@@ -1097,9 +1154,9 @@
   cfloat* buf = lds;
   cfloat* tws = lds + C::TILE;
   cfloat* twr = tws + fx_twsize(H);
-  MVN_PHASE(ctx, (fx_r2c_load_stage0<H>(P, r0, buf, tws, twr, tid)));
+  MVN_PHASE(ctx, (fx_r2c_load_stage0<H, LINES>(P, r0, buf, tws, twr, tid)));
   fx_dif<H, T, TP, C::PAD, NT, -1, 1, C::TWT>(buf, tws, ctx);
-  MVN_PHASE(ctx, (fx_r2c_post<H>(P, r0, buf, twr, tid)));
+  MVN_PHASE(ctx, (fx_r2c_post<H, LINES>(P, r0, buf, twr, tid)));
   MVN_PHASE(ctx, (fx_r2c_store<H, LINES, fx_lines_wide<MVN_EPI_STORE>()>(P, r0, buf, tid)));
 }
 
@@ -1154,7 +1211,7 @@
     for (int it = 0; it < C::IT0; ++it) {
       const int w = tid + it * NT;
       if (!C::EXACT && w >= C::M0 * C::T) break;
-      const unsigned short* src = P.epi.view16 + (r0 + w / C::M0) * P.RP + 2 * (w % C::M0);
+      const unsigned short* src = P.epi.view16 + fx_real_row<LINES>(r0, w / C::M0) * P.RP + 2 * (w % C::M0);
 #pragma unroll
       for (int jo = 0; jo < C::R0; ++jo) r.eu[it][jo] = mvn_u16_pair_fetch(src + 2 * jo * C::M0);
     }
@@ -1163,7 +1220,7 @@
     for (int it = 0; it < C::IT0; ++it) {
       const int w = tid + it * NT;
       if (!C::EXACT && w >= C::M0 * C::T) break;
-      const cfloat* src = reinterpret_cast<const cfloat*>(pa + (r0 + w / C::M0) * P.RP) + (w % C::M0);
+      const cfloat* src = reinterpret_cast<const cfloat*>(pa + fx_real_row<LINES>(r0, w / C::M0) * P.RP) + (w % C::M0);
 #pragma unroll
       for (int jo = 0; jo < C::R0; ++jo) r.ea[it][jo] = src[jo * C::M0];
     }
@@ -1174,7 +1231,7 @@
       const int w = tid + it * NT;
       if (!C::EXACT && w >= C::M0 * C::T) break;
       const cfloat* src =
-          reinterpret_cast<const cfloat*>(P.epi.weights + (r0 + w / C::M0) * P.RP) + (w % C::M0);
+          reinterpret_cast<const cfloat*>(P.epi.weights + fx_real_row<LINES>(r0, w / C::M0) * P.RP) + (w % C::M0);
 #pragma unroll
       for (int jo = 0; jo < C::R0; ++jo) r.eb[it][jo] = src[jo * C::M0];
     }
@@ -1209,11 +1266,41 @@
   }
 }
 
-template <int H>
+template <int H, bool LINES = false>
 MVN_HD void fx_c2r_pre(const RowsParams& P, long r0, cfloat* buf, const cfloat* twr, int tid) {
   typedef FxRowsCfg<H> C;
   constexpr int T = C::T, NT = C::NT;
   const FxPair* tab = reinterpret_cast<const FxPair*>(twr + C::TWR);
+  if constexpr (LINES) {
+    static_assert(T == 16 && (H / 2) % 64 == 0 && H <= NT, "split lines: 16-row tiles, whole waves per e");
+    if (tid >= H) return;
+    const int e = fx_wave_uniform(tid / (H / 2)), k = tid % (H / 2);
+    const int n = ((int)(r0 & (FX_LINES_N1 - 1)) >> 3) + e;
+    const FxPair t = tab[k];
+    cfloat* pa = buf + t.a + 8 * e;
+    cfloat* pb = buf + t.b + 8 * e;
+    const cfloat w = twr[k];
+    cfloat xa[8], xb[8];
+#pragma unroll
+    for (int m = 0; m < 8; ++m) xa[m] = pa[m], xb[m] = pb[m];
+    fx_lines_outer8<+1>(P.lines_tw, n, xa);
+    fx_lines_outer8<+1>(P.lines_tw, n, xb);
+#pragma unroll
+    for (int m = 0; m < 8; ++m) {
+      const cfloat xk = xa[m], xm = xb[m];
+      if (k == 0) {
+        pa[m] = cmake(xk.x + xk.y, xk.x - xk.y);
+        pb[m] = cmake(2.f * xm.x, -2.f * xm.y);
+      } else {
+        const cfloat E = cadd_c(xk, xm);
+        const cfloat Dk = csub_c(xk, xm);
+        const cfloat O = cmulc(Dk, w);
+        pa[m] = cadd_i<+1>(E, O);
+        pb[m] = cconj_add_i<+1>(E, O);
+      }
+    }
+    return;
+  }
 #pragma unroll
   for (int it = 0; it < C::ITP; ++it) {
     const int i = tid + it * NT;
@@ -1238,7 +1325,7 @@
   }
 }
 
-template <int H, bool KEEP, int EPI, typename Regs>
+template <int H, bool KEEP, int EPI, bool LINES = false, typename Regs>
 MVN_HD void fx_c2r_stage0_epilogue(const RowsParams& P, long r0, cfloat* buf, const cfloat* tws, Regs& r, int tid) {
   typedef FxRowsCfg<H> C;
   constexpr int TP = C::TP, NT = C::NT, R = C::R0, M = C::M0;
@@ -1256,9 +1343,10 @@
 #pragma unroll
     for (int k = 1; k < R; ++k) a[k] = cmulc(a[k], tw[k]);
     dftR<R, +1>(a);
-    const long i0 = (r0 + rho) * P.RP + 2 * j2;
+    const long row = fx_real_row<LINES>(r0, rho);
+    const long i0 = row * P.RP + 2 * j2;
     if constexpr (mvn_epi_nm(EPI)) {
-      const bool row_in = mvn_stat_row_in(P.st, r0 + rho);
+      const bool row_in = mvn_stat_row_in(P.st, row);
 #pragma unroll
       for (int jo = 0; jo < R; ++jo) {
         a[jo] = mvn_nm_pair(P.epi, a[jo], fx_operand<EPI>(r.ea[it][jo], r.eu[it][jo]), r.nm, P.st, row_in, 2 * (j2 + jo * M));
@@ -1266,7 +1354,7 @@
       }
     }
     if constexpr (mvn_epi_base(EPI) == MVN_EPI_UPDATE_STATS) {
-      const bool row_in = mvn_stat_row_in(P.st, r0 + rho);
+      const bool row_in = mvn_stat_row_in(P.st, row);
 #pragma unroll
       for (int jo = 0; jo < R; ++jo)
         a[jo] = mvn_update_pair_stats<mvn_epi_tv(EPI)>(P.epi, i0 + 2 * jo * M, a[jo], r.ea[it][jo], r.eb[it][jo], r.st, P.st, row_in,
@@ -1302,11 +1390,11 @@
   cfloat* tws = lds + C::TILE;
   cfloat* twr = tws + fx_twsize(H);
   MVN_PHASE(ctx, (fx_c2r_load<H, EPI, LINES>(P, r0, buf, tws, twr, r, tid)));
-  MVN_PHASE(ctx, (fx_c2r_pre<H>(P, r0, buf, twr, tid)));
+  MVN_PHASE(ctx, (fx_c2r_pre<H, LINES>(P, r0, buf, twr, tid)));
   fx_dit<H, T, TP, C::PAD, NT, +1, 1, C::TWT>(buf, tws, ctx);
-  MVN_PHASE(ctx, (fx_c2r_stage0_epilogue<H, true, EPI>(P, r0, buf, tws, r, tid)));
+  MVN_PHASE(ctx, (fx_c2r_stage0_epilogue<H, true, EPI, LINES>(P, r0, buf, tws, r, tid)));
   fx_dif<H, T, TP, C::PAD, NT, -1, 1, C::TWT>(buf, tws, ctx);
-  MVN_PHASE(ctx, (fx_r2c_post<H>(P, r0, buf, twr, tid)));
+  MVN_PHASE(ctx, (fx_r2c_post<H, LINES>(P, r0, buf, twr, tid)));
   MVN_PHASE(ctx, (fx_r2c_store<H, LINES, fx_lines_wide<EPI>()>(P, r0, buf, tid)));
 }
 
@@ -1320,9 +1408,9 @@
   cfloat* tws = lds + C::TILE;
   cfloat* twr = tws + fx_twsize(H);
   MVN_PHASE(ctx, (fx_c2r_load<H, EPI, LINES>(P, r0, buf, tws, twr, r, tid)));
-  MVN_PHASE(ctx, (fx_c2r_pre<H>(P, r0, buf, twr, tid)));
+  MVN_PHASE(ctx, (fx_c2r_pre<H, LINES>(P, r0, buf, twr, tid)));
   fx_dit<H, T, TP, C::PAD, NT, +1, 1, C::TWT>(buf, tws, ctx);
-  MVN_PHASE(ctx, (fx_c2r_stage0_epilogue<H, false, EPI>(P, r0, buf, tws, r, tid)));
+  MVN_PHASE(ctx, (fx_c2r_stage0_epilogue<H, false, EPI, LINES>(P, r0, buf, tws, r, tid)));
 }
 
 template <int H, int KIND, int EPI, typename Ctx, bool LINES = false>
diff --git a/libmultiviewnative_amd/csrc/mvn_kernels.hip b/libmultiviewnative_amd/csrc/mvn_kernels.hip
--- a/libmultiviewnative_amd/csrc/mvn_kernels.hip
+++ b/libmultiviewnative_amd/csrc/mvn_kernels.hip
@@ -654,8 +654,8 @@
 
 static void check_lines(const RowsParams& p, long nblocks) {
   constexpr int H = 256;
-  if (!fx_rows_lines_ok<H>() || !p.fixed || p.h != H || p.C != H || !p.nyq_packed || p.lines_d1 < 1 ||
-      p.lines_d1 % FxRowsCfg<H>::T || p.row_base % FxRowsCfg<H>::T || p.rows != nblocks * FxRowsCfg<H>::T)
+  if (!fx_rows_lines_ok<H>() || !p.fixed || p.h != H || p.C != H || !p.nyq_packed || !p.lines_tw || p.lines_d1 != FX_LINES_N1 ||
+      p.row_base % FX_LINES_N1 || p.rows % FX_LINES_N1 || p.rows != nblocks * FxRowsCfg<H>::T)
     throw std::invalid_argument("mvn: line-layout last-axis pass outside its range");
 }
 
diff --git a/libmultiviewnative_amd/csrc/mvn_mid_fused.hpp b/libmultiviewnative_amd/csrc/mvn_mid_fused.hpp
--- a/libmultiviewnative_amd/csrc/mvn_mid_fused.hpp
+++ b/libmultiviewnative_amd/csrc/mvn_mid_fused.hpp
@@ -24,7 +24,7 @@
 #define MF_LINES 8
 #define MF_PITCH 576
 #define MF_BUF (MF_LINES * MF_PITCH)
-#define MF_TWL 512
+#define MF_TWL 64
 #define MF_LDS_CFLOATS (4 * MF_BUF + MF_TWL)
 
 struct MidFusedParams {
@@ -144,19 +144,15 @@
 }
 
 MVN_HD void mf_build_twiddles(const MidFusedParams& P, cfloat* twl, int tid) {
-  if (tid < 448) {
-    const int m = tid / 64 + 1, l = tid & 63;
-    twl[tid] = P.tw[l * m];
-  } else if (tid < 448 + 56) {
-    const int e = tid - 448, m = e / 8 + 1, j = e & 7;
-    twl[tid] = P.tw[8 * j * m];
-  }
-}
-MVN_HD cfloat mf_tw0(const cfloat* twl, int l, int m) { return twl[(m - 1) * 64 + l]; }
-MVN_HD cfloat mf_tw1(const cfloat* twl, int l, int m) { return twl[448 + (m - 1) * 8 + (l & 7)]; }
-
-template <int K>
-MVN_HD void mf_fwd0(MfRegs<K>& r, cfloat* buf, int tid) {
+  if (tid < 56) {
+    const int m = tid / 8 + 1, a = tid & 7;
+    twl[tid] = P.tw[8 * a * m];
+  }
+}
+MVN_HD cfloat mf_tw1(const cfloat* twl, int l, int m) { return twl[(m - 1) * 8 + (l >> 3)]; }
+
+template <int K>
+MVN_HD void mf_fwd1(MfRegs<K>& r, cfloat* buf, int tid) {
   const int wv = tid >> 6, l = tid & 63;
   cfloat* line = buf + wv * MF_PITCH;
   cfloat a[8];
@@ -169,171 +165,71 @@
   for (int m = 0; m < 8; ++m) line[72 * m + l] = a[m];
 }
 template <int K>
-MVN_HD void mf_tw0_ahead(MfRegs<K>& r, const cfloat* twl, int tid) {
+MVN_HD void mf_tw1_ahead(MfRegs<K>& r, const cfloat* twl, int tid) {
   const int l = tid & 63;
 #pragma unroll
-  for (int m = 1; m < 8; ++m) r.t2[m] = mf_tw0(twl, l, m);
-}
-template <int K>
-MVN_HD void mf_fwd1_r(MfRegs<K>& r, const cfloat* buf, int tid) {
+  for (int m = 1; m < 8; ++m) r.t2[m] = mf_tw1(twl, l, m);
+}
+template <int K>
+MVN_HD void mf_fwd2_r(MfRegs<K>& r, const cfloat* buf, int tid) {
   const int wv = tid >> 6, l = tid & 63;
   const cfloat* p = buf + wv * MF_PITCH + 72 * (l >> 3) + (l & 7);
 #pragma unroll
   for (int m = 0; m < 8; ++m) r.t[m] = p[8 * m];
 }
 template <int K>
-MVN_HD void mf_fwd1_c(MfRegs<K>& r, const cfloat* twl, int tid) {
+MVN_HD void mf_fwd2_b(const MfRegs<K>& r, cfloat* buf, int tid) {
+  const int wv = tid >> 6, l = tid & 63;
+  cfloat* line = buf + wv * MF_PITCH;
+#pragma unroll
+  for (int m = 0; m < 8; ++m) line[64 * m + l] = r.t[m];
+}
+template <int K>
+MVN_HD void mf_fwd2_r2(MfRegs<K>& r, const cfloat* buf, int tid) {
+  const int wv = tid >> 6, l = tid & 63;
+  const cfloat* p = buf + wv * MF_PITCH + 72 * (l >> 3) + (l & 7);
+#pragma unroll
+  for (int m = 0; m < 8; ++m) r.t2[m] = p[8 * m];
+}
+template <int K>
+MVN_HD void mf_fwd2_b2(const MfRegs<K>& r, cfloat* buf, int tid) {
+  const int wv = tid >> 6, l = tid & 63;
+  cfloat* line = buf + wv * MF_PITCH;
+#pragma unroll
+  for (int m = 0; m < 8; ++m) line[64 * m + l] = r.t2[m];
+}
+
+template <int K>
+MVN_HD void mf_inv2_r(MfRegs<K>& r, const cfloat* buf, int tid) {
+  const int wv = tid >> 6, l = tid & 63;
+  const cfloat* line = buf + wv * MF_PITCH;
+#pragma unroll
+  for (int m = 0; m < 8; ++m) r.t[m] = line[64 * m + l];
+}
+template <int K>
+MVN_HD void mf_inv2_b(const MfRegs<K>& r, cfloat* buf, int tid) {
+  const int wv = tid >> 6, l = tid & 63;
+  cfloat* p = buf + wv * MF_PITCH + 72 * (l >> 3) + (l & 7);
+#pragma unroll
+  for (int m = 0; m < 8; ++m) p[8 * m] = r.t[m];
+}
+template <int K>
+MVN_HD void mf_inv1_r(MfRegs<K>& r, const cfloat* buf, int tid) {
+  const int wv = tid >> 6, l = tid & 63;
+  const cfloat* line = buf + wv * MF_PITCH;
+#pragma unroll
+  for (int m = 0; m < 8; ++m) r.t[m] = line[72 * m + l];
+}
+template <int K>
+MVN_HD void mf_inv1_c_store(MfRegs<K>& r, const cfloat* twl, cfloat* dst, int tid) {
   const int l = tid & 63;
-  (void)l;
-  dftR<8, -1>(r.t);
-#pragma unroll
-  for (int m = 1; m < 8; ++m) r.t[m] = mf_cmul(r.t[m], mf_tw1(twl, l, m));
-}
-template <int K>
-MVN_HD void mf_fwd1_r2(MfRegs<K>& r, const cfloat* buf, int tid) {
-  const int wv = tid >> 6, l = tid & 63;
-  const cfloat* p = buf + wv * MF_PITCH + 72 * (l >> 3) + (l & 7);
-#pragma unroll
-  for (int m = 0; m < 8; ++m) r.t2[m] = p[8 * m];
-}
-template <int K>
-MVN_HD void mf_fwd1_c2(MfRegs<K>& r, const cfloat* twl, int tid) {
-  const int l = tid & 63;
-  (void)l;
-  dftR<8, -1>(r.t2);
-#pragma unroll
-  for (int m = 1; m < 8; ++m) r.t2[m] = mf_cmul(r.t2[m], mf_tw1(twl, l, m));
-}
-template <int K>
-MVN_HD void mf_fwd1_b2(const MfRegs<K>& r, cfloat* buf, int tid) {
-  const int wv = tid >> 6, l = tid & 63;
-  cfloat* p = buf + wv * MF_PITCH + 72 * (l >> 3) + (l & 7);
-#pragma unroll
-  for (int m = 0; m < 8; ++m) p[9 * m] = r.t2[m];
-}
-template <int K>
-MVN_HD void mf_fwd2_r2(MfRegs<K>& r, const cfloat* buf, int tid) {
-  const int wv = tid >> 6, l = tid & 63;
-  const cfloat* p = buf + wv * MF_PITCH + 72 * (l >> 3) + 9 * (l & 7);
-#pragma unroll
-  for (int m = 0; m < 8; ++m) r.t2[m] = p[m];
-}
-template <int K>
-MVN_HD void mf_fwd2_b2(const MfRegs<K>& r, cfloat* buf, int tid) {
-  const int wv = tid >> 6, l = tid & 63;
-  cfloat* line = buf + wv * MF_PITCH;
-#pragma unroll
-  for (int m = 0; m < 8; ++m) line[64 * m + l] = r.t2[m];
-}
-template <int K>
-MVN_HD void mf_fwd1_a(MfRegs<K>& r, const cfloat* buf, const cfloat* twl, int tid) {
-  mf_fwd1_r<K>(r, buf, tid);
-  mf_fwd1_c<K>(r, twl, tid);
-}
-template <int K>
-MVN_HD void mf_fwd1_b(const MfRegs<K>& r, cfloat* buf, int tid) {
-  const int wv = tid >> 6, l = tid & 63;
-  cfloat* p = buf + wv * MF_PITCH + 72 * (l >> 3) + (l & 7);
-#pragma unroll
-  for (int m = 0; m < 8; ++m) p[9 * m] = r.t[m];
-}
-template <int K>
-MVN_HD void mf_fwd2_r(MfRegs<K>& r, const cfloat* buf, int tid) {
-  const int wv = tid >> 6, l = tid & 63;
-  const cfloat* p = buf + wv * MF_PITCH + 72 * (l >> 3) + 9 * (l & 7);
-#pragma unroll
-  for (int m = 0; m < 8; ++m) r.t[m] = p[m];
-}
-template <int K>
-MVN_HD void mf_fwd2_a(MfRegs<K>& r, const cfloat* buf, int tid) {
-  mf_fwd2_r<K>(r, buf, tid);
-  dftR<8, -1>(r.t);
-}
-template <int K>
-MVN_HD void mf_fwd2_b(const MfRegs<K>& r, cfloat* buf, int tid) {
-  const int wv = tid >> 6, l = tid & 63;
-  cfloat* line = buf + wv * MF_PITCH;
-#pragma unroll
-  for (int m = 0; m < 8; ++m) line[64 * m + l] = r.t[m];
-}
-
-template <int K>
-MVN_HD void mf_inv2_r(MfRegs<K>& r, const cfloat* buf, int tid) {
-  const int wv = tid >> 6, l = tid & 63;
-  const cfloat* line = buf + wv * MF_PITCH;
-#pragma unroll
-  for (int m = 0; m < 8; ++m) r.t[m] = line[64 * m + l];
-}
-template <int K>
-MVN_HD void mf_inv2_a(MfRegs<K>& r, const cfloat* buf, int tid) {
-  mf_inv2_r<K>(r, buf, tid);
-  dftR<8, +1>(r.t);
-}
-template <int K>
-MVN_HD void mf_inv2_b(const MfRegs<K>& r, cfloat* buf, int tid) {
-  const int wv = tid >> 6, l = tid & 63;
-  cfloat* p = buf + wv * MF_PITCH + 72 * (l >> 3) + 9 * (l & 7);
-#pragma unroll
-  for (int m = 0; m < 8; ++m) p[m] = r.t[m];
-}
-template <int K>
-MVN_HD void mf_inv1_r(MfRegs<K>& r, const cfloat* buf, int tid) {
-  const int wv = tid >> 6, l = tid & 63;
-  const cfloat* p = buf + wv * MF_PITCH + 72 * (l >> 3) + (l & 7);
-#pragma unroll
-  for (int m = 0; m < 8; ++m) r.t[m] = p[9 * m];
-}
-template <int K>
-MVN_HD void mf_inv1_c(MfRegs<K>& r, const cfloat* twl, int tid) {
-  const int l = tid & 63;
-  (void)l;
 #pragma unroll
   for (int m = 1; m < 8; ++m) r.t[m] = mf_cmulc(r.t[m], mf_tw1(twl, l, m));
   dftR<8, +1>(r.t);
-}
-template <int K>
-MVN_HD void mf_inv1_a(MfRegs<K>& r, const cfloat* buf, const cfloat* twl, int tid) {
-  mf_inv1_r<K>(r, buf, tid);
-  mf_inv1_c<K>(r, twl, tid);
-}
-template <int K>
-MVN_HD void mf_inv1_b(const MfRegs<K>& r, cfloat* buf, int tid) {
-  const int wv = tid >> 6, l = tid & 63;
-  cfloat* p = buf + wv * MF_PITCH + 72 * (l >> 3) + (l & 7);
-#pragma unroll
-  for (int m = 0; m < 8; ++m) p[8 * m] = r.t[m];
-}
-template <int K>
-MVN_HD void mf_inv0_r(MfRegs<K>& r, const cfloat* buf, int tid) {
-  const int wv = tid >> 6, l = tid & 63;
-  const cfloat* line = buf + wv * MF_PITCH;
-#pragma unroll
-  for (int m = 0; m < 8; ++m) r.t[m] = line[72 * m + l];
-}
-template <int K>
-MVN_HD void mf_inv0_c_store(MfRegs<K>& r, const cfloat* twl, cfloat* dst, int tid) {
-  const int l = tid & 63;
-#pragma unroll
-  for (int m = 1; m < 8; ++m) r.t[m] = mf_cmulc(r.t[m], mf_tw0(twl, l, m));
-  dftR<8, +1>(r.t);
 #pragma unroll
   for (int m = 0; m < 8; ++m) dst[l + 64 * m] = r.t[m];
 }
-template <int K>
-MVN_HD void mf_inv0_store(MfRegs<K>& r, const cfloat* buf, const cfloat* twl, cfloat* dst, int tid) {
-  mf_inv0_r<K>(r, buf, tid);
-  mf_inv0_c_store<K>(r, twl, dst, tid);
-}
-
-template <int K>
-MVN_HD void mf_store_line(const MidFusedParams& P, MfRegs<K>& r, const cfloat* buf, const cfloat* twl, int c, int z0,
-                          int nout, int batch, int tid) {
-  const int m = batch * MF_LINES + (tid >> 6) - (K - 1);
-  if (m < 0 || m >= nout) return;
-  int z = z0 + m;
-  z = z >= P.d0 ? z - P.d0 : z;
-  mf_inv0_store<K>(r, buf, twl, P.out + ((long)z * P.H + c) * MF_N1, tid);
-}
+
 template <int K>
 MVN_HD void mf_store_line_c(const MidFusedParams& P, MfRegs<K>& r, const cfloat* twl, int c, int z0, int nout, int batch,
                             int tid) {
@@ -341,11 +237,11 @@
   if (m < 0 || m >= nout) return;
   int z = z0 + m;
   z = z >= P.d0 ? z - P.d0 : z;
-  mf_inv0_c_store<K>(r, twl, P.out + ((long)z * P.H + c) * MF_N1, tid);
-}
-
-MVN_HD int mf_bin_of(int f) { return 64 * (f >> 6) + 8 * (f & 7) + ((f >> 3) & 7); }
-MVN_HD int mf_freq_of(int q) { return ((q >> 3) & 7) + 8 * (q & 7) + 64 * (q >> 6); }
+  mf_inv1_c_store<K>(r, twl, P.out + ((long)z * P.H + c) * MF_N1, tid);
+}
+
+MVN_HD int mf_bin_of(int f) { return f; }
+MVN_HD int mf_freq_of(int q) { return q; }
 MVN_HD cfloat mf_herm0(cfloat a, cfloat b) { return cmake(0.5f * (a.x + b.x), 0.5f * (a.y - b.y)); }
 MVN_HD cfloat mf_hermh(cfloat a, cfloat b) { return cmake(0.5f * (a.y + b.y), 0.5f * (b.x - a.x)); }
 
@@ -355,10 +251,7 @@
   const int f = mf_freq_of(tid), fm = (MF_N1 - f) & (MF_N1 - 1);
   r.qm = mf_bin_of(fm);
   r.dcmode = f == fm ? MF_DC_SELF : (f < MF_N1 / 2 ? MF_DC_LOW : MF_DC_HIGH);
-  {
-    const int l = tid & 63, g = (l >> 3) + 8 * (l & 7);
-    r.cpar = g == 0 ? 64 : 8 * ((64 - g) & 7) + ((64 - g) >> 3);
-  }
+  r.cpar = 64 - (tid & 63);
   const cfloat* tp = P.taps + r.qm;
 #pragma unroll
   for (int j = 0; j < K; ++j) {
@@ -476,7 +369,7 @@
     MVN_PHASE_NOSYNC(ctx, (mf_setup_dc<K>(P, r, tid)));
   }
   MVN_PHASE(ctx, (void)0);
-  MVN_PHASE_NOSYNC(ctx, (mf_tw0_ahead<K>(r, twl, tid)));
+  MVN_PHASE_NOSYNC(ctx, (mf_tw1_ahead<K>(r, twl, tid)));
 #if defined(__HIPCC__) && !defined(MVN_HOST_EMU)
   const int wave_young = mvn_uniform((ctx.tid >> 8) & 1);
 #define MF_PRIO_RESET() __builtin_amdgcn_s_setprio(0);
@@ -506,27 +399,23 @@
     if (dc) {
       MF_WPHASE(ctx, (mf_inv2_fix_dc<K>(r, inv, tid)));
     }
-    MF_WPHASE(ctx, (mf_fwd0<K>(r, fwd, tid), mf_fetch<K>(P, r, c, z0, i + 2, nsteps, tid)));
+    MF_WPHASE(ctx, (mf_fwd1<K>(r, fwd, tid), mf_fetch<K>(P, r, c, z0, i + 2, nsteps, tid)));
     MF_FLINE(0)
+    MF_FLINE(1)
     MF_WPHASE(ctx, (dftR<8, +1>(r.t), mf_inv2_b<K>(r, inv, tid)));
     MF_WPHASE(ctx, (mf_inv1_r<K>(r, inv, tid)));
-    MF_WPHASE(ctx, (mf_fwd1_r2<K>(r, fwd, tid)));
-    MF_FLINE(1)
+    MF_WPHASE(ctx, (mf_fwd2_r2<K>(r, fwd, tid)));
     MF_FLINE(2)
+    MF_FLINE(3)
     MF_PRIO_RAISE_YOUNG()
-    MF_WPHASE(ctx, (mf_inv1_c<K>(r, twl, tid), mf_inv1_b<K>(r, inv, tid)));
-    MF_WPHASE(ctx, (mf_fwd1_c2<K>(r, twl, tid), mf_fwd1_b2<K>(r, fwd, tid)));
-    MF_WPHASE(ctx, (mf_inv0_r<K>(r, inv, tid)));
-    MF_WPHASE(ctx, (mf_fwd2_r2<K>(r, fwd, tid)));
-    MF_FLINE(3)
+    MF_WPHASE(ctx, (mf_store_line_c<K>(P, r, twl, c, z0, nout, i - 1, tid)));
     MF_FLINE(4)
-    MF_WPHASE(ctx, (mf_store_line_c<K>(P, r, twl, c, z0, nout, i - 1, tid)));
     MF_WPHASE(ctx, (dftR<8, -1>(r.t2), mf_fwd2_b2<K>(r, fwd, tid)));
     MF_FLINE(5)
     MF_FLINE(6)
     MF_FLINE(7)
 #undef MF_FLINE
-    MF_WPHASE(ctx, (mf_tw0_ahead<K>(r, twl, tid)));
+    MF_WPHASE(ctx, (mf_tw1_ahead<K>(r, twl, tid)));
     MVN_PHASE(ctx, (void)0);
   }
 #undef MF_PRIO_RESET
@@ -556,11 +445,9 @@
   const int c = (int)(block - batch * P.H);
   cfloat* twl = lds + 4 * MF_BUF;
   MVN_PHASE(ctx, (mf_taps_load(P, r, batch, c, tid), mf_build_twiddles(P, twl, tid)));
-  MF_WPHASE(ctx, (mf_tw0_ahead<1>(r, twl, tid)));
-  MF_WPHASE(ctx, (mf_fwd0<1>(r, lds, tid)));
-  MF_WPHASE(ctx, (mf_fwd1_a<1>(r, lds, twl, tid)));
-  MF_WPHASE(ctx, (mf_fwd1_b<1>(r, lds, tid)));
-  MF_WPHASE(ctx, (mf_fwd2_a<1>(r, lds, tid)));
+  MF_WPHASE(ctx, (mf_tw1_ahead<1>(r, twl, tid)));
+  MF_WPHASE(ctx, (mf_fwd1<1>(r, lds, tid)));
+  MF_WPHASE(ctx, (mf_fwd2_r<1>(r, lds, tid), dftR<8, -1>(r.t)));
   MF_WPHASE(ctx, (mf_fwd2_b<1>(r, lds, tid)));
   MVN_PHASE_NOSYNC(ctx, (mf_taps_store(P, lds, batch, c, tid)));
 }
diff --git a/libmultiviewnative_amd/csrc/mvn_pass_bodies.hpp b/libmultiviewnative_amd/csrc/mvn_pass_bodies.hpp
--- a/libmultiviewnative_amd/csrc/mvn_pass_bodies.hpp
+++ b/libmultiviewnative_amd/csrc/mvn_pass_bodies.hpp
@@ -517,6 +517,7 @@
   int nyq_packed;
   int lines, lines_d1;
   long row_base;
+  const cfloat* lines_tw;
   MvnStatsParams st;
 };
 
```
